# ruiminshen/yolo-tf

Measured on AMD Instinct MI355X. Metric: train_throughput, higher is better.
Workload: dtype bf16; 1 GPU; Darknet-19 YOLOv2 VOC-20 416x416 training step (standardise+fwd+loss+bwd+Adam), batch 16 per GPU (BASELINE configs[1]); global_batch=16, parallelism=dp1, optimizer=adam, weights=random-init (Xavier, seed 0), collective=none (1 rank)

## Files before the change

include/yolo2_hip.h:

```cpp
#ifndef YOLO2_HIP_H
#define YOLO2_HIP_H

#include <stddef.h>
#include <stdint.h>

#ifdef __cplusplus
extern "C" {
#endif

enum { YOLO2_F32 = 0, YOLO2_BF16 = 1 };
enum {
    YOLO2_OK = 0,
    YOLO2_E_ARG = 1,
    YOLO2_E_LAUNCH = 2,
    YOLO2_E_UNSUPPORTED = 3
};

int yolo2_abi_version(void);
const char *yolo2_last_error(void);
uint32_t yolo2_crc32c(const void *data, size_t n, uint32_t crc);
int yolo2_shutdown(void);
int yolo2_check_async_errors(void *stream);
#define YOLO2_ASYNC_ERROR_WORDS 8
int yolo2_async_error_snapshot(unsigned *host_words, void *stream);

size_t yolo2_conv2d_workspace_bytes(int B, int H, int W, int Cp, int Nf, int ksize, int dtype);
size_t yolo2_bn_workspace_bytes(int C);
size_t yolo2_bias_grad_workspace_bytes(int ld);
size_t yolo2_image_prep_workspace_bytes(int B);
size_t yolo2_loss_workspace_bytes(int B, int cells, int A);
size_t yolo2_nms_workspace_bytes(int B, int N, int C);
size_t yolo2_clip_workspace_bytes(int nseg);
size_t yolo2_augment_workspace_bytes(int B);

int yolo2_conv2d(const void *P, const void *F, const float *bias, void *O,
                 int B, int H, int W, int Cp, int ldp, int Nf, int ldo, int ksize,
                 int dtype, void *stream);

int yolo2_conv2d_ws(const void *P, const void *F, const float *bias, void *O, float *ws,
                    size_t ws_bytes, int B, int H, int W, int Cp, int ldp, int Nf, int ldo,
                    int ksize, int dtype, void *stream);

int yolo2_conv2d_wgrad_accumulates(int B, int H, int W, int Cin, int ldx, int Cout, int ldy, int ksize, int dtype);
int yolo2_conv2d_wgrad(const void *X, const void *dY, float *dW,
                       int B, int H, int W, int Cin, int ldx, int Cout, int ldy, int ksize,
                       int dtype, void *stream);

size_t yolo2_conv2d_wgrad_workspace_bytes(int B, int H, int W, int Cin, int ldx, int Cout, int ldy, int ksize, int dtype);
int yolo2_conv2d_wgrad_ws(const void *X, const void *dY, float *dW, float *ws, size_t ws_bytes, int B, int H, int W,
                          int Cin, int ldx, int Cout, int ldy, int ksize, int dtype, void *stream);
int yolo2_set_deterministic(int on);
int yolo2_get_deterministic(void);

int yolo2_filter_prep(const float *W, void *Ffwd, void *Fdgr, int ksize, int Cin, int ldcin,
                      int Cout, int ldcout, int dtype, void *stream);

#define YOLO2_FILTER_PREP_TILE 64
#define YOLO2_FILTER_PREP_TILE_N 128
int yolo2_filter_prep_blocks(int ksize, int ldcin, int ldcout);
typedef struct yolo2_filter_desc {
    const float *W;
    void *Ffwd;
    void *Fdgr;
    int ksize, cin, ldcin, cout, ldcout, first_block;
} yolo2_filter_desc;
int yolo2_filter_prep_batch(const yolo2_filter_desc *descs_device, int n, int total_blocks, int dtype,
                            void *stream);

int yolo2_adam_filter_prep(const yolo2_filter_desc *descs_device, int n, int total_blocks, const long *small_ranges_device, int n_small,
                           float *params, const float *grads, float *m, float *v, float alpha, float beta1, float beta2, float eps,
                           float gscale, int dtype, void *stream);

int yolo2_conv2d_bias_leaky(const void *P, const void *F, const float *bias, void *O, float *ws, size_t ws_bytes, int B,
                            int H, int W, int Cp, int ldp, int Nf, int ldo, int ksize, float alpha, int dtype, void *stream);

int yolo2_conv2d_dgrad_bn(const void *dY, const void *F, void *dX, float *ws, size_t ws_bytes, int B, int H, int W, int Cp, int ldp,
                          int Nf, int ldo, int ksize, const void *Yprev, const float *mean, const float *var, const float *gamma,
                          const float *beta, float *dgamma, float *dbeta, float *bn_part, double *red_ws, float eps, float alpha,
                          int *pending, int dtype, void *stream);
int yolo2_conv2d_dgrad_bn_fuses(int B, int H, int W, int Nf, int ksize, int dtype);
int yolo2_bn_part_to_grads(float *bn_part, int C, float *dgamma, float *dbeta, void *stream);

#define YOLO2_BN_PART_ROWS 256
int yolo2_conv2d_bn(const void *P, const void *F, void *O, float *ws, size_t ws_bytes, int B, int H, int W, int Cp, int ldp,
                    int Nf, int ldo, int ksize, const float *shift, float *bn_part, int dtype, void *stream);
int yolo2_bn_finalize(float *bn_part, const float *shift, long M, int C, float *mean, float *var, float *moving_mean,
                      float *moving_var, double decay, void *stream);

int yolo2_last_bn_part_rows(void);
int yolo2_bn_fin_supported(int rows, int C, int dtype);
int yolo2_bn_leaky_fin(const void *Y, const float *bn_part, int rows, const float *shift, float *mean, float *var, float *moving_mean,
                       float *moving_var, double decay, const float *gamma, const float *beta, void *A, long M, int C, int lda,
                       float eps, float alpha, float *zero, long zero_floats, int dtype, void *stream);
int yolo2_bn_leaky_pool_fin(const void *Y, const float *bn_part, int rows, const float *shift, float *mean, float *var,
                            float *moving_mean, float *moving_var, double decay, const float *gamma, const float *beta, void *P,
                            unsigned char *idx, void *ymax, void *A_full, int B, int H, int W, int C, int ldp, float eps, float alpha,
                            float *zero, long zero_floats, int dtype, void *stream);
int yolo2_bn_leaky_bwd_apply_fin(const void *dA, int ldda, const void *Y, const float *mean, const float *var, const float *gamma,
                                 const float *beta, const float *part, int rows, long plane_stride, float *dgamma, float *dbeta,
                                 void *dY, long M, int C, float eps, float alpha, float *zero, long zero_floats, int dtype, void *stream);
int yolo2_bn_leaky_pool_bwd_apply_fin(const void *dP, int lddp, const unsigned char *idx, const void *Y, const float *mean,
                                      const float *var, const float *gamma, const float *beta, const float *part, int rows,
                                      long plane_stride, float *dgamma, float *dbeta, void *dY, int B, int H, int W, int C, float eps,
                                      float alpha, float *zero, long zero_floats, int dtype, void *stream);
int yolo2_first_layer_wgrad_bn(const void *X, const void *Y, const void *dP, int lddp, const unsigned char *idx, const float *mean, const float *var,
                               const float *gamma, const float *beta, const float *part, int rows, long plane_stride, float *dgamma, float *dbeta,
                               float *dW, int B, int H, int W, int Cin, float eps, float alpha, float *zero, long zero_floats, int dtype, void *stream);
int yolo2_bn_leaky_bwd_reduce_part(const void *dA, int ldda, const void *Y, const float *mean, const float *var, const float *gamma,
                                   const float *beta, double *ws, int *rows, int rows_limit, long M, int C, float eps, float alpha,
                                   int dtype, void *stream);
int yolo2_bn_leaky_pool_bwd_reduce_part(const void *dP, int lddp, const unsigned char *idx, const void *Y, const float *mean,
                                        const float *var, const float *gamma, const float *beta, double *ws, int *rows,
                                        int rows_limit, int B, int H, int W, int C, float eps, float alpha, int dtype, void *stream);

int yolo2_first_layer_stats(const void *P, const void *F, int B, int H, int W, const float *shift, float *bn_part, int dtype, void *stream);
int yolo2_first_layer_bn_leaky_pool(const void *P, const void *F, const float *mean, const float *var, const float *gamma,
                                    const float *beta, void *Pout, unsigned char *idx, int B, int H, int W, int ldp, float eps,
                                    float alpha, int dtype, void *stream);
int yolo2_first_layer_pool_bwd_reduce(const void *P, const void *F, const void *dP, int lddp, const unsigned char *idx,
                                      const float *mean, const float *var, const float *gamma, const float *beta, float *bn_part,
                                      int B, int H, int W, float eps, float alpha, int dtype, void *stream);
int yolo2_first_layer_pool_bwd_apply(const void *P, const void *F, const void *dP, int lddp, const unsigned char *idx,
                                     const float *mean, const float *var, const float *gamma, const float *beta,
                                     const float *dgamma, const float *dbeta, void *dY, int B, int H, int W, float eps, float alpha,
                                     int dtype, void *stream);

int yolo2_bn_stats(const void *Y, float *mean, float *var, double *ws, long M, int C,
                   int dtype, void *stream);
int yolo2_bn_stats_ema(const void *Y, float *mean, float *var, float *moving_mean, float *moving_var,
                       double decay, double *ws, long M, int C, int dtype, void *stream);
int yolo2_bn_ema(float *moving_mean, float *moving_var, const float *mean, const float *var,
                 int C, double decay, void *stream);
int yolo2_bn_leaky(const void *Y, const float *mean, const float *var, const float *gamma,
                   const float *beta, void *A, long M, int C, int lda, float eps, float alpha,
                   int dtype, void *stream);
int yolo2_bn_leaky_bwd_reduce(const void *dA, int ldda, const void *Y, const float *mean,
                              const float *var, const float *gamma, const float *beta,
                              float *dgamma, float *dbeta, double *ws, long M, int C,
                              float eps, float alpha, int dtype, void *stream);
int yolo2_bn_leaky_bwd_apply(const void *dA, int ldda, const void *Y, const float *mean,
                             const float *var, const float *gamma, const float *beta,
                             const float *dgamma, const float *dbeta, void *dY, long M, int C,
                             float eps, float alpha, int dtype, void *stream);

int yolo2_bn_leaky_pool(const void *Y, const float *mean, const float *var, const float *gamma, const float *beta, void *P,
                        unsigned char *idx, int B, int H, int W, int C, int ldp, float eps, float alpha, int dtype, void *stream);
int yolo2_bn_leaky_pool_bwd_reduce(const void *dP, int lddp, const unsigned char *idx, const void *Y, const float *mean,
                                   const float *var, const float *gamma, const float *beta, float *dgamma, float *dbeta,
                                   double *ws, int B, int H, int W, int C, float eps, float alpha, int dtype, void *stream);
int yolo2_bn_leaky_pool_bwd_apply(const void *dP, int lddp, const unsigned char *idx, const void *Y, const float *mean,
                                  const float *var, const float *gamma, const float *beta, const float *dgamma,
                                  const float *dbeta, void *dY, int B, int H, int W, int C, float eps, float alpha,
                                  int dtype, void *stream);

int yolo2_maxpool_fwd(const void *A, void *P, int B, int H, int W, int C, int stride,
                      int dtype, void *stream);
int yolo2_maxpool_bwd(const void *A, const void *dP, void *dA, int B, int H, int W, int C,
                      int stride, int dtype, void *stream);
int yolo2_maxpool_bwd_acc(const void *A, const void *dP, void *dA, int B, int H, int W, int C, int dtype, void *stream);

int yolo2_reorg(const void *in, void *out, int B, int H, int W, int C, int ldo, int dtype,
                void *stream);
int yolo2_reorg_bwd(const void *dout, int ldd, void *din, int B, int H, int W, int C, int dtype,
                    void *stream);
int yolo2_copy_channels(const void *src, int lds, void *dst, int ldd, long M, int C, int dtype,
                        void *stream);
int yolo2_add_inplace(void *dst, const void *src, long n, int dtype, void *stream);
int yolo2_bias_grad(const void *dY, int ld, float *dbias, double *ws, long M, int C, int dtype,
                    void *stream);

int yolo2_image_prep(const float *img, void *out, double *ws, int B, int HW, int mode, int dtype,
                     void *stream);

int yolo2_head_decode(const void *logits, int ld, const float *anchors, float *conf,
                      float *xy_min, float *xy_max, int *nan_flag, int B, int cell_h, int cell_w,
                      int A, int C, int dtype, void *stream);

int yolo2_head_decode_attrs(const void *logits, int ld, const float *anchors, float *iou, float *prob,
                            float *xy, float *wh, int B, int cell_h, int cell_w, int A, int C,
                            int dtype, void *stream);

int yolo2_loss(const void *logits, int ld, const float *anchors, const float *mask,
               const float *prob, const float *coords, const float *off_min, const float *off_max,
               const float *areas, const float *hparam, float *objectives, void *dlogits,
               float *ws, int B, int cell_h, int cell_w, int A, int C, int dtype, void *stream);
int yolo2_loss_partials(const void *logits, int ld, const float *anchors, const float *mask, const float *prob,
                        const float *coords, const float *off_min, const float *off_max, const float *areas,
                        const float *hparam, void *dlogits, float *ws, int B, int cell_h, int cell_w, int A, int C, int dtype,
                        void *stream);
int yolo2_loss_objectives(const float *ws, float *objectives, int B, int cell_h, int cell_w, int A, void *stream);

int yolo1_loss(const void *net, int ld, const float *mask, const float *prob, const float *coords, const float *off_min,
               const float *off_max, const float *areas, const float *hparam, float *objectives, void *dnet, float *ws,
               int B, int cell_h, int cell_w, int boxes_per_cell, int C, int dtype, void *stream);
int yolo1_head_decode(const void *net, int ld, float *conf, float *xy_min, float *xy_max, int *nan_flag, int B, int cell_h,
                      int cell_w, int boxes_per_cell, int C, int dtype, void *stream);
int yolo2_leaky_bwd(const void *A, const void *dA, void *dZ, long n, float alpha, int dtype, void *stream);
int yolo2_dropout(const void *X, void *Y, unsigned char *mask, long n, float keep_prob, unsigned long long seed, int dtype,
                  void *stream);
int yolo2_dropout_bwd(const void *dY, const unsigned char *mask, void *dX, long n, float keep_prob, int dtype, void *stream);
int yolo2_l2_regularizer(const float *w, float *g, long n, float scale, double *loss, void *stream);

int yolo2_nms(float *conf, const float *xy_min, const float *xy_max, int *order_out, int *ws,
              int B, int N, int C, float threshold, float threshold_iou, void *stream);

int yolo2_adam(float *w, const float *g, float *m, float *v, long n, float alpha, float beta1,
               float beta2, float eps, float gscale, void *stream);
int yolo2_momentum(float *w, const float *g, float *acc, long n, float lr, float momentum,
                   float gscale, void *stream);
int yolo2_sgd(float *w, const float *g, long n, float lr, float gscale, void *stream);
int yolo2_rmsprop(float *w, const float *g, float *ms, float *mom, long n, float lr, float decay,
                  float momentum, float eps, float gscale, void *stream);
int yolo2_adagrad(float *w, const float *g, float *acc, long n, float lr, float gscale,
                  void *stream);
int yolo2_adadelta(float *w, const float *g, float *acc, float *acc_update, long n, float lr,
                   float rho, float eps, float gscale, void *stream);
int yolo2_ftrl(float *w, const float *g, float *accum, float *linear, long n, float lr, float lr_power,
               float l1, float l2, float gscale, void *stream);
int yolo2_scale(float *x, long n, float scale, void *stream);
int yolo2_zero_ranges(float *x, const long *ranges_host, int nranges, void *stream);
int yolo2_bn_fold(const float *W, const float *gamma, const float *beta, const float *moving_mean,
                  const float *moving_var, float *Wf, float *bias, long rows, int C, float eps, void *stream);
int yolo2_clip_by_norm(float *g, const long *seg_off, int nseg, float clip, double *ws,
                       void *stream);
size_t yolo2_clip_fixed_workspace_bytes(int nseg);
int yolo2_clip_by_norm_fixed(float *g, const long *seg_off, int nseg, float clip, double *ws, size_t ws_bytes, void *stream);

int yolo2_selftest_tr16(short *out, void *stream);
int yolo2_debug_last_conv_plan(int *out8);
int yolo2_debug_noop(void *stream);
int yolo2_debug_set_igemm_tap(int mode);
int yolo2_debug_set_s4_abl(int abl);
int yolo2_debug_set_pp(int grid, int sched, int min_steps, int min_share);
int yolo2_debug_set_pp_cost(int cv);
int yolo2_debug_set_streamk_wait_us(int us, int unclamped);
int yolo2_debug_last_wgrad_plan(int *out8);
void yolo2_debug_set_wgrad_variant(int variant);
int yolo2_debug_wgrad_row_plan(int B, int H, int W, int Cin, int Cout, int cus, int force_variant, int *out9);
int yolo2_debug_wgrad_ws_plan(int B, int H, int W, int Cin, int ldx, int Cout, int ldy, int ksize, int dtype, int cus, int *out4);
int yolo2_debug_magic_u32(unsigned d, unsigned *m, unsigned *s);

#define YOLO2_AUG_FLIP 1u
#define YOLO2_AUG_BRIGHTNESS 2u
#define YOLO2_AUG_SATURATION 4u
#define YOLO2_AUG_HUE 8u
#define YOLO2_AUG_CONTRAST 16u
#define YOLO2_AUG_NOISE 32u
#define YOLO2_AUG_GRAY 64u
typedef struct yolo2_augment_params {
    long long src_offset;
    int src_w, src_h;
    int crop_x, crop_y, crop_w, crop_h;
    unsigned flags;
    float brightness, saturation, hue, contrast, noise_scale;
    unsigned long long noise_seed;
} yolo2_augment_params;
int yolo2_augment_images(const unsigned char *src, const yolo2_augment_params *params_device, double *ws, float *out,
                         int B, int H, int W, int any_contrast, void *stream);

int yolo2_transform_labels(const int *objects_class, const float *objects_coord, const int *first_object, float *mask,
                           float *prob, float *coords, float *offset_xy_min, float *offset_xy_max, float *areas, int B,
                           int classes, int cell_width, int cell_height, int *error_flag, void *stream);

int yolo2_set_stream_workgroups(int n);
int yolo2_get_stream_workgroups(void);
int yolo2_cast_f32_bf16(const float *src, void *dst, long n, void *stream);
int yolo2_cast_bf16_f32(const void *src, float *dst, long n, void *stream);
int yolo2_debug_occupy(int workgroups, int *stop, int *started, int max_us, void *stream);

enum { YOLO2_EVAL_MODE_DETECT = 0, YOLO2_EVAL_MODE_ALL = 1 };
enum { YOLO2_EVAL_FP = 0, YOLO2_EVAL_TP = 1, YOLO2_EVAL_IGNORED = 2 };
#define YOLO2_EVAL_MAX_GT_PER_IMAGE 512
#define YOLO2_EVAL_MAX_CLASSES (1 << 20)
#define YOLO2_EVAL_STATE_WORDS 2
typedef struct {
    float score;
    int image;
    int box;
    unsigned class_flag;
} yolo2_eval_record;
size_t yolo2_eval_record_bytes(long max_records);
size_t yolo2_eval_collect_workspace_bytes(int B);
size_t yolo2_eval_workspace_bytes(long max_records, int C);
size_t yolo2_eval_result_bytes(int C);
int yolo2_eval_collect(const float *conf, const float *xy_min, const float *xy_max, const int *gt_class, const float *gt_box,
                       const unsigned char *gt_difficult, const int *gt_first, int G, int B, int N, int C, int n_valid, int image_base,
                       int mode, float threshold, float iou_threshold, void *records, long max_records, unsigned long long *state,
                       int *npos, int *ws, void *stream);
int yolo2_eval_finalize(const void *records, long max_records, unsigned long long *state, const int *npos, int C, int n_images, int N,
                        void *ws, size_t ws_bytes, void *results, void *sorted_records, int *cum_tp, int *cum_fp, void *stream);

#define YOLO2_EVAL_COCO_MAX_AREAS 4
#define YOLO2_EVAL_COCO_MAX_IOUS 10
#define YOLO2_EVAL_COCO_MAX_RECALLS 101
#define YOLO2_EVAL_COCO_MAX_SLICES 8
#define YOLO2_EVAL_COCO_MAX_DETS 128
#define YOLO2_EVAL_COCO_MAX_CLASSES 1024
typedef struct {
    float score;
    int image;
    int box;
    int cls;
    int rank;
    unsigned reserved;
    unsigned long long matched;
    unsigned long long ignored;
} yolo2_eval_coco_record;
size_t yolo2_eval_coco_record_bytes(long max_records);
size_t yolo2_eval_coco_collect_workspace_bytes(int B, int N, int C);
size_t yolo2_eval_coco_workspace_bytes(long max_records, int C);
size_t yolo2_eval_coco_result_bytes(int S, int T, int A, int C);
int yolo2_eval_coco_collect(const float *conf, const float *xy_min, const float *xy_max, const int *gt_class, const float *gt_box,
                            const float *gt_area, const unsigned char *gt_flags, const int *gt_first, const float *scale, int G, int B,
                            int N, int C, int n_valid, int image_base, int mode, float threshold, const float *area_ranges, int A,
                            const float *iou_thresholds, int T, int max_dets, void *records, long max_records,
                            unsigned long long *state, int *npig, void *ws, size_t ws_bytes, void *stream);
int yolo2_eval_coco_finalize(const void *records, long max_records, unsigned long long *state, const int *npig, int C, int n_images, int N,
                             int A, int T, int max_dets, const int *slices, int S, const double *recall_thresholds, int R, void *ws,
                             size_t ws_bytes, void *results, void *stream);

#define YOLO2_ANCHOR_MAX_K 32
#define YOLO2_ANCHOR_MAX_JOBS 65535
#define YOLO2_ANCHOR_MAX_BOXES ((1 << 27) - 1)
size_t yolo2_anchor_workspace_bytes(int jobs, int kmax);
int yolo2_anchor_assign(const float *boxes, int n, const float *centroids, const int *job_k, int jobs, int kmax,
                        unsigned long long *ws, size_t ws_bytes, const int *done, unsigned char *assignment, void *stream);
int yolo2_anchor_update(float *centroids, const int *job_k, int jobs, int kmax, unsigned long long *ws, size_t ws_bytes, int n,
                        int *done, int *iterations, long long *counts, double *avg_iou, void *stream);

#define YOLO2_HIST_BUCKETS 1550
#define YOLO2_HIST_WORDS (YOLO2_HIST_BUCKETS + 6)
typedef struct yolo2_hist_job {
    const void *base;
    long long rows;
    int c, ld, dtype;
    int first_item;
} yolo2_hist_job;
size_t yolo2_histogram_workspace_bytes(int njobs);
size_t yolo2_histogram_result_bytes(int njobs);
int yolo2_histogram_items(long long rows, int c, int ld, int dtype);
int yolo2_histogram(const yolo2_hist_job *jobs, int njobs, int items, void *out, size_t out_bytes, void *ws, size_t ws_bytes, void *stream);

#define YOLO2_IMAGE_GROUP 8
#define YOLO2_IMAGE_RECORD_BYTES 16
typedef struct yolo2_image_job {
    const void *base;
    long long rows;
    int c, ld, dtype;
    int first_item;
    long long out_offset;
    long long sum_offset;
} yolo2_image_job;
size_t yolo2_image_summary_workspace_bytes(int njobs, long long sum_pixels);
size_t yolo2_image_summary_result_bytes(int njobs, long long image_bytes);
int yolo2_image_summary_items(long long rows, int c, int ld, int dtype);
int yolo2_image_summary_depth(int c);
int yolo2_image_summary(const yolo2_image_job *jobs, int njobs, int items, void *out, size_t out_bytes, void *ws, size_t ws_bytes, void *stream);

enum { YOLO2_I8_OUT_I8 = 0, YOLO2_I8_OUT_BF16 = 1, YOLO2_I8_OUT_F32 = 2, YOLO2_I8_OUT_ACC = 3 };
int yolo2_conv2d_i8(const void *P, const void *F, const float *mult, const float *bias, void *O, int B, int H, int W, int Cp, int ldp,
                    int Nf, int ldo, int ksize, float alpha, float inv_s_out, int out_kind, void *stream);
typedef struct yolo2_absmax_job {
    const void *base;
    long long rows;
    int c, ld, dtype;
    int slot;
} yolo2_absmax_job;
int yolo2_absmax(const yolo2_absmax_job *jobs, int njobs, unsigned *out, void *stream);
int yolo2_quantize(const void *X, int ldx, void *Q, int ldq, long rows, int c, float inv_s, int dtype, void *stream);
int yolo2_maxpool_i8(const void *A, int lda, void *P, int ldp, int B, int H, int W, int C, int stride, void *stream);
int yolo2_reorg_i8(const void *in, void *out, int B, int H, int W, int C, int ldo, void *stream);

#ifdef __cplusplus
}
#endif
#endif
```

yolo_tf_amd/_lib.py:

```python
import ctypes
import os

_HERE = os.path.dirname(os.path.abspath(__file__))
LIB_PATH = os.environ.get('YOLO2_LIB_PATH') or os.path.join(_HERE, 'csrc', 'libyolo2hip.so')

F32, BF16 = 0, 1
I8_OUT_I8, I8_OUT_BF16, I8_OUT_F32, I8_OUT_ACC = 0, 1, 2, 3


class HipKernelError(RuntimeError):
    pass


_p = ctypes.c_void_p
_i = ctypes.c_int
_l = ctypes.c_long
_f = ctypes.c_float

SIGNATURES = {
    'yolo2_conv2d': [_p, _p, _p, _p, _i, _i, _i, _i, _i, _i, _i, _i, _i, _p],
    'yolo2_conv2d_ws': [_p, _p, _p, _p, _p, ctypes.c_size_t, _i, _i, _i, _i, _i, _i, _i, _i, _i, _p],
    'yolo2_conv2d_bias_leaky': [_p, _p, _p, _p, _p, ctypes.c_size_t, _i, _i, _i, _i, _i, _i, _i, _i, _f, _i, _p],
    'yolo2_conv2d_dgrad_bn': [_p, _p, _p, _p, ctypes.c_size_t, _i, _i, _i, _i, _i, _i, _i, _i, _p, _p, _p, _p, _p, _p, _p, _p, _p, _f, _f, _p, _i, _p],
    'yolo2_bn_part_to_grads': [_p, _i, _p, _p, _p],
    'yolo2_debug_noop': [_p],
    'yolo2_conv2d_wgrad': [_p, _p, _p, _i, _i, _i, _i, _i, _i, _i, _i, _i, _p],
    'yolo2_conv2d_wgrad_ws': [_p, _p, _p, _p, ctypes.c_size_t, _i, _i, _i, _i, _i, _i, _i, _i, _i, _p],
    'yolo2_set_deterministic': [_i],
    'yolo2_filter_prep': [_p, _p, _p, _i, _i, _i, _i, _i, _i, _p],
    'yolo2_filter_prep_batch': [_p, _i, _i, _i, _p],
    'yolo2_adam_filter_prep': [_p, _i, _i, _p, _i, _p, _p, _p, _p, _f, _f, _f, _f, _f, _i, _p],
    'yolo2_first_layer_stats': [_p, _p, _i, _i, _i, _p, _p, _i, _p],
    'yolo2_first_layer_bn_leaky_pool': [_p, _p, _p, _p, _p, _p, _p, _p, _i, _i, _i, _i, _f, _f, _i, _p],
    'yolo2_first_layer_pool_bwd_reduce': [_p, _p, _p, _i, _p, _p, _p, _p, _p, _p, _i, _i, _i, _f, _f, _i, _p],
    'yolo2_first_layer_pool_bwd_apply': [_p, _p, _p, _i, _p, _p, _p, _p, _p, _p, _p, _p, _i, _i, _i, _f, _f, _i, _p],
    'yolo2_conv2d_bn': [_p, _p, _p, _p, ctypes.c_size_t, _i, _i, _i, _i, _i, _i, _i, _i, _p, _p, _i, _p],
    'yolo2_bn_finalize': [_p, _p, _l, _i, _p, _p, _p, _p, ctypes.c_double, _p],
    'yolo2_bn_leaky_fin': [_p, _p, _i, _p, _p, _p, _p, _p, ctypes.c_double, _p, _p, _p, _l, _i, _i, _f, _f, _p, _l, _i, _p],
    'yolo2_bn_leaky_pool_fin': [_p, _p, _i, _p, _p, _p, _p, _p, ctypes.c_double, _p, _p, _p, _p, _p, _p, _i, _i, _i, _i, _i, _f, _f, _p, _l, _i, _p],
    'yolo2_bn_leaky_bwd_apply_fin': [_p, _i, _p, _p, _p, _p, _p, _p, _i, _l, _p, _p, _p, _l, _i, _f, _f, _p, _l, _i, _p],
    'yolo2_first_layer_wgrad_bn': [_p, _p, _p, _i, _p, _p, _p, _p, _p, _p, _i, _l, _p, _p, _p, _i, _i, _i, _i, _f, _f, _p, _l, _i, _p],
    'yolo2_bn_leaky_pool_bwd_apply_fin': [_p, _i, _p, _p, _p, _p, _p, _p, _p, _i, _l, _p, _p, _p, _i, _i, _i, _i, _f, _f, _p, _l, _i, _p],
    'yolo2_bn_leaky_bwd_reduce_part': [_p, _i, _p, _p, _p, _p, _p, _p, _p, _i, _l, _i, _f, _f, _i, _p],
    'yolo2_bn_leaky_pool_bwd_reduce_part': [_p, _i, _p, _p, _p, _p, _p, _p, _p, _p, _i, _i, _i, _i, _i, _f, _f, _i, _p],
    'yolo2_bn_leaky_pool': [_p, _p, _p, _p, _p, _p, _p, _i, _i, _i, _i, _i, _f, _f, _i, _p],
    'yolo2_bn_leaky_pool_bwd_reduce': [_p, _i, _p, _p, _p, _p, _p, _p, _p, _p, _p, _i, _i, _i, _i, _f, _f, _i, _p],
    'yolo2_bn_leaky_pool_bwd_apply': [_p, _i, _p, _p, _p, _p, _p, _p, _p, _p, _p, _i, _i, _i, _i, _f, _f, _i, _p],
    'yolo2_augment_images': [_p, _p, _p, _p, _i, _i, _i, _i, _p],
    'yolo2_transform_labels': [_p, _p, _p, _p, _p, _p, _p, _p, _p, _i, _i, _i, _i, _p, _p],
    'yolo2_bn_stats': [_p, _p, _p, _p, _l, _i, _i, _p],
    'yolo2_bn_stats_ema': [_p, _p, _p, _p, _p, ctypes.c_double, _p, _l, _i, _i, _p],
    'yolo2_bn_ema': [_p, _p, _p, _p, _i, ctypes.c_double, _p],
    'yolo2_bn_leaky': [_p, _p, _p, _p, _p, _p, _l, _i, _i, _f, _f, _i, _p],
    'yolo2_bn_leaky_bwd_reduce': [_p, _i, _p, _p, _p, _p, _p, _p, _p, _p, _l, _i, _f, _f, _i, _p],
    'yolo2_bn_leaky_bwd_apply': [_p, _i, _p, _p, _p, _p, _p, _p, _p, _p, _l, _i, _f, _f, _i, _p],
    'yolo2_maxpool_fwd': [_p, _p, _i, _i, _i, _i, _i, _i, _p],
    'yolo2_maxpool_bwd': [_p, _p, _p, _i, _i, _i, _i, _i, _i, _p],
    'yolo2_maxpool_bwd_acc': [_p, _p, _p, _i, _i, _i, _i, _i, _p],
    'yolo2_reorg': [_p, _p, _i, _i, _i, _i, _i, _i, _p],
    'yolo2_reorg_bwd': [_p, _i, _p, _i, _i, _i, _i, _i, _p],
    'yolo2_copy_channels': [_p, _i, _p, _i, _l, _i, _i, _p],
    'yolo2_add_inplace': [_p, _p, _l, _i, _p],
    'yolo2_bias_grad': [_p, _i, _p, _p, _l, _i, _i, _p],
    'yolo2_image_prep': [_p, _p, _p, _i, _i, _i, _i, _p],
    'yolo2_head_decode': [_p, _i, _p, _p, _p, _p, _p, _i, _i, _i, _i, _i, _i, _p],
    'yolo2_head_decode_attrs': [_p, _i, _p, _p, _p, _p, _p, _i, _i, _i, _i, _i, _i, _p],
    'yolo2_loss': [_p, _i, _p, _p, _p, _p, _p, _p, _p, ctypes.POINTER(_f), _p, _p, _p, _i, _i, _i, _i, _i, _i, _p],
    'yolo2_loss_partials': [_p, _i, _p, _p, _p, _p, _p, _p, _p, ctypes.POINTER(_f), _p, _p, _i, _i, _i, _i, _i, _i, _p],
    'yolo2_loss_objectives': [_p, _p, _i, _i, _i, _i, _p],
    'yolo1_loss': [_p, _i, _p, _p, _p, _p, _p, _p, ctypes.POINTER(_f), _p, _p, _p, _i, _i, _i, _i, _i, _i, _p],
    'yolo1_head_decode': [_p, _i, _p, _p, _p, _p, _i, _i, _i, _i, _i, _i, _p],
    'yolo2_leaky_bwd': [_p, _p, _p, _l, _f, _i, _p],
    'yolo2_dropout': [_p, _p, _p, _l, _f, ctypes.c_ulonglong, _i, _p],
    'yolo2_dropout_bwd': [_p, _p, _p, _l, _f, _i, _p],
    'yolo2_l2_regularizer': [_p, _p, _l, _f, _p, _p],
    'yolo2_nms': [_p, _p, _p, _p, _p, _i, _i, _i, _f, _f, _p],
    'yolo2_adam': [_p, _p, _p, _p, _l, _f, _f, _f, _f, _f, _p],
    'yolo2_momentum': [_p, _p, _p, _l, _f, _f, _f, _p],
    'yolo2_sgd': [_p, _p, _l, _f, _f, _p],
    'yolo2_rmsprop': [_p, _p, _p, _p, _l, _f, _f, _f, _f, _f, _p],
    'yolo2_adagrad': [_p, _p, _p, _l, _f, _f, _p],
    'yolo2_adadelta': [_p, _p, _p, _p, _l, _f, _f, _f, _f, _p],
    'yolo2_clip_by_norm': [_p, _p, _i, _f, _p, _p],
    'yolo2_clip_by_norm_fixed': [_p, _p, _i, _f, _p, ctypes.c_size_t, _p],
    'yolo2_ftrl': [_p, _p, _p, _p, _l, _f, _f, _f, _f, _f, _p],
    'yolo2_scale': [_p, _l, _f, _p],
    'yolo2_zero_ranges': [_p, _p, _i, _p],
    'yolo2_bn_fold': [_p, _p, _p, _p, _p, _p, _p, _l, _i, _f, _p],
    'yolo2_selftest_tr16': [_p, _p],
    'yolo2_set_stream_workgroups': [_i],
    'yolo2_cast_f32_bf16': [_p, _p, _l, _p],
    'yolo2_cast_bf16_f32': [_p, _p, _l, _p],
    'yolo2_debug_occupy': [_i, _p, _p, _i, _p],
    'yolo2_check_async_errors': [_p],
    'yolo2_async_error_snapshot': [_p, _p],
    'yolo2_debug_set_streamk_wait_us': [_i, _i],
    'yolo2_eval_collect': [_p, _p, _p, _p, _p, _p, _p, _i, _i, _i, _i, _i, _i, _i, _f, _f, _p, _l, _p, _p, _p, _p],
    'yolo2_eval_finalize': [_p, _l, _p, _p, _i, _i, _i, _p, ctypes.c_size_t, _p, _p, _p, _p, _p],
    'yolo2_eval_coco_collect': [_p] * 9 + [_i] * 7 + [_f, _p, _i, _p, _i, _i, _p, _l, _p, _p, _p, ctypes.c_size_t, _p],
    'yolo2_eval_coco_finalize': [_p, _l, _p, _p, _i, _i, _i, _i, _i, _i, _p, _i, _p, _i, _p, ctypes.c_size_t, _p, _p],
    'yolo2_anchor_assign': [_p, _i, _p, _p, _i, _i, _p, ctypes.c_size_t, _p, _p, _p],
    'yolo2_anchor_update': [_p, _p, _i, _i, _p, ctypes.c_size_t, _i, _p, _p, _p, _p, _p],
    'yolo2_histogram': [_p, _i, _i, _p, ctypes.c_size_t, _p, ctypes.c_size_t, _p],
    'yolo2_image_summary': [_p, _i, _i, _p, ctypes.c_size_t, _p, ctypes.c_size_t, _p],
    'yolo2_conv2d_i8': [_p, _p, _p, _p, _p, _i, _i, _i, _i, _i, _i, _i, _i, _f, _f, _i, _p],
    'yolo2_absmax': [_p, _i, _p, _p],
    'yolo2_quantize': [_p, _i, _p, _i, _l, _i, _f, _i, _p],
    'yolo2_maxpool_i8': [_p, _i, _p, _i, _i, _i, _i, _i, _i, _p],
    'yolo2_reorg_i8': [_p, _p, _i, _i, _i, _i, _i, _p],
}

QUERIES = {
    'yolo2_abi_version': (_i, []),
    'yolo2_last_error': (ctypes.c_char_p, []),
    'yolo2_shutdown': (_i, []),
    'yolo2_crc32c': (ctypes.c_uint32, [_p, ctypes.c_size_t, ctypes.c_uint32]),
    'yolo2_conv2d_wgrad_accumulates': (_i, [_i] * 9),
    'yolo2_filter_prep_blocks': (_i, [_i, _i, _i]),
    'yolo2_conv2d_dgrad_bn_fuses': (_i, [_i] * 6),
    'yolo2_debug_set_wgrad_variant': (None, [_i]),
    'yolo2_last_bn_part_rows': (_i, []),
    'yolo2_get_stream_workgroups': (_i, []),
    'yolo2_bn_fin_supported': (_i, [_i, _i, _i]),
    'yolo2_debug_last_conv_plan': (_i, [ctypes.POINTER(_i)]),
    'yolo2_debug_set_igemm_tap': (_i, [_i]),
    'yolo2_debug_set_pp': (_i, [_i, _i, _i, _i]),
    'yolo2_debug_set_pp_cost': (_i, [_i]),
    'yolo2_debug_set_s4_abl': (_i, [_i]),
    'yolo2_debug_last_wgrad_plan': (_i, [ctypes.POINTER(_i)]),
    'yolo2_debug_wgrad_row_plan': (_i, [_i, _i, _i, _i, _i, _i, _i, ctypes.POINTER(_i)]),
    'yolo2_debug_wgrad_ws_plan': (_i, [_i] * 10 + [ctypes.POINTER(_i)]),
    'yolo2_conv2d_wgrad_workspace_bytes': (ctypes.c_size_t, [_i] * 9),
    'yolo2_get_deterministic': (_i, []),
    'yolo2_debug_magic_u32': (_i, [ctypes.c_uint, ctypes.POINTER(ctypes.c_uint), ctypes.POINTER(ctypes.c_uint)]),
    'yolo2_conv2d_workspace_bytes': (ctypes.c_size_t, [_i] * 7),
    'yolo2_bn_workspace_bytes': (ctypes.c_size_t, [_i]),
    'yolo2_bias_grad_workspace_bytes': (ctypes.c_size_t, [_i]),
    'yolo2_image_prep_workspace_bytes': (ctypes.c_size_t, [_i]),
    'yolo2_loss_workspace_bytes': (ctypes.c_size_t, [_i, _i, _i]),
    'yolo2_nms_workspace_bytes': (ctypes.c_size_t, [_i, _i, _i]),
    'yolo2_clip_workspace_bytes': (ctypes.c_size_t, [_i]),
    'yolo2_clip_fixed_workspace_bytes': (ctypes.c_size_t, [_i]),
    'yolo2_augment_workspace_bytes': (ctypes.c_size_t, [_i]),
    'yolo2_eval_record_bytes': (ctypes.c_size_t, [_l]),
    'yolo2_eval_collect_workspace_bytes': (ctypes.c_size_t, [_i]),
    'yolo2_eval_workspace_bytes': (ctypes.c_size_t, [_l, _i]),
    'yolo2_eval_result_bytes': (ctypes.c_size_t, [_i]),
    'yolo2_eval_coco_record_bytes': (ctypes.c_size_t, [_l]),
    'yolo2_eval_coco_collect_workspace_bytes': (ctypes.c_size_t, [_i, _i, _i]),
    'yolo2_eval_coco_workspace_bytes': (ctypes.c_size_t, [_l, _i]),
    'yolo2_eval_coco_result_bytes': (ctypes.c_size_t, [_i, _i, _i, _i]),
    'yolo2_anchor_workspace_bytes': (ctypes.c_size_t, [_i, _i]),
    'yolo2_histogram_workspace_bytes': (ctypes.c_size_t, [_i]),
    'yolo2_histogram_result_bytes': (ctypes.c_size_t, [_i]),
    'yolo2_histogram_items': (_i, [ctypes.c_longlong, _i, _i, _i]),
    'yolo2_image_summary_workspace_bytes': (ctypes.c_size_t, [_i, ctypes.c_longlong]),
    'yolo2_image_summary_result_bytes': (ctypes.c_size_t, [_i, ctypes.c_longlong]),
    'yolo2_image_summary_items': (_i, [ctypes.c_longlong, _i, _i, _i]),
    'yolo2_image_summary_depth': (_i, [_i]),
}


class AugmentParams(ctypes.Structure):
    _fields_ = [('src_offset', ctypes.c_longlong), ('src_w', _i), ('src_h', _i), ('crop_x', _i), ('crop_y', _i), ('crop_w', _i), ('crop_h', _i),
                ('flags', ctypes.c_uint), ('brightness', _f), ('saturation', _f), ('hue', _f), ('contrast', _f), ('noise_scale', _f),
                ('noise_seed', ctypes.c_ulonglong)]


class HistJob(ctypes.Structure):
    _fields_ = [('base', ctypes.c_void_p), ('rows', ctypes.c_longlong), ('c', _i), ('ld', _i), ('dtype', _i), ('first_item', _i)]


class ImageJob(ctypes.Structure):
    _fields_ = [('base', ctypes.c_void_p), ('rows', ctypes.c_longlong), ('c', _i), ('ld', _i), ('dtype', _i), ('first_item', _i),
                ('out_offset', ctypes.c_longlong), ('sum_offset', ctypes.c_longlong)]


class AbsmaxJob(ctypes.Structure):
    _fields_ = [('base', ctypes.c_void_p), ('rows', ctypes.c_longlong), ('c', _i), ('ld', _i), ('dtype', _i), ('slot', _i)]


class FilterDesc(ctypes.Structure):
    _fields_ = [('W', ctypes.c_void_p), ('Ffwd', ctypes.c_void_p), ('Fdgr', ctypes.c_void_p), ('ksize', _i), ('cin', _i),
                ('ldcin', _i), ('cout', _i), ('ldcout', _i), ('first_block', _i)]


_lib = None
MISSING = set()


def _mapped_hip_runtimes():
    try:
        with open('/proc/self/maps') as f:
            return sorted({line.split()[-1] for line in f if 'libamdhip64' in line})
    except OSError:
        return []


def load():
    global _lib
    if _lib is not None:
        return _lib
    if not os.path.exists(LIB_PATH):
        raise HipKernelError(
            'HIP extension %s is missing: run `python yolo_tf_amd/csrc/build.py` (or __graft_entry__.build()). '
            'There is no CPU fallback.' % LIB_PATH)
    import torch
    lib = ctypes.CDLL(LIB_PATH)
    runtimes = _mapped_hip_runtimes()
    if len(runtimes) > 1:
        raise HipKernelError('two HIP runtimes are mapped in this process (%s): something loaded %s before torch' % (', '.join(runtimes), LIB_PATH))
    baseline = os.environ.get('YOLO2_LIB_BASELINE') == '1' and bool(os.environ.get('YOLO2_LIB_PATH'))

    def resolve(name):
        try:
            return getattr(lib, name)
        except AttributeError:
            if not baseline:
                raise
            MISSING.add(name)

            def absent(*_args, _name=name):
                raise HipKernelError('%s is not exported by the baseline library %s' % (_name, LIB_PATH))
            setattr(lib, name, absent)
            return None
    for name, (res, args) in QUERIES.items():
        fn = resolve(name)
        if fn is not None:
            fn.restype = res
            fn.argtypes = args
    for name, args in SIGNATURES.items():
        fn = resolve(name)
        if fn is not None:
            fn.restype = _i
            fn.argtypes = args
    _lib = lib
    over = env_overrides()
    if over:
        import warnings
        warnings.warn('YOLO2_* switches set in the environment change kernel selection away from the tested defaults: %s' % ', '.join(over))
    return lib


def env_overrides():
    return sorted('%s=%s' % (k, v) for k, v in os.environ.items() if k.startswith('YOLO2_'))


def query(name, *args):
    return getattr(load(), name)(*args)


def call(name, *args):
    lib = load()
    rc = getattr(lib, name)(*args)
    if rc != 0:
        raise HipKernelError('%s failed (code %d): %s' % (name, rc, lib.yolo2_last_error().decode()))


def ptr(t):
    return None if t is None else t.data_ptr()


def dtype_code(torch_dtype):
    import torch
    if torch_dtype == torch.float32:
        return F32
    if torch_dtype == torch.bfloat16:
        return BF16
    raise ValueError('unsupported dtype %r' % (torch_dtype,))
```

yolo_tf_amd/csrc/conv_c64.hip:

```cpp
#include "common.h"
#include "conv_shared.h"
#include <atomic>

#define C64_TP 256
#define C64_KSTEPS 36
#define C64_STAT_ROWS 32
#define C64_FPITCH 1168

__device__ __forceinline__ int c64_slot_filter(int rho) { return 16 * ((rho >> 2) & 1) + (rho & 3) + 4 * (rho >> 3); }
__device__ __forceinline__ unsigned c64_div(unsigned q, unsigned m, unsigned s) { return __umulhi(q, m) >> s; }

struct C64Geo {
    int H, W, M, Mp;
    int L;
    int RR;
    int HLa;
    int NP0;
    int shl_off;
    unsigned mP, sP, mH, sH;
};

template <int MODE, int NFG>
__global__ __launch_bounds__(512) void conv_c64_fwd_kernel(
    const bf16 *__restrict__ X, unsigned x_bytes, const bf16 *__restrict__ F, bf16 *__restrict__ O, C64Geo g,
    const float *__restrict__ vec, float *__restrict__ bn_part, float alpha) {
    extern __shared__ __attribute__((aligned(1024))) unsigned char smem[];
    constexpr int NB = NFG == 4 ? 2 : 1;
    constexpr int NPASS = NFG == 4 ? 2 : 1;
    constexpr int ROWB = NFG * 64;
    const int H = g.H, W = g.W, Mp = g.Mp;
    const int tid = threadIdx.x, lane = tid & 63;
    const int wave = __builtin_amdgcn_readfirstlane(tid >> 6);
    const int fg = NFG == 4 ? (wave & 3) : 0;
    const int pg = NFG == 4 ? (wave >> 2) : wave;
    const int half = lane >> 5, l31 = lane & 31;
    const unsigned P1 = (unsigned)(W + 1), H1 = (unsigned)(H + 1);
    const int s0 = (int)blockIdx.x * g.L;
    const int e0 = min(s0 + g.L, Mp);
    if (s0 >= Mp) return;
    const int RRB = g.RR * 128, NPR = g.RR >> 3;
    const int pbase = s0 - g.HLa;

    const __amdgpu_buffer_rsrc_t rsrcX = __builtin_amdgcn_make_buffer_rsrc(const_cast<bf16 *>(X), 0, x_bytes, 0x00020000);
    typedef __attribute__((address_space(3))) void *lds_void_ptr;
    typedef const __attribute__((address_space(3))) bf16x8 *lds_frag_ptr;

    bf16x8 filt[C64_KSTEPS];
    auto load_filter = [&]() {
        constexpr int RPR = NFG == 4 ? 64 : 32, FROUND = RPR * C64_FPITCH;
        const __amdgpu_buffer_rsrc_t rsrcF = __builtin_amdgcn_make_buffer_rsrc(const_cast<bf16 *>(F), 0, (unsigned)(NFG * 32) * 1152u, 0x00020000);
        unsigned char *const fst = smem + g.NP0 * 1024;
#pragma unroll 1
        for (int rd = 0; rd < (NFG == 4 ? 2 : 1); ++rd) {
            for (int p = wave; p * 1024 < FROUND; p += 8) {
                const int pos = p * 1024 + lane * 16;
                const int n = pos / C64_FPITCH, off = pos - n * C64_FPITCH;
                const unsigned voff = (off < 1152 && n < RPR) ? (unsigned)((RPR * rd + n) * 1152 + off) : Y2_OOB;
                __builtin_amdgcn_raw_ptr_buffer_load_lds(rsrcF, (lds_void_ptr)(fst + p * 1024), 16, voff, 0, 0, 0);
            }
            asm volatile("s_waitcnt vmcnt(0)" ::: "memory");
            __syncthreads();
            if (NFG == 1 || (fg >> 1) == rd) {
                const unsigned a0 = y2_lds_addr(fst) + (unsigned)((32 * (fg & 1) + c64_slot_filter(l31)) * C64_FPITCH + 16 * half);
#pragma unroll
                for (int st = 0; st < C64_KSTEPS; ++st) filt[st] = *(lds_frag_ptr)(uintptr_t)(a0 + (unsigned)(st * 32));
            }
            __syncthreads();
        }
    };

    const int prow = lane >> 3;
    auto stage_piece = [&](int j, int slot) {
        const int row = j * 8 + prow;
        const unsigned q = (unsigned)(pbase + row);
        const unsigned R = c64_div(q, g.mP, g.sP);
        const unsigned img = c64_div(R, g.mH, g.sH);
        const unsigned c = q - __umul24(R, P1), r = R - __umul24(img, H1);
        const bool ok = (q < (unsigned)Mp) & (c < (unsigned)W) & (r < (unsigned)H);
        const unsigned m = q - R - __umul24(img, (unsigned)W);
        const unsigned voff = ok ? m * 128u + (unsigned)((((lane & 7) ^ ((row >> 1) & 7))) << 4) : Y2_OOB;
        __builtin_amdgcn_raw_ptr_buffer_load_lds(rsrcX, (lds_void_ptr)(smem + slot * 1024), 16, voff, 0, 0, 0);
    };
    for (int j = wave; j < g.NP0; j += 8) stage_piece(j, j);
    load_filter();

    const unsigned lds0 = y2_lds_addr(smem);
    unsigned abase[9];
#pragma unroll
    for (int tp = 0; tp < 9; ++tp) {
        const int shift = (tp / 3 - 1) * (W + 1) + (tp % 3 - 1);
        const int row = pg * (NFG == 4 ? 64 : 32) + l31 + g.HLa + shift;
        abase[tp] = (unsigned)(row * 128 + ((half ^ ((row >> 1) & 7)) << 4));
    }

    typedef __attribute__((ext_vector_type(2))) float f32x2;
    f32x2 cst[8];
    float *const shl = reinterpret_cast<float *>(smem + g.shl_off);
    float tq[8];
#pragma unroll
    for (int qd = 0; qd < 8; ++qd) tq[qd] = 0.f;
    if (MODE == 1) {
        if (tid < 128) shl[tid] = vec ? vec[tid] : 0.f;
        asm volatile("s_waitcnt lgkmcnt(0)" ::: "memory");
    }
#pragma unroll
    for (int r2 = 0; r2 < 8; ++r2) {
        const int f = 32 * fg + 16 * half + 2 * r2;
        cst[r2] = (MODE == 2 && vec) ? f32x2{vec[f], vec[f + 1]} : f32x2{0.f, 0.f};
    }

    const int T = (e0 - s0 + C64_TP - 1) / C64_TP;
    int pslot = g.NP0;
    if (pslot >= NPR) pslot -= NPR;
    unsigned tro = 0;
    for (int t = 0; t < T; ++t) {
        __builtin_amdgcn_s_barrier();
        const int tb = s0 + t * C64_TP;
        if (t + 1 < T) {
#pragma unroll
            for (int u = 0; u < 4; ++u) {
                const int k = wave + 8 * u;
                int sl = pslot + k;
                if (sl >= NPR) sl -= NPR;
                stage_piece(g.NP0 + t * 32 + k, sl);
            }
        }
        pslot += 32;
        if (pslot >= NPR) pslot -= NPR;
#pragma unroll 1
        for (int pa = 0; pa < NPASS; ++pa) {
            if (tb + pa * 128 >= e0) break;
            f32x16 acc[2];
#pragma unroll
            for (int i = 0; i < 2; ++i)
#pragma unroll
                for (int r = 0; r < 16; ++r) acc[i][r] = 0.f;
            unsigned poff = tro + (unsigned)(pa * 16384);
            if (poff >= (unsigned)RRB) poff -= (unsigned)RRB;
            bf16x8 fb[2][NB];
            unsigned ad[NB];
            auto load = [&](int st, int set) {
                const int tp = st >> 2, kk = st & 3;
                if (kk == 0) {
                    unsigned x = abase[tp] + poff;
#pragma unroll
                    for (int i = 0; i < NB; ++i) {
                        x = min(x, x - (unsigned)RRB);
                        ad[i] = x + lds0;
                        x += 4096u;
                    }
                }
#pragma unroll
                for (int i = 0; i < NB; ++i) fb[set][i] = *(lds_frag_ptr)(uintptr_t)(ad[i] ^ (unsigned)(kk * 32));
            };
            load(0, 0);
#pragma unroll
            for (int st = 0; st < C64_KSTEPS; ++st) {
                if (st + 1 < C64_KSTEPS) load(st + 1, (st + 1) & 1);
                __builtin_amdgcn_sched_barrier(0);
                if (NFG == 4) {
#pragma unroll
                    for (int i = 0; i < NB; ++i) acc[i] = __builtin_amdgcn_mfma_f32_32x32x16_bf16(filt[st], fb[st & 1][i], acc[i], 0, 0, 0);
                } else {
                    acc[st & 1] = __builtin_amdgcn_mfma_f32_32x32x16_bf16(filt[st], fb[st & 1][0], acc[st & 1], 0, 0, 0);
                }
                __builtin_amdgcn_sched_barrier(0);
            }
            if (NFG == 1) {
#pragma unroll
                for (int r = 0; r < 16; ++r) acc[0][r] += acc[1][r];
            }
#if defined(__HIP_DEVICE_COMPILE__)
            if (pa == NPASS - 1 || tb + (pa + 1) * 128 >= e0)
                asm volatile("s_waitcnt vmcnt(0)" ::: "memory");
            const bool odd = (lane & 1) != 0;
            typedef __attribute__((ext_vector_type(2))) __bf16 bf16x2;
            unsigned pk[NB][8];
            float lfi[NB];
            unsigned moffi[NB];
#pragma unroll
            for (int i = 0; i < NB; ++i) {
                const unsigned q = (unsigned)(tb + (NFG == 4 ? pa * 128 + pg * 64 + i * 32 : pg * 32) + l31);
                const unsigned R = c64_div(q, g.mP, g.sP);
                const unsigned c = q - __umul24(R, P1);
                const unsigned img = c64_div(R, g.mH, g.sH);
                const unsigned r_ = R - __umul24(img, H1);
                const bool live = (q < (unsigned)e0) & (c < (unsigned)W) & (r_ < (unsigned)H);
                const unsigned m = __umul24(__umul24(img, (unsigned)H) + r_, (unsigned)W) + c;
                moffi[i] = live ? m * (unsigned)ROWB + (unsigned)(fg * 64 + half * 32) : 0xffffffffu;
                lfi[i] = live ? 1.0f : 0.0f;
#pragma unroll
                for (int qd = 0; qd < 8; ++qd) {
                    float v0 = acc[i][2 * qd], v1 = acc[i][2 * qd + 1];
                    if (MODE == 2) {
                        v0 += cst[qd][0]; v1 += cst[qd][1];
                        v0 = fmaxf(v0, alpha * v0); v1 = fmaxf(v1, alpha * v1);
                    }
                    const bf16x2 o2 = {(bf16)v0, (bf16)v1};
                    pk[i][qd] = __builtin_bit_cast(unsigned, o2);
                }
            }
            __builtin_amdgcn_sched_barrier(0);
#pragma unroll
            for (int i = 0; i < NB; ++i) {
                unsigned s0_[4], s1_[4];
#pragma unroll
                for (int d = 0; d < 4; ++d) {
                    const unsigned x = pk[i][d], y = pk[i][4 + d];
                    const unsigned xs = (unsigned)__builtin_amdgcn_mov_dpp((int)x, 0xB1, 0xF, 0xF, true), ys = (unsigned)__builtin_amdgcn_mov_dpp((int)y, 0xB1, 0xF, 0xF, true);
                    s0_[d] = odd ? ys : x;
                    s1_[d] = odd ? y : xs;
                }
                const unsigned mo_even = (unsigned)__builtin_amdgcn_mov_dpp((int)moffi[i], 0xA0, 0xF, 0xF, true);
                const unsigned mo_odd = (unsigned)__builtin_amdgcn_mov_dpp((int)moffi[i], 0xF5, 0xF, 0xF, true);
                const unsigned lo16 = odd ? 16u : 0u;
                if (mo_even != 0xffffffffu)
                    *reinterpret_cast<u32x4 *>(reinterpret_cast<unsigned char *>(O) + mo_even + lo16) = u32x4{s0_[0], s0_[1], s0_[2], s0_[3]};
                if (mo_odd != 0xffffffffu)
                    *reinterpret_cast<u32x4 *>(reinterpret_cast<unsigned char *>(O) + mo_odd + lo16) = u32x4{s1_[0], s1_[1], s1_[2], s1_[3]};
            }
            __builtin_amdgcn_sched_barrier(0);
            if (MODE == 1 && bn_part) {
                const bool odd2 = (lane & 2) != 0;
#pragma unroll
                for (int qd = 0; qd < 8; ++qd) {
                    const f32x2 svq = *reinterpret_cast<const f32x2 *>(shl + 32 * fg + 16 * half + 2 * qd);
                    f32x2 a1 = {0.f, 0.f}, a2 = {0.f, 0.f};
#pragma unroll
                    for (int i = 0; i < NB; ++i) {
                        const f32x2 lf2 = {lfi[i], lfi[i]};
                        const f32x2 y2 = {__builtin_bit_cast(float, pk[i][qd] << 16), __builtin_bit_cast(float, pk[i][qd] & 0xffff0000u)};
                        const f32x2 d2 = (y2 - svq) * lf2;
                        a1 += d2;
                        a2 = __builtin_elementwise_fma(d2, d2, a2);
                    }
                    float k0, k1;
                    {
                        const float t0_ = odd ? a1[0] : a2[0], t1_ = odd ? a1[1] : a2[1];
                        const float r0 = __builtin_bit_cast(float, __builtin_amdgcn_mov_dpp(__builtin_bit_cast(int, t0_), 0xB1, 0xF, 0xF, true));
                        const float r1 = __builtin_bit_cast(float, __builtin_amdgcn_mov_dpp(__builtin_bit_cast(int, t1_), 0xB1, 0xF, 0xF, true));
                        k0 = (odd ? a2[0] : a1[0]) + r0;
                        k1 = (odd ? a2[1] : a1[1]) + r1;
                    }
                    {
                        const float s_ = odd2 ? k0 : k1;
                        const float r_ = __builtin_bit_cast(float, __builtin_amdgcn_mov_dpp(__builtin_bit_cast(int, s_), 0x4E, 0xF, 0xF, true));
                        tq[qd] += (odd2 ? k1 : k0) + r_;
                    }
                }
            }
#endif
        }
        tro += (unsigned)(C64_TP * 128);
        if (tro >= (unsigned)RRB) tro -= (unsigned)RRB;
    }
    if (MODE == 1 && bn_part) {
#pragma unroll
        for (int o = 4; o <= 16; o <<= 1) {
            float x[8];
#pragma unroll
            for (int qd = 0; qd < 8; ++qd) x[qd] = __shfl_xor(tq[qd], o, 64);
#pragma unroll
            for (int qd = 0; qd < 8; ++qd) tq[qd] += x[qd];
        }
        if (l31 < 4) {
            const int slot = (int)(blockIdx.x & (C64_STAT_ROWS - 1));
            const int plane = lane & 1, par = (lane >> 1) & 1;
#pragma unroll
            for (int qd = 0; qd < 8; ++qd)
                unsafeAtomicAdd(bn_part + (plane * Y2_BN_PART_ROWS + slot) * 128 + 32 * fg + 16 * half + 2 * qd + par, tq[qd]);
        }
    }
}

#define C64W_TP 128
__global__ __launch_bounds__(512) void conv_c64_wide_kernel(const bf16 *__restrict__ X, unsigned x_bytes, const bf16 *__restrict__ F, bf16 *__restrict__ O, C64Geo g) {
    extern __shared__ __attribute__((aligned(1024))) unsigned char smem[];
    constexpr int TP = C64W_TP;
    const int H = g.H, W = g.W, Mp = g.Mp;
    const int tid = threadIdx.x, lane = tid & 63;
    const int wave = __builtin_amdgcn_readfirstlane(tid >> 6);
    const int fg = wave & 1, kh = (wave >> 1) & 1, pg = wave >> 2;
    const int half = lane >> 5, l31 = lane & 31;
    const unsigned P1 = (unsigned)(W + 1), H1 = (unsigned)(H + 1);
    const int s0 = (int)blockIdx.x * g.L;
    const int e0 = min(s0 + g.L, Mp);
    if (s0 >= Mp) return;
    const int RRB = g.RR * 128, NPR = g.RR >> 3;
    const int pbase = s0 - g.HLa;
    unsigned char *const xchg = smem + 2 * RRB;

    const __amdgpu_buffer_rsrc_t rsrcX = __builtin_amdgcn_make_buffer_rsrc(const_cast<bf16 *>(X), 0, x_bytes, 0x00020000);
    typedef __attribute__((address_space(3))) void *lds_void_ptr;
    typedef const __attribute__((address_space(3))) bf16x8 *lds_frag_ptr;

    const int prow = lane >> 3;
    auto stage_piece = [&](int j, int slot) {
        const int row = j * 8 + prow;
        const unsigned q = (unsigned)(pbase + row);
        const unsigned R = c64_div(q, g.mP, g.sP);
        const unsigned img = c64_div(R, g.mH, g.sH);
        const unsigned c = q - __umul24(R, P1), r = R - __umul24(img, H1);
        const bool ok = (q < (unsigned)Mp) & (c < (unsigned)W) & (r < (unsigned)H);
        const unsigned m = q - R - __umul24(img, (unsigned)W);
        const unsigned voff = ok ? m * 256u + (unsigned)((((lane & 7) ^ ((row >> 1) & 7))) << 4) : Y2_OOB;
        __builtin_amdgcn_raw_ptr_buffer_load_lds(rsrcX, (lds_void_ptr)(smem + slot * 1024), 16, voff, 0, 0, 0);
        __builtin_amdgcn_raw_ptr_buffer_load_lds(rsrcX, (lds_void_ptr)(smem + RRB + slot * 1024), 16, ok ? voff + 128u : Y2_OOB, 0, 0, 0);
    };
    for (int j = wave; j < g.NP0; j += 8) stage_piece(j, j);

    bf16x8 filt[C64_KSTEPS];
    {
        constexpr int FROUND = 32 * C64_FPITCH;
        const __amdgpu_buffer_rsrc_t rsrcF = __builtin_amdgcn_make_buffer_rsrc(const_cast<bf16 *>(F), 0, 64u * 2304u, 0x00020000);
        unsigned char *const fst = smem + RRB + g.NP0 * 1024;
#pragma unroll 1
        for (int rd = 0; rd < 4; ++rd) {
            const int fgr = rd & 1, khr = rd >> 1;
            for (int p = wave; p * 1024 < FROUND; p += 8) {
                const int pos = p * 1024 + lane * 16;
                const int n = pos / C64_FPITCH, off = pos - n * C64_FPITCH;
                const unsigned voff = (off < 1152 && n < 32) ? (unsigned)((32 * fgr + n) * 2304 + khr * 1152 + off) : Y2_OOB;
                __builtin_amdgcn_raw_ptr_buffer_load_lds(rsrcF, (lds_void_ptr)(fst + p * 1024), 16, voff, 0, 0, 0);
            }
            asm volatile("s_waitcnt vmcnt(0)" ::: "memory");
            __syncthreads();
            if (fg == fgr && kh == khr) {
                const unsigned a0 = y2_lds_addr(fst) + (unsigned)(c64_slot_filter(l31) * C64_FPITCH + 16 * half);
#pragma unroll
                for (int st = 0; st < C64_KSTEPS; ++st) filt[st] = *(lds_frag_ptr)(uintptr_t)(a0 + (unsigned)(st * 32));
            }
            __syncthreads();
        }
    }

    const unsigned lds0 = y2_lds_addr(smem) + (unsigned)(kh * RRB);
    unsigned abase[9];
#pragma unroll
    for (int tp = 0; tp < 9; ++tp) {
        const int shift = (tp / 3 - 1) * (W + 1) + (tp % 3 - 1);
        const int row = pg * 64 + l31 + g.HLa + shift;
        abase[tp] = (unsigned)(row * 128 + ((half ^ ((row >> 1) & 7)) << 4));
    }

    const int T = (e0 - s0 + TP - 1) / TP;
    int pslot = g.NP0;
    if (pslot >= NPR) pslot -= NPR;
    unsigned tro = 0;
    for (int t = 0; t < T; ++t) {
        __builtin_amdgcn_s_barrier();
        const int tb = s0 + t * TP;
        if (t + 1 < T) {
#pragma unroll
            for (int u = 0; u < 2; ++u) {
                const int k = wave + 8 * u;
                int sl = pslot + k;
                if (sl >= NPR) sl -= NPR;
                stage_piece(g.NP0 + t * (TP / 8) + k, sl);
            }
        }
        pslot += TP / 8;
        if (pslot >= NPR) pslot -= NPR;
        f32x16 acc[2];
#pragma unroll
        for (int i = 0; i < 2; ++i)
#pragma unroll
            for (int r = 0; r < 16; ++r) acc[i][r] = 0.f;
        bf16x8 fb[2][2];
        unsigned ad[2];
        auto load = [&](int st, int set) {
            const int tp = st >> 2, kk = st & 3;
            if (kk == 0) {
                unsigned x = abase[tp] + tro;
#pragma unroll
                for (int i = 0; i < 2; ++i) {
                    x = min(x, x - (unsigned)RRB);
                    ad[i] = x + lds0;
                    x += 4096u;
                }
            }
#pragma unroll
            for (int i = 0; i < 2; ++i) fb[set][i] = *(lds_frag_ptr)(uintptr_t)(ad[i] ^ (unsigned)(kk * 32));
        };
        load(0, 0);
#pragma unroll
        for (int st = 0; st < C64_KSTEPS; ++st) {
            if (st + 1 < C64_KSTEPS) load(st + 1, (st + 1) & 1);
            __builtin_amdgcn_sched_barrier(0);
#pragma unroll
            for (int i = 0; i < 2; ++i) acc[i] = __builtin_amdgcn_mfma_f32_32x32x16_bf16(filt[st], fb[st & 1][i], acc[i], 0, 0, 0);
            __builtin_amdgcn_sched_barrier(0);
        }
#if defined(__HIP_DEVICE_COMPILE__)
        f32x16 keep, give;
#pragma unroll
        for (int r = 0; r < 16; ++r) { keep[r] = kh ? acc[1][r] : acc[0][r]; give[r] = kh ? acc[0][r] : acc[1][r]; }
        {
            f32x4 *const xw = reinterpret_cast<f32x4 *>(xchg + wave * 4096);
#pragma unroll
            for (int q4 = 0; q4 < 4; ++q4) xw[q4 * 64 + lane] = f32x4{give[4 * q4], give[4 * q4 + 1], give[4 * q4 + 2], give[4 * q4 + 3]};
            asm volatile("s_waitcnt lgkmcnt(0)" ::: "memory");
            __builtin_amdgcn_s_barrier();
            const f32x4 *const xr = reinterpret_cast<const f32x4 *>(xchg + (wave ^ 2) * 4096);
#pragma unroll
            for (int q4 = 0; q4 < 4; ++q4) {
                const f32x4 v = xr[q4 * 64 + lane];
                keep[4 * q4] += v[0]; keep[4 * q4 + 1] += v[1]; keep[4 * q4 + 2] += v[2]; keep[4 * q4 + 3] += v[3];
            }
        }
        asm volatile("s_waitcnt vmcnt(0)" ::: "memory");
        {
            const bool odd = (lane & 1) != 0;
            typedef __attribute__((ext_vector_type(2))) __bf16 bf16x2;
            const unsigned q = (unsigned)(tb + pg * 64 + kh * 32 + l31);
            const unsigned R = c64_div(q, g.mP, g.sP);
            const unsigned c = q - __umul24(R, P1);
            const unsigned img = c64_div(R, g.mH, g.sH);
            const unsigned r_ = R - __umul24(img, H1);
            const bool live = (q < (unsigned)e0) & (c < (unsigned)W) & (r_ < (unsigned)H);
            const unsigned m = __umul24(__umul24(img, (unsigned)H) + r_, (unsigned)W) + c;
            const unsigned moff = live ? m * 128u + (unsigned)(fg * 64 + half * 32) : 0xffffffffu;
            unsigned pk[8];
#pragma unroll
            for (int qd = 0; qd < 8; ++qd) {
                const bf16x2 o2 = {(bf16)keep[2 * qd], (bf16)keep[2 * qd + 1]};
                pk[qd] = __builtin_bit_cast(unsigned, o2);
            }
            unsigned s0_[4], s1_[4];
#pragma unroll
            for (int d = 0; d < 4; ++d) {
                const unsigned x = pk[d], y = pk[4 + d];
                const unsigned xs = (unsigned)__builtin_amdgcn_mov_dpp((int)x, 0xB1, 0xF, 0xF, true), ys = (unsigned)__builtin_amdgcn_mov_dpp((int)y, 0xB1, 0xF, 0xF, true);
                s0_[d] = odd ? ys : x;
                s1_[d] = odd ? y : xs;
            }
            const unsigned mo_even = (unsigned)__builtin_amdgcn_mov_dpp((int)moff, 0xA0, 0xF, 0xF, true);
            const unsigned mo_odd = (unsigned)__builtin_amdgcn_mov_dpp((int)moff, 0xF5, 0xF, 0xF, true);
            const unsigned lo16 = odd ? 16u : 0u;
            if (mo_even != 0xffffffffu)
                *reinterpret_cast<u32x4 *>(reinterpret_cast<unsigned char *>(O) + mo_even + lo16) = u32x4{s0_[0], s0_[1], s0_[2], s0_[3]};
            if (mo_odd != 0xffffffffu)
                *reinterpret_cast<u32x4 *>(reinterpret_cast<unsigned char *>(O) + mo_odd + lo16) = u32x4{s1_[0], s1_[1], s1_[2], s1_[3]};
        }
#endif
        tro += (unsigned)(TP * 128);
        if (tro >= (unsigned)RRB) tro -= (unsigned)RRB;
    }
}

static int y2_c64_wide(const void *P, const void *F, void *O, int B, int H, int W, int cus, hipStream_t st) {
    const long Mp = (long)B * (H + 1) * (W + 1);
    if (Mp + 2 * C64W_TP >= (1L << 23) || H < 1 || W < 1 || cus < 1) return 1;
    C64Geo g;
    g.H = H; g.W = W; g.M = B * H * W; g.Mp = (int)Mp;
    g.L = (int)(((Mp + cus - 1) / cus + C64W_TP - 1) / C64W_TP) * C64W_TP;
    const int grid = (int)((Mp + g.L - 1) / g.L);
    g.HLa = (W + 2 + 7) & ~7;
    g.NP0 = (g.HLa + C64W_TP + W + 2 + 7) / 8;
    g.RR = (8 * g.NP0 + C64W_TP + 63) & ~63;
    g.shl_off = 0;
    const size_t plane = (size_t)g.RR * 128, lds = 2 * plane + 8 * 4096;
    if (lds > 160 * 1024 || (plane - (size_t)g.NP0 * 1024) + 8 * 4096 < 37 * 1024) return 1;
    y2_magic_u32((unsigned)(W + 1), &g.mP, &g.sP);
    y2_magic_u32((unsigned)(H + 1), &g.mH, &g.sH);
    static std::atomic<size_t> lds_set[64];
    int dev = 0;
    if (hipGetDevice(&dev) != hipSuccess || dev < 0 || dev >= 64) dev = 0;
    if (lds > lds_set[dev].load(std::memory_order_relaxed)) {
        if (hipFuncSetAttribute((const void *)conv_c64_wide_kernel, hipFuncAttributeMaxDynamicSharedMemorySize, (int)lds) != hipSuccess) return 1;
        lds_set[dev].store(lds, std::memory_order_relaxed);
    }
    conv_c64_wide_kernel<<<grid, 512, lds, st>>>((const bf16 *)P, (unsigned)((size_t)g.M * 128 * 2), (const bf16 *)F, (bf16 *)O, g);
    return 0;
}

bool y2_c64_shape(int Cp, int ldp, int Nf, int ldo, int ksize, int dtype) {
    if (dtype != YOLO2_BF16 || ksize != 3) return false;
    if (Cp == 128 && ldp == 128) return Nf == 64 && ldo == 64;
    return Cp == 64 && ldp == 64 && ((Nf == 128 && ldo == 128) || (Nf == 32 && ldo == 32));
}

int y2_c64_fwd(const void *P, const void *F, void *O, int B, int H, int W, int Nf, const float *bias, float alpha, const float *bn_shift, float *bn_part,
               int cus, int *rows, hipStream_t st) {
    if (Nf == 64) {
        if (bn_part || bias || alpha != 1.0f) return 1;
        if (rows) *rows = 0;
        return y2_c64_wide(P, F, O, B, H, W, cus, st);
    }
    const long Mp = (long)B * (H + 1) * (W + 1);
    if (Mp + 2 * C64_TP >= (1L << 23) || H < 1 || W < 1 || cus < 1) return 1;
    const bool narrow = Nf == 32;
    if (narrow && (bn_part || bias || alpha != 1.0f)) return 1;
    C64Geo g;
    g.H = H; g.W = W; g.M = B * H * W; g.Mp = (int)Mp;
    const int gran = narrow ? 256 : 128;
    g.L = (int)(((Mp + cus - 1) / cus + gran - 1) / gran) * gran;
    const int grid = (int)((Mp + g.L - 1) / g.L);
    g.HLa = (W + 2 + 7) & ~7;
    g.NP0 = (g.HLa + C64_TP + W + 2 + 7) / 8;
    g.RR = (8 * g.NP0 + C64_TP + 63) & ~63;
    const size_t fround = (size_t)(narrow ? 32 : 64) * C64_FPITCH;
    size_t lds = (size_t)g.RR * 128;
    if (lds < (size_t)g.NP0 * 1024 + (fround + 1023) / 1024 * 1024) lds = (size_t)g.NP0 * 1024 + (fround + 1023) / 1024 * 1024;
    g.shl_off = (int)lds;
    lds += 512;
    if (lds > 160 * 1024) return 1;
    y2_magic_u32((unsigned)(W + 1), &g.mP, &g.sP);
    y2_magic_u32((unsigned)(H + 1), &g.mH, &g.sH);
    const unsigned x_bytes = (unsigned)((size_t)g.M * 64 * 2);
    static std::atomic<size_t> lds_set[4][64];
    int dev = 0;
    if (hipGetDevice(&dev) != hipSuccess || dev < 0 || dev >= 64) dev = 0;
#define C64_LAUNCH(SLOT, MODEv, NFGv, vecp)                                                                                                  \
    do {                                                                                                                                     \
        if (lds > lds_set[SLOT][dev].load(std::memory_order_relaxed)) {                                                                      \
            if (hipFuncSetAttribute((const void *)conv_c64_fwd_kernel<MODEv, NFGv>, hipFuncAttributeMaxDynamicSharedMemorySize, (int)lds) != hipSuccess) return 1; \
            lds_set[SLOT][dev].store(lds, std::memory_order_relaxed);                                                                        \
        }                                                                                                                                    \
        conv_c64_fwd_kernel<MODEv, NFGv><<<grid, 512, lds, st>>>((const bf16 *)P, x_bytes, (const bf16 *)F, (bf16 *)O, g, vecp, bn_part, alpha); \
    } while (0)
    if (narrow) C64_LAUNCH(3, 0, 1, (const float *)nullptr);
    else if (bn_part) C64_LAUNCH(1, 1, 4, bn_shift);
    else if (bias || alpha != 1.0f) C64_LAUNCH(2, 2, 4, bias);
    else C64_LAUNCH(0, 0, 4, (const float *)nullptr);
#undef C64_LAUNCH
    if (rows) *rows = grid < C64_STAT_ROWS ? grid : C64_STAT_ROWS;
    return 0;
}
```

yolo_tf_amd/csrc/conv_igemm.hip:

```cpp
#include "common.h"
#include "conv_shared.h"
#include "conv_epilogue.h"
#include <stdlib.h>
#include <atomic>
#include <mutex>
#include <type_traits>

template <typename T> struct Mma;
template <> struct Mma<bf16> {
    static constexpr int KSTEP = 16;
    typedef bf16x8 Frag;
    static __device__ __forceinline__ f32x16 mma(Frag a, Frag b, f32x16 c) {
        return __builtin_amdgcn_mfma_f32_32x32x16_bf16(a, b, c, 0, 0, 0);
    }
};
template <> struct Mma<float> {
    static constexpr int KSTEP = 2;
    typedef float Frag;
    static __device__ __forceinline__ f32x16 mma(Frag a, Frag b, f32x16 c) {
        return __builtin_amdgcn_mfma_f32_32x32x2f32(a, b, c, 0, 0, 0);
    }
};

template <typename T, int BN, int WGN, int NSTAGE, int KS, int SPLITK, bool CTAIL, int CH = 4, int NW = 4, int BMv = 128, bool BNBWD = false>
// ... 443 lines not shown
extern "C" int yolo2_async_error_snapshot(unsigned *host_words, void *stream) {
    if (!host_words) { yolo2_set_error("yolo2_async_error_snapshot: host_words is NULL"); return YOLO2_E_ARG; }
    int dev = 0;
    if (hipGetDevice(&dev) != hipSuccess || dev < 0 || dev >= 64) { yolo2_set_error("yolo2_async_error_snapshot: no current device"); return YOLO2_E_LAUNCH; }
    unsigned *pool;
    {
        std::lock_guard<std::mutex> lock(g_flag_mutex);
        pool = g_flag_pool[dev];
    }
    if (!pool) {
        for (int i = 0; i < YOLO2_ASYNC_ERROR_WORDS; ++i) host_words[i] = 0u;
        return YOLO2_OK;
    }
    static_assert(YOLO2_ASYNC_ERROR_WORDS == Y2_STREAM_FLAG_SETS, "one status word per flag set");
    async_error_gather_kernel<<<1, 64, 0, (hipStream_t)stream>>>(pool, host_words);
    Y2_CHECK_LAUNCH();
    return YOLO2_OK;
}
extern "C" int yolo2_check_async_errors(void *stream) {
    int dev = 0;
    if (hipStreamSynchronize((hipStream_t)stream) != hipSuccess || hipGetDevice(&dev) != hipSuccess || dev < 0 || dev >= 64) {
        yolo2_set_error("yolo2_check_async_errors: HIP error: %s", hipGetErrorString(hipGetLastError()));
        return YOLO2_E_LAUNCH;
    }
    std::lock_guard<std::mutex> lock(g_flag_mutex);
    if (!g_flag_pool[dev]) return YOLO2_OK;
    unsigned status[Y2_STREAM_FLAG_SETS] = {0};
    if (hipMemcpy2D(status, sizeof(unsigned), g_flag_pool[dev] + Y2_STREAM_FLAG_WORDS, Y2_STREAM_FLAG_STRIDE * sizeof(unsigned), sizeof(unsigned),
                    Y2_STREAM_FLAG_SETS, hipMemcpyDeviceToHost) != hipSuccess) {
        yolo2_set_error("yolo2_check_async_errors: reading the stream-K status words failed");
        return YOLO2_E_LAUNCH;
    }
    unsigned gave_up = 0;
    for (int i = 0; i < Y2_STREAM_FLAG_SETS; ++i) gave_up += status[i];
    if (!gave_up) return YOLO2_OK;
    (void)hipDeviceSynchronize();
    (void)hipMemset(g_flag_pool[dev], 0, (size_t)Y2_STREAM_FLAG_SETS * Y2_STREAM_FLAG_STRIDE * sizeof(unsigned));
    const unsigned ticks = g_sk_wait_ticks.load(std::memory_order_relaxed);
    for (int i = 0; ticks && i < Y2_STREAM_FLAG_SETS; ++i)
        (void)hipMemcpy(g_flag_pool[dev] + (size_t)i * Y2_STREAM_FLAG_STRIDE + Y2_STREAM_FLAG_WORDS + 1, &ticks, sizeof(ticks), hipMemcpyHostToDevice);
    yolo2_set_error("stream-K hand-off: %u wait(s) for a partner workgroup's partial tile gave up; convolution outputs since the last check are invalid", gave_up);
    return YOLO2_E_LAUNCH;
}
extern "C" int yolo2_debug_set_streamk_wait_us(int us, int unclamped) {
    if (us < 0 || (unsigned)us > 0xffffffffu / 100u) { yolo2_set_error("yolo2_debug_set_streamk_wait_us: us outside 0 .. %u (100 MHz ticks in 32 bits)", 0xffffffffu / 100u); return YOLO2_E_ARG; }
    const unsigned ticks = (unsigned)us * 100u;
    g_sk_wait_ticks.store(ticks, std::memory_order_relaxed);
    g_sk_unclamped.store(unclamped, std::memory_order_relaxed);
    int dev = 0;
    if (hipGetDevice(&dev) != hipSuccess || dev < 0 || dev >= 64) { yolo2_set_error("yolo2_debug_set_streamk_wait_us: no current device"); return YOLO2_E_LAUNCH; }
    std::lock_guard<std::mutex> lock(g_flag_mutex);
    if (!ensure_pool_locked(dev)) { yolo2_set_error("yolo2_debug_set_streamk_wait_us: no flag pool"); return YOLO2_E_LAUNCH; }
    (void)hipDeviceSynchronize();
    for (int i = 0; i < Y2_STREAM_FLAG_SETS; ++i)
        if (hipMemcpy(g_flag_pool[dev] + (size_t)i * Y2_STREAM_FLAG_STRIDE + Y2_STREAM_FLAG_WORDS + 1, &ticks, sizeof(ticks), hipMemcpyHostToDevice) != hipSuccess)
            return YOLO2_E_LAUNCH;
    return YOLO2_OK;
}
extern "C" int yolo2_shutdown(void) {
    std::lock_guard<std::mutex> lock(g_flag_mutex);
    int cur = 0;
    (void)hipGetDevice(&cur);
    for (int d = 0; d < 64; ++d)
        if (g_flag_pool[d]) {
            if (hipSetDevice(d) == hipSuccess) { (void)hipDeviceSynchronize(); (void)hipFree(g_flag_pool[d]); }
            g_flag_pool[d] = nullptr;
            g_flag_counter[d] = 0;
        }
    (void)hipSetDevice(cur);
    return YOLO2_OK;
}

static int choose_ksplit(int tiles, int nk, int target) {
    if (target <= 0 || nk < 128 || tiles > 128) return 1;
    int ks = (target + tiles - 1) / tiles;
    int max_ks = nk / 8;
    if (ks > max_ks) ks = max_ks;
    return ks < 1 ? 1 : ks;
}

static thread_local int g_last_plan[8] = {0, 0, 0, 0, 0, 0, 0, 0};
static thread_local int g_last_stat_rows = Y2_BN_PART_ROWS;
static int y2_stat_rows_limit(int Nf, int vec) {
    int lpr = Nf / vec;
    if (lpr > 16) lpr = 16;
    if (lpr < 1) lpr = 1;
    const long lim = (128L << 10) / ((long)lpr * vec * 8);
    return lim > Y2_BN_PART_ROWS ? Y2_BN_PART_ROWS : (int)lim;
}
static int y2_stat_rows(long wave_rows, int limit) {
    if (wave_rows <= limit) return (int)wave_rows;
    int r = 16;
    while (r < 128 && (long)r * 16 < wave_rows) r <<= 1;
    while (r > limit) r >>= 1;
    return r;
}
static Y2BnBwd y2_with_stat_rows(Y2BnBwd bz, long wave_rows, int Nf, int vec) {
    const int limit = y2_stat_rows_limit(Nf, vec);
    const int r = y2_stat_rows(wave_rows, limit);
    g_last_stat_rows = r;
    bz.stat_mask_inv = wave_rows <= limit ? 0 : (Y2_BN_PART_ROWS - 1) ^ (r - 1);
    return bz;
}
extern "C" int yolo2_last_bn_part_rows(void) { return g_last_stat_rows; }
#define Y2_IGEMM_ARGS (const T *)P, p_bytes, (const T *)F, f_bytes, bias, (T *)O, ws, H, W, Cp, ldp, Nf, ldo, M, NT, remap, bn_shift
#define Y2_IGEMM_BM(BMv, BNv, WGNv, NSv, KSv, SPLITv, CTv, CHv, NWv, gridv)                                        \
    do {                                                                                                           \
        const dim3 g_ = (gridv);                                                                                   \
        const int plan_[8] = {BMv, BNv, NWv, CHv, NSv, SPLITv, (int)g_.x, (int)g_.y};                              \
        for (int i_ = 0; i_ < 8; ++i_) g_last_plan[i_] = plan_[i_];                                                \
        typedef Y2IgemmPlan<T, BMv, BNv, WGNv, NSv, CHv, NWv> Plan_;       \
                                                 \
        const bool fusedbw_ = bz.Y && SPLITv != 1 && !CTv && wide_store && Plan_::WIDE_FITS;                       \
        const Y2BnBwd bz_ = y2_with_stat_rows(bz, (long)cdiv(M, BMv) * (fusedbw_ ? Plan_::STAT_ROWS_BNBWD : Plan_::STAT_ROWS_FWD), Nf, VEC); \
        if (!bz.Y)                                                                                                 \
            conv_igemm_kernel<T, BNv, WGNv, NSv, KSv, SPLITv, CTv, CHv, NWv, BMv, false><<<g_, NWv * 64, 0, st>>>(  \
                Y2_IGEMM_ARGS, bn_part, sk_flags, act_alpha, wide_store, bz_);                                     \
        else if (fusedbw_)                                                                                         \
            conv_igemm_kernel<T, BNv, WGNv, NSv, KSv, (SPLITv == 1 ? 0 : SPLITv), false, CHv, NWv, BMv, true><<<g_, NWv * 64, 0, st>>>( \
                Y2_IGEMM_ARGS, bn_part, sk_flags, act_alpha, wide_store, bz_);                                     \
        else {       \
            *stats_done = false;                                                                                   \
            conv_igemm_kernel<T, BNv, WGNv, NSv, KSv, SPLITv, CTv, CHv, NWv, BMv, false><<<g_, NWv * 64, 0, st>>>(  \
                Y2_IGEMM_ARGS, nullptr, sk_flags, act_alpha, wide_store, Y2BnBwd{nullptr, nullptr, nullptr, nullptr, nullptr, 0.f, 0.f, 0}); \
        }                                                                                                          \
    } while (0)
#define Y2_IGEMM(BNv, WGNv, NSv, KSv, SPLITv, CTv, CHv, NWv, gridv) Y2_IGEMM_BM(128, BNv, WGNv, NSv, KSv, SPLITv, CTv, CHv, NWv, gridv)
#define Y2_IGEMM_KS_CT(BNv, WGNv, NSv, SPLITv, NWv, gridv)                              \
    do {                                                                               \
        if (ksize == 3) {                                                              \
            if (ctail) Y2_IGEMM(BNv, WGNv, NSv, 3, SPLITv, true, 4, NWv, gridv);       \
            else Y2_IGEMM(BNv, WGNv, NSv, 3, SPLITv, false, 4, NWv, gridv);            \
        } else {                                                                       \
            if (ctail) Y2_IGEMM(BNv, WGNv, NSv, 1, SPLITv, true, 4, NWv, gridv);       \
            else Y2_IGEMM(BNv, WGNv, NSv, 1, SPLITv, false, 4, NWv, gridv);            \
        }                                                                              \
    } while (0)
#define Y2_IGEMM_KS_WIDE(SPLITv, gridv)                                                 \
    do {                                                                               \
        if (ksize == 3) Y2_IGEMM(128, 2, 3, 3, SPLITv, false, 8, 8, gridv);            \
        else Y2_IGEMM(128, 2, 3, 1, SPLITv, false, 8, 8, gridv);                       \
    } while (0)

static std::atomic<int> g_igemm_tap{y2_env_int("YOLO2_IGEMM_TAP", 2)};
extern "C" int yolo2_debug_set_igemm_tap(int mode) {
    g_igemm_tap.store(mode == 3 ? 3 : (mode != 0 ? 2 : 0), std::memory_order_relaxed);
    return YOLO2_OK;
}
static std::atomic<int> g_s4_abl{0};
extern "C" int yolo2_debug_set_s4_abl(int abl) {
    g_s4_abl.store(abl, std::memory_order_relaxed);
    return YOLO2_OK;
}
static std::atomic<int> g_pp_grid{0};
static std::atomic<int> g_pp_dmapos{y2_env_int("YOLO2_PP_SCHED", 2)};
static std::atomic<long> g_pp_min_steps{18};
static std::atomic<long> g_pp_min_share{24};
static const int g_pp_long_share = y2_env_int("YOLO2_PP_LONG_SHARE", 26);
static std::atomic<int> g_pp_cv{y2_env_int("YOLO2_PP_CV", 6)};
extern "C" int yolo2_debug_set_pp_cost(int cv) {
    if (cv < 0 || cv > 4096) { yolo2_set_error("yolo2_debug_set_pp_cost: 0 .. 4096 K steps"); return YOLO2_E_ARG; }
    g_pp_cv.store(cv, std::memory_order_relaxed);
    return YOLO2_OK;
}
extern "C" int yolo2_debug_set_pp(int grid, int dmapos, int min_steps, int min_share) {
    if (grid != -1) g_pp_grid.store(grid, std::memory_order_relaxed);
    if (dmapos >= 0) g_pp_dmapos.store(dmapos, std::memory_order_relaxed);
    if (min_steps >= 0) g_pp_min_steps.store(min_steps, std::memory_order_relaxed);
    if (min_share >= 0) g_pp_min_share.store(min_share, std::memory_order_relaxed);
    return YOLO2_OK;
}

static std::atomic<int> g_stream_wgs{0};
extern "C" int yolo2_set_stream_workgroups(int n) {
    if (n < 0 || n > Y2_STREAM_FLAG_WORDS) { yolo2_set_error("yolo2_set_stream_workgroups: 0 (default) .. %d", Y2_STREAM_FLAG_WORDS); return YOLO2_E_ARG; }
    g_stream_wgs.store(n, std::memory_order_relaxed);
    return YOLO2_OK;
}
extern "C" int yolo2_get_stream_workgroups(void) {
    const int n = g_stream_wgs.load(std::memory_order_relaxed);
    return n > 0 ? n : tune().cus;
}
static Tune tune_now() {
    Tune t = tune();
    const int n = g_stream_wgs.load(std::memory_order_relaxed);
    if (n > 0) { t.cus = n; t.stream_max_tiles = 3 * n; }
    return t;
}

template <typename T>
static int launch_conv(const void *P, const void *F, const float *bias, void *O, float *ws, size_t ws_bytes, int B, int H, int W,
                       int Cp, int ldp, int Nf, int ldo, int ksize, hipStream_t st, const float *bn_shift, float *bn_part, bool *stats_done, float act_alpha,
                       const Y2BnBwd bz = Y2BnBwd{nullptr, nullptr, nullptr, nullptr, nullptr, 0.f, 0.f, 0}) {
    const int M = B * H * W;
    const int MT = cdiv(M, 128);
    constexpr int VEC = 16 / sizeof(T);
    constexpr int BK = 4 * VEC;
    const Tune tu = tune_now();
    const unsigned p_bytes = (unsigned)((size_t)M * ldp * sizeof(T));
    const unsigned f_bytes = (unsigned)((size_t)Nf * ksize * ksize * Cp * sizeof(T));
    const bool ctail = (Cp % BK) != 0;
    unsigned *sk_flags = nullptr;
    const int wide_store = ((uintptr_t)O & 15) == 0 && ldo % VEC == 0 && (Nf % VEC == 0 || ldo < Nf + VEC);
    const int remap = tu.remap >= 0 ? tu.remap : (f_bytes <= (3u << 19) ? 1 : 0);
    const int MT2 = cdiv(M, 256), NT2 = cdiv(Nf, 128);
    const long nk_wide = (Cp % (8 * VEC) == 0) ? (long)ksize * ksize * (Cp / (8 * VEC)) : 0;
    if constexpr (std::is_same<T, bf16>::value) {
        const int tap_mode = g_igemm_tap.load(std::memory_order_relaxed);
        if (tap_mode != 0 && ksize == 3 && Cp % 64 == 0 && W <= 55 && Nf > 64 && wide_store && ws && tu.stream &&
            (long)9 * (Cp / 64) >= g_pp_min_steps.load(std::memory_order_relaxed) && tu.cus <= Y2_STREAM_FLAG_WORDS) {
            const long tiles_t = (long)MT2 * NT2, units_p = tiles_t * 9 * (Cp / 64);
            const int gm = g_pp_grid.load(std::memory_order_relaxed);
            const bool can_stream = (size_t)tu.cus * 256 * 128 * sizeof(float) <= ws_bytes;
            int grid = 0;
            if (gm == 1) grid = can_stream ? tu.cus : 0;
            else if (gm == 2) grid = tiles_t <= Y2_STREAM_FLAG_WORDS ? (int)tiles_t : 0;
            else if (gm >= 8) grid = (can_stream && gm <= tu.cus) ? gm : 0;
            else if (gm <= -2) grid = (can_stream && tiles_t * -gm <= tu.cus) ? (int)(tiles_t * -gm) : 0;
            else if (tiles_t * 10 >= (long)tu.cus * 6 && tiles_t <= tu.cus) grid = (int)tiles_t;
            else if (can_stream && ((units_p >= g_pp_min_share.load(std::memory_order_relaxed) * tu.cus && tiles_t * 4 >= tu.cus) ||
                                    (bz.Y && M >= 8192 && units_p >= 10L * tu.cus) ||
                                    (g_pp_long_share > 0 && units_p >= (long)g_pp_long_share * tu.cus && tiles_t * 8 >= tu.cus))) grid = tu.cus;
            if (grid > units_p && !g_sk_unclamped.load(std::memory_order_relaxed)) grid = (int)units_p;
            if (grid > 0 && (sk_flags = stream_flags()) != nullptr) {
                const int plan_[8] = {256, 128, 8, 8, 18, 2, grid, 1};
                for (int i_ = 0; i_ < 8; ++i_) g_last_plan[i_] = plan_[i_];
                const int tile_rows = tap_mode == 3 ? (bz.Y ? Y2S_STAT_ROWS_BNBWD : Y2S_STAT_ROWS_FWD) : (bz.Y ? Y2P_STAT_ROWS_BNBWD : Y2P_STAT_ROWS_FWD);
                const Y2BnBwd bz_ = y2_with_stat_rows(bz, (long)MT2 * tile_rows, Nf, VEC);
                int cv = grid == tiles_t ? 0 : g_pp_cv.load(std::memory_order_relaxed);
                if (cv > units_p / grid / 2) cv = (int)(units_p / grid / 2);
                g_last_plan[7] = 1 + (cv << 8);
                if (tap_mode == 3) {
                    g_last_plan[2] = 4;
                    if (y2_conv3x3_s4_launch(P, p_bytes, F, f_bytes, bias, O, ws, H, W, Cp, ldp, Nf, ldo, M, NT2, bn_shift, bn_part, sk_flags, act_alpha, bz_, 1, grid,
                                             g_s4_abl.load(std::memory_order_relaxed), st) == 0)
                        return 0;
                    g_last_plan[2] = 8;
                }
                if (y2_conv3x3_pp_launch(P, p_bytes, F, f_bytes, bias, O, ws, H, W, Cp, ldp, Nf, ldo, M, NT2, bn_shift, bn_part, sk_flags, act_alpha, bz_,
                                          1, grid, g_pp_dmapos.load(std::memory_order_relaxed), cv, st) == 0)
                    return 0;
            }
        }
    }
    if (Nf > 64 && tu.bm256 && ws && tu.stream && nk_wide >= 128 && MT2 * NT2 >= 64 && MT2 * NT2 <= 3 * tu.cus && tu.cus <= Y2_STREAM_FLAG_WORDS &&
        (size_t)tu.cus * 256 * 128 * sizeof(float) <= ws_bytes && (sk_flags = stream_flags()) != nullptr) {
        const int NT = NT2;
        dim3 grid(tu.cus);
        if (ksize == 3) Y2_IGEMM_BM(256, 128, 2, 3, 3, 2, false, 8, 8, grid);
        else Y2_IGEMM_BM(256, 128, 2, 3, 1, 2, false, 8, 8, grid);
    } else if (Nf > 64) {
        const int NT = cdiv(Nf, 128);
        int ks = (ws && !y2_deterministic()) ? choose_ksplit(MT * NT, ksize * ksize * cdiv(Cp, 4 * VEC), tu.target_blocks) : 1;
        if (ks > 1 && (size_t)M * Nf * sizeof(float) > ws_bytes) ks = 1;
        const bool wide = tu.wide && ks == 1 && MT * NT <= 256 && Cp % (8 * VEC) == 0;
        const long units = (long)MT * NT * ksize * ksize * (Cp / (8 * VEC));
        const bool stream = tu.stream && ws && tu.wide && Cp % (8 * VEC) == 0 && units >= 24L * tu.cus &&
                            (MT * NT < tu.cus || (MT * NT <= tu.stream_max_tiles && units / (MT * NT) >= 96)) &&
                            tu.cus <= Y2_STREAM_FLAG_WORDS && (size_t)tu.cus * 128 * 128 * sizeof(float) <= ws_bytes &&
                            (sk_flags = stream_flags()) != nullptr;
        if (stream) {
            dim3 grid(tu.cus);
            if (ksize == 3) Y2_IGEMM(128, 2, 3, 3, 2, false, 8, 8, grid);
            else Y2_IGEMM(128, 2, 3, 1, 2, false, 8, 8, grid);
        } else if (ks > 1) {
            *stats_done = false;
            if (hipMemsetAsync(ws, 0, (size_t)M * Nf * sizeof(float), st) != hipSuccess) return 1;
            dim3 grid(MT * NT, ks);
            Y2_IGEMM_KS_CT(128, 2, 3, 1, 4, grid);
            long total = (long)M * Nf;
            int g = (int)((total + 255) / 256 < 2048 ? (total + 255) / 256 : 2048);
            splitk_finish_kernel<T><<<g, 256, 0, st>>>(ws, bias, (T *)O, M, Nf, ldo, act_alpha);
        } else {
            ws = nullptr;
            dim3 grid(MT * NT);
            if (wide) Y2_IGEMM_KS_WIDE(0, grid);
            else if (Cp % (8 * VEC) == 0) {
                if (ksize == 3) Y2_IGEMM(128, 2, 2, 3, 0, false, 8, 8, grid);
                else Y2_IGEMM(128, 2, 2, 1, 0, false, 8, 8, grid);
            } else Y2_IGEMM_KS_CT(128, 2, 3, 0, 8, grid);
        }
    } else {
        const int NT = 1;
        ws = nullptr;
        dim3 grid(MT);
        if (ksize == 3 && Cp % (8 * VEC) == 0) {
            if (Nf > 32) Y2_IGEMM(64, 1, 2, 3, 0, false, 8, 4, grid);
            else Y2_IGEMM(32, 1, 2, 3, 0, false, 8, 4, grid);
        } else if (Nf > 32) Y2_IGEMM_KS_CT(64, 1, 3, 0, 4, grid);
        else Y2_IGEMM_KS_CT(32, 1, 3, 0, 4, grid);
    }
    return 0;
}

static bool y2_dgrad_bn_fuses(int B, int H, int W, int Nf, int ksize, int dtype) {
    static const bool fuse = y2_env_int("YOLO2_FUSE_BN_BWD", 1) != 0;
    static const bool fuse_narrow = y2_env_int("YOLO2_FUSE_BN_BWD_NARROW", 0) != 0;
    const int vec = dtype == YOLO2_BF16 ? 8 : 4;
    return fuse && Nf % vec == 0 && (fuse_narrow || !(ksize == 3 && Nf <= 64 && (long)B * H * W >= 100000));
}
extern "C" int yolo2_conv2d_dgrad_bn_fuses(int B, int H, int W, int Nf, int ksize, int dtype) {
    return (B > 0 && H > 0 && W > 0 && Nf > 0 && (dtype == YOLO2_F32 || dtype == YOLO2_BF16) && y2_dgrad_bn_fuses(B, H, W, Nf, ksize, dtype)) ? 1 : 0;
}

static int conv2d_impl(const void *P, const void *F, const float *bias, void *O, float *ws, size_t ws_bytes, int B, int H,
                       int W, int Cp, int ldp, int Nf, int ldo, int ksize, int dtype, void *stream, const char *fn,
                       const float *bn_shift = nullptr, float *bn_part = nullptr, float act_alpha = 1.0f, const Y2BnBwd *bwd = nullptr,
                       float *dgamma = nullptr, float *dbeta = nullptr, double *red_ws = nullptr, int *pending = nullptr) {
    if (!(P && F && O) || !(B > 0 && H > 0 && W > 0 && Cp > 0 && Nf > 0) || !(ksize == 1 || ksize == 3) || !(ldp >= Cp && ldo >= Nf)) {
        yolo2_set_error("%s: argument check failed: pointers / extents / ksize / strides", fn);
        return YOLO2_E_ARG;
    }
    const int vec = dtype == YOLO2_BF16 ? 8 : 4;
    const size_t esz = dtype == YOLO2_BF16 ? 2 : 4;
    if ((size_t)B * H * W * (size_t)ldp * esz >= (1ull << 31) || (size_t)Nf * ksize * ksize * Cp * esz >= (1ull << 31) || (size_t)B * H * W >= (1ull << 31) ||
        Cp % vec || ldp % vec || ((uintptr_t)P & 15) || ((uintptr_t)F & 15)) {
        yolo2_set_error("%s: argument check failed: operand >= 2 GiB or misaligned (channels must be a multiple of %d)", fn, vec);
        return YOLO2_E_ARG;
    }
    int rc = 0;
    static const bool first_direct = y2_env_int("YOLO2_FIRST_DIRECT", 1) != 0;
    if (first_direct && !bias && !bwd && act_alpha == 1.0f && y2_first_layer_shape(Cp, ldp, Nf, ldo, ksize)) {
        if (dtype != YOLO2_F32 && dtype != YOLO2_BF16) { yolo2_set_error("%s: bad dtype %d", fn, dtype); return YOLO2_E_ARG; }
        y2_first_layer_fwd(P, F, O, B, H, W, dtype, (hipStream_t)stream, bn_shift, bn_part);
        for (int i = 0; i < 8; ++i) g_last_plan[i] = -1;
        g_last_stat_rows = Y2_BN_PART_ROWS;
        Y2_CHECK_LAUNCH();
        return YOLO2_OK;
    }
    static const bool c32_direct = y2_env_int("YOLO2_C32", 1) != 0;
    if (c32_direct && !bwd && y2_c32_shape(Cp, ldp, Nf, ldo, ksize, dtype) && ((uintptr_t)O & 15) == 0) {
        const Tune tu = tune_now();
        int rows = 0;
        if (y2_c32_fwd(P, F, O, B, H, W, bias, act_alpha, bn_shift, bn_part, tu.cus, &rows, (hipStream_t)stream) == 0) {
            const int plan_[8] = {512, 64, 8, 8, 9, 0, rows, 1};
            for (int i = 0; i < 8; ++i) g_last_plan[i] = plan_[i];
            if (bn_part) g_last_stat_rows = rows;
            Y2_CHECK_LAUNCH();
            return YOLO2_OK;
        }
    }
    static const bool c64_direct = y2_env_int("YOLO2_C64", 1) != 0;
    if (c64_direct && !bwd && y2_c64_shape(Cp, ldp, Nf, ldo, ksize, dtype) && ((uintptr_t)O & 15) == 0 && ((uintptr_t)F & 15) == 0) {
        const Tune tu = tune_now();
        int rows = 0;
        if (y2_c64_fwd(P, F, O, B, H, W, Nf, bias, act_alpha, bn_shift, bn_part, tu.cus, &rows, (hipStream_t)stream) == 0) {
            const int plan_[8] = {Nf == 64 ? 128 : 256, Nf, 8, 8, 9, 0, rows, 1};
            for (int i = 0; i < 8; ++i) g_last_plan[i] = plan_[i];
            if (bn_part) g_last_stat_rows = rows;
            Y2_CHECK_LAUNCH();
            return YOLO2_OK;
        }
    }
    bool stats_done = true;
    if (bwd) {
        static const bool d1_direct = y2_env_int("YOLO2_D1", 1) != 0;
        const bool can = y2_dgrad_bn_fuses(B, H, W, Nf, ksize, dtype);
        if (can && d1_direct && bn_part && y2_d1_shape(Cp, ldp, Nf, ldo, ksize, dtype, (long)B * H * W) && ((uintptr_t)O & 15) == 0 && ((uintptr_t)bwd->Y & 15) == 0) {
            const Tune tu = tune_now();
            int rows = 0;
            if (y2_d1_dgrad_bn(P, F, O, (long)B * H * W, Cp, Nf, bn_part, *bwd, tu.cus, &rows, (hipStream_t)stream) == 0) {
                const int plan_[8] = {128, 128, 8, Cp / 8, 1, 0x100, rows, Nf / 128};
                for (int i = 0; i < 8; ++i) g_last_plan[i] = plan_[i];
                g_last_stat_rows = rows;
                Y2_CHECK_LAUNCH();
                if (pending) *pending = 1;
                return pending ? YOLO2_OK : y2_bn_part_to_grads(bn_part, Nf, dgamma, dbeta, (hipStream_t)stream);
            }
        }
        if (can) {
            Y2_DISPATCH_DTYPE(dtype, rc = launch_conv<T>(P, F, bias, O, ws, ws_bytes, B, H, W, Cp, ldp, Nf, ldo, ksize, (hipStream_t)stream,
                                                         nullptr, bn_part, &stats_done, act_alpha, *bwd));
        } else {
            stats_done = false;
            Y2_DISPATCH_DTYPE(dtype, rc = launch_conv<T>(P, F, bias, O, ws, ws_bytes, B, H, W, Cp, ldp, Nf, ldo, ksize, (hipStream_t)stream,
                                                         nullptr, nullptr, &stats_done, act_alpha));
            stats_done = false;
        }
        if (rc) { yolo2_set_error("%s: workspace memset failed", fn); return YOLO2_E_LAUNCH; }
        Y2_CHECK_LAUNCH();
        g_last_plan[5] |= stats_done ? 0x100 : 0;
        if (pending) *pending = stats_done ? 1 : 0;
        if (stats_done) return pending ? YOLO2_OK : y2_bn_part_to_grads(bn_part, Nf, dgamma, dbeta, (hipStream_t)stream);
        return yolo2_bn_leaky_bwd_reduce(O, ldo, bwd->Y, bwd->mean, bwd->var, bwd->gamma, bwd->beta, dgamma, dbeta, red_ws, (long)B * H * W, Nf,
                                         bwd->eps, bwd->alpha, dtype, stream);
    }
    Y2_DISPATCH_DTYPE(dtype, rc = launch_conv<T>(P, F, bias, O, ws, ws_bytes, B, H, W, Cp, ldp, Nf, ldo, ksize, (hipStream_t)stream,
                                                 bn_shift, bn_part, &stats_done, act_alpha));
    if (rc) { yolo2_set_error("%s: workspace memset failed", fn); return YOLO2_E_LAUNCH; }
    Y2_CHECK_LAUNCH();
    if (bn_part && !stats_done)
        return y2_colsum_into(O, ldo, (long)B * H * W, Nf, bn_shift, bn_part, dtype, (hipStream_t)stream, &g_last_stat_rows);
    return YOLO2_OK;
}

extern "C" size_t yolo2_conv2d_workspace_bytes(int B, int H, int W, int Cp, int Nf, int ksize, int dtype) {
    if (!(B > 0 && H > 0 && W > 0 && Cp > 0 && Nf > 0) || !(dtype == YOLO2_F32 || dtype == YOLO2_BF16)) return 0;
    const Tune &tu = tune();
    const size_t M = (size_t)B * H * W;
    const int vec = dtype == YOLO2_BF16 ? 8 : 4;
    size_t need = (size_t)tu.cus * 256 * 128 * sizeof(float);
    const long tiles = (long)cdiv((long)M, 128) * cdiv(Nf, 128);
    if (choose_ksplit((int)(tiles > (1 << 30) ? (1 << 30) : tiles), ksize * ksize * cdiv(Cp, 4 * vec), tu.target_blocks) > 1 && M * Nf * sizeof(float) > need)
        need = M * Nf * sizeof(float);
    return need;
}

extern "C" int yolo2_debug_last_conv_plan(int *out8) {
    if (!out8) return YOLO2_E_ARG;
    for (int i = 0; i < 8; ++i) out8[i] = g_last_plan[i];
    return YOLO2_OK;
}

extern "C" int yolo2_conv2d(const void *P, const void *F, const float *bias, void *O, int B, int H,
                            int W, int Cp, int ldp, int Nf, int ldo, int ksize, int dtype, void *stream) {
    return conv2d_impl(P, F, bias, O, nullptr, 0, B, H, W, Cp, ldp, Nf, ldo, ksize, dtype, stream, "yolo2_conv2d");
}

extern "C" int yolo2_conv2d_bn(const void *P, const void *F, void *O, float *ws, size_t ws_bytes, int B, int H, int W, int Cp, int ldp,
                               int Nf, int ldo, int ksize, const float *shift, float *bn_part, int dtype, void *stream) {
    if (!shift || !bn_part || ldo != Nf) {
        yolo2_set_error("yolo2_conv2d_bn: argument check failed: shift / bn_part NULL or ldo != Nf");
        return YOLO2_E_ARG;
    }
    return conv2d_impl(P, F, nullptr, O, ws, ws_bytes, B, H, W, Cp, ldp, Nf, ldo, ksize, dtype, stream, "yolo2_conv2d_bn", shift, bn_part);
}

extern "C" int yolo2_conv2d_dgrad_bn(const void *dY, const void *F, void *dX, float *ws, size_t ws_bytes, int B, int H, int W, int Cp, int ldp,
                                     int Nf, int ldo, int ksize, const void *Yprev, const float *mean, const float *var, const float *gamma,
                                     const float *beta, float *dgamma, float *dbeta, float *bn_part, double *red_ws, float eps, float alpha,
                                     int *pending, int dtype, void *stream) {
    if (!Yprev || !mean || !var || !gamma || !beta || !dgamma || !dbeta || !bn_part || !red_ws) {
        yolo2_set_error("yolo2_conv2d_dgrad_bn: argument check failed: a producer-layer pointer is NULL");
        return YOLO2_E_ARG;
    }
    const Y2BnBwd bz{Yprev, mean, var, gamma, beta, eps, alpha, 0};
    return conv2d_impl(dY, F, nullptr, dX, ws, ws_bytes, B, H, W, Cp, ldp, Nf, ldo, ksize, dtype, stream, "yolo2_conv2d_dgrad_bn", nullptr, bn_part, 1.0f,
                       &bz, dgamma, dbeta, red_ws, pending);
}
extern "C" int yolo2_bn_part_to_grads(float *bn_part, int C, float *dgamma, float *dbeta, void *stream) {
    if (!bn_part || !dgamma || !dbeta || C <= 0) { yolo2_set_error("yolo2_bn_part_to_grads: argument check failed"); return YOLO2_E_ARG; }
    return y2_bn_part_to_grads(bn_part, C, dgamma, dbeta, (hipStream_t)stream);
}

extern "C" int yolo2_conv2d_bias_leaky(const void *P, const void *F, const float *bias, void *O, float *ws, size_t ws_bytes, int B, int H, int W,
                                       int Cp, int ldp, int Nf, int ldo, int ksize, float alpha, int dtype, void *stream) {
    if (!bias) { yolo2_set_error("yolo2_conv2d_bias_leaky: bias is NULL"); return YOLO2_E_ARG; }
    return conv2d_impl(P, F, bias, O, ws, ws_bytes, B, H, W, Cp, ldp, Nf, ldo, ksize, dtype, stream, "yolo2_conv2d_bias_leaky", nullptr, nullptr, alpha);
}

extern "C" int yolo2_conv2d_ws(const void *P, const void *F, const float *bias, void *O, float *ws, size_t ws_bytes, int B,
                               int H, int W, int Cp, int ldp, int Nf, int ldo, int ksize, int dtype, void *stream) {
    return conv2d_impl(P, F, bias, O, ws, ws_bytes, B, H, W, Cp, ldp, Nf, ldo, ksize, dtype, stream, "yolo2_conv2d_ws");
}
```

yolo_tf_amd/csrc/conv_shared.h:

```cpp
#pragma once
#include "common.h"

#define Y2_OOB 0x80000000u

#define Y2_STREAM_FLAG_WORDS 1024
#define Y2_STREAM_FLAG_STRIDE (Y2_STREAM_FLAG_WORDS + 64)
#define Y2_SK_DEFAULT_WAIT_TICKS 200000000u
#if defined(__HIP_DEVICE_COMPILE__)
__device__ __forceinline__ void y2_sk_wait_and_clear(unsigned *flags, int p) {
    if (__hip_atomic_load(flags + p, __ATOMIC_RELAXED, __HIP_MEMORY_SCOPE_AGENT) == 0u) {
        const unsigned cfg = __hip_atomic_load(flags + Y2_STREAM_FLAG_WORDS + 1, __ATOMIC_RELAXED, __HIP_MEMORY_SCOPE_AGENT);
        const unsigned long long limit = cfg ? cfg : Y2_SK_DEFAULT_WAIT_TICKS, t0 = wall_clock64();
        while (__hip_atomic_load(flags + p, __ATOMIC_RELAXED, __HIP_MEMORY_SCOPE_AGENT) == 0u) {
            __builtin_amdgcn_s_sleep(8);
            if (wall_clock64() - t0 > limit) {
                __hip_atomic_fetch_add(flags + Y2_STREAM_FLAG_WORDS, 1u, __ATOMIC_RELAXED, __HIP_MEMORY_SCOPE_AGENT);
                break;
            }
        }
    }
    __hip_atomic_store(flags + p, 0u, __ATOMIC_RELAXED, __HIP_MEMORY_SCOPE_AGENT);
}
#else
__device__ inline void y2_sk_wait_and_clear(unsigned *, int) {}
#endif

struct Y2BnBwd {
    const void *Y;
    const float *mean, *var, *gamma, *beta;
    float eps, alpha;
    int stat_mask_inv;
};

template <typename T, int BM, int BN, int WGN, int NSTAGE, int CH, int NW> struct Y2IgemmPlan {
    static constexpr int VEC = 16 / (int)sizeof(T);
    static constexpr int ROWB = CH * 16;
    static constexpr int RPI = 64 / CH;
    static constexpr int WGM = NW / WGN;
    static constexpr int TM = BM / WGM / 32, TN = BN / WGN / 32;
    static constexpr int B_IT = (BN / RPI + NW - 1) / NW;
    static constexpr int STAGE = (BM + B_IT * NW * RPI) * ROWB, RING = NSTAGE * STAGE;
    static constexpr int WROWS = TM * 32, WROWB = TN * 32 * (int)sizeof(T), WSTRIDE = WROWB + 16, WCPR = WROWB / 16;
    static constexpr int IMAGES = NW * WROWS * WSTRIDE;
    static constexpr bool WIDE_FITS = IMAGES <= RING;
    static constexpr bool RED = WGM > 1 && IMAGES + NW * WCPR * 2 * VEC * 4 <= RING;
    static constexpr int STAT_ROWS_FWD = WGM, STAT_ROWS_BNBWD = RED ? 1 : WGM;
};
constexpr int Y2P_STAT_ROWS_FWD = 4, Y2P_STAT_ROWS_BNBWD = 1;
constexpr int Y2S_STAT_ROWS_FWD = 4, Y2S_STAT_ROWS_BNBWD = 4;
constexpr int D1_STAT_ROWS = 32;

int y2_conv3x3_pp_launch(const void *P, unsigned p_bytes, const void *F, unsigned f_bytes, const float *bias, void *O, float *ws, int H, int W, int Cp,
                         int ldp, int Nf, int ldo, int M, int NT, const float *bn_shift, float *bn_part, unsigned *sk_flags, float act_alpha,
                         const Y2BnBwd &bz, int k_rotate, int grid, int sched, int cv, hipStream_t st);

int y2_conv3x3_s4_launch(const void *P, unsigned p_bytes, const void *F, unsigned f_bytes, const float *bias, void *O, float *ws, int H, int W, int Cp,
                         int ldp, int Nf, int ldo, int M, int NT, const float *bn_shift, float *bn_part, unsigned *sk_flags, float act_alpha,
                         const Y2BnBwd &bz, int k_rotate, int grid, int abl, hipStream_t st);

struct Y2W3Plan { int variant, ks, qchunk, blocks, remap, direct, BC, BN, waves; };
Y2W3Plan y2_wgrad3_plan(int B, int H, int W, int Cin, int Cout, int cus, int force_variant);
int y2_wgrad3_launch(const Y2W3Plan &p, const void *X, const void *dY, float *dW, int B, int H, int W, int Cin, int ldx, int Cout, int ldy, hipStream_t st,
                     float *ws = nullptr);
__host__ __device__ inline long y2_wgrad_slot_stride(int taps, int Cin, int Cout) { return ((long)taps * Cin * Cout + 3) & ~3L; }
void y2_magic_u32(unsigned d, unsigned *m, unsigned *s);

bool y2_w32_shape(int Cin, int ldx, int Cout, int ldy, int ksize, int dtype);
int y2_w32_blocks(int B, int H, int W, int cus);
int y2_w32_wgrad(const void *X, const void *dY, float *dW, int B, int H, int W, int cus, int *blocks, hipStream_t st, float *ws = nullptr);

bool y2_c32_shape(int Cp, int ldp, int Nf, int ldo, int ksize, int dtype);
int y2_c32_fwd(const void *P, const void *F, void *O, int B, int H, int W, const float *bias, float alpha, const float *bn_shift, float *bn_part,
               int cus, int *rows, hipStream_t st);

bool y2_c64_shape(int Cp, int ldp, int Nf, int ldo, int ksize, int dtype);
int y2_c64_fwd(const void *P, const void *F, void *O, int B, int H, int W, int Nf, const float *bias, float alpha, const float *bn_shift, float *bn_part,
               int cus, int *rows, hipStream_t st);

bool y2_d1_shape(int Cp, int ldp, int Nf, int ldo, int ksize, int dtype, long M);
int y2_d1_dgrad_bn(const void *P, const void *F, void *O, long M, int Cp, int Nf, float *bn_part, const Y2BnBwd &bz, int cus, int *rows, hipStream_t st);
```

yolo_tf_amd/engine.py:

```python
import numpy as np
import os

import torch

from . import ops, _lib
from .graph import pad8

BN_EPS = 1e-5
BN_DECAY = 0.999
LEAKY_ALPHA = 0.1

_DTYPES = {'bf16': torch.bfloat16, 'bfloat16': torch.bfloat16, 'f32': torch.float32, 'float32': torch.float32}


BN_PART_ROWS = 256
ARENA_ALIGN = 64


def layout_params(graph):
    offsets, off = {}, 0
    for v in reversed(graph.trainable()):
        offsets[v.name] = (off, v.size)
        off += (v.size + ARENA_ALIGN - 1) // ARENA_ALIGN * ARENA_ALIGN
    return offsets, off


def layer_end_offsets(graph, offsets):
    ends = {}
    for op in graph.ops:
        if op['kind'] == 'conv':
            names = [op['weights'].name] + [op[k].name for k in ('gamma', 'beta', 'biases') if k in op]
            ends[op['name']] = max(offsets[n][0] + (offsets[n][1] + ARENA_ALIGN - 1) // ARENA_ALIGN * ARENA_ALIGN for n in names)
    return ends


_SKEW_KB = 20
_skew_counter = [0]


def staggered(n, dtype, device, fill=0.0):
    esz = torch.empty(0, dtype=dtype).element_size()
    if _SKEW_KB <= 0 or n * esz < (1 << 20):
        return torch.full((n,), fill, dtype=dtype, device=device) if fill else torch.zeros(n, dtype=dtype, device=device)
    k = _skew_counter[0] = _skew_counter[0] + 1
    skew = (k % 16) * _SKEW_KB * 1024 // esz
    base = torch.full((n + 16 * _SKEW_KB * 1024 // esz,), fill, dtype=dtype, device=device) if fill else torch.zeros(n + 16 * _SKEW_KB * 1024 // esz, dtype=dtype, device=device)
    return base[skew:skew + n]


class _PartPool(object):

    def __init__(self, n, floats, device):
        self.bufs = [torch.zeros(floats, dtype=torch.float32, device=device) for _ in range(n)]
        self.dirty = [0] * n
        self.busy = [False] * n

    def acquire(self, floats):
        for i, (d, b) in enumerate(zip(self.dirty, self.busy)):
            if d == 0 and not b:
                break
        else:
            i = next(j for j, b in enumerate(self.busy) if not b)
            self.bufs[i][:self.dirty[i]].zero_()
        self.dirty[i] = int(floats)
        self.busy[i] = True
        return i

    def consumed(self, i, cleared=False):
        self.busy[i] = False
        if cleared:
            self.dirty[i] = 0

    def take_to_zero(self, exclude):
        for i, (d, b) in enumerate(zip(self.dirty, self.busy)):
            if i != exclude and d and not b:
                self.dirty[i] = 0
                return self.bufs[i], d
        return None, 0


class Engine(object):
    def __init__(self, graph, batch_size, dtype='bf16', training=True, seed=0, device=None, sync_bn=False, side_priority=-1, deterministic=False):
        self.deterministic = bool(deterministic) and training
        if self.deterministic and any(op.get('l2') or (op['kind'] == 'conv' and not op['bn'] and op['act']) for op in graph.ops):
            raise NotImplementedError('deterministic=True covers the YOLOv2 family: the YOLO (v1) fully connected head is not audited')
        if not torch.cuda.is_available():
            raise RuntimeError('yolo_tf_amd.Engine needs an MI355X (no CPU path exists)')
        ops._lib.load()
        self.side_priority = side_priority
        self.sync_bn = bool(sync_bn) and training
        self.bn_group, self.bn_world = None, 1
        self.graph = graph
        self.B = int(batch_size)
        self.dtype = _DTYPES[dtype] if isinstance(dtype, str) else dtype
        self.training = training
        self.device = torch.device(device if device is not None else 'cuda:%d' % torch.cuda.current_device())
        self._alloc_variables()
        self._alloc_activations()
        self.init_variables(seed)
        self._filters_dirty = True
        self._zero_ranges = None
        self.reg_loss = torch.zeros(1, dtype=torch.float64, device=self.device)
        self._has_l2 = any(op.get('l2') for op in graph.ops)
        self.dropout_masks = None
        self.dropout_seed = int(seed) + 1
        self.dropout_rank = 0
        self.dropout_step = 0
        self._dropout_calls = 0
        self._masks = {}
        self._phase = 'fwd'
        self.kernel_timer = None

    def _alloc_variables(self):
        g = self.graph
        other = [v for v in g.variables.values() if not v.trainable]
        self.param_offsets, off = layout_params(g)
        self.n_params = off
        self.params = staggered(off, torch.float32, self.device)
        self.grads = staggered(off, torch.float32, self.device) if self.training else None
        self.state_offsets = {}
        off = 0
        for v in other:
            self.state_offsets[v.name] = (off, v.size)
            off += (v.size + 3) // 4 * 4
        self.state = torch.zeros(max(off, 4), dtype=torch.float32, device=self.device)
        self.state_snap = torch.zeros_like(self.state)
        self.svar = {}
        self.var = {}
        self.gvar = {}
        for name, (o, n) in self.param_offsets.items():
            self.var[name] = self.params[o:o + n]
            if self.training:
                self.gvar[name] = self.grads[o:o + n]
        for name, (o, n) in self.state_offsets.items():
            self.var[name] = self.state[o:o + n]
            self.svar[name] = self.state_snap[o:o + n]
        segs = sorted(self.param_offsets.values())
        self.seg_off = torch.tensor([s[0] for s in segs] + [self.n_params], dtype=torch.int64, device=self.device)
        self.n_seg = len(segs)

    def init_variables(self, seed=0):
        rng = np.random.RandomState(seed)
        for v in self.graph.variables.values():
            self.var[v.name].copy_(torch.from_numpy(v.init(rng, v.shape).reshape(-1)))
        self._filters_dirty = True

    def get_variables(self):
        torch.cuda.synchronize()
        return {v.name: self.var[v.name].cpu().numpy().reshape(v.shape) for v in self.graph.variables.values()}

    def set_variables(self, values, strict=True):
        for v in self.graph.variables.values():
            if v.name in values:
                a = np.asarray(values[v.name], np.float32)
                assert a.shape == v.shape, (v.name, a.shape, v.shape)
                self.var[v.name].copy_(torch.from_numpy(np.ascontiguousarray(a).reshape(-1)))
            elif strict:
                raise KeyError(v.name)
        self._filters_dirty = True

    def get_gradients(self):
        torch.cuda.synchronize()
        return {v.name: self.gvar[v.name].cpu().numpy().reshape(v.shape) for v in self.graph.trainable()}

    def _alloc_activations(self):
        B, T, dev = self.B, self.dtype, self.device
        self._roots, self._groots = {}, {}
        for t in self.graph.tensors:
            if t.base is None:
                self._roots[t.name] = staggered(B * t.h * t.w * t.ld, T, dev)
                if self.training and t not in self.graph.inputs.values():
                    self._groots[t.name] = staggered(B * t.h * t.w * t.ld, T, dev)
        self.conv = {}
        max_y = 0
        max_c = 8
        for op in self.graph.ops:
            if op['kind'] != 'conv':
                continue
            k, cin, cout = op['ksize'], op['cin'], op['cout']
            cp, ldy = pad8(cin), pad8(cout)
            st = {'Ffwd': staggered(cout * k * k * cp, T, dev)}
            if self.training and op['x'] not in self.graph.inputs.values():
                st['Fdgr'] = staggered(cin * k * k * ldy, T, dev)
            if op['bn']:
                st['mean'] = torch.zeros(cout, dtype=torch.float32, device=dev)
                st['var'] = torch.ones(cout, dtype=torch.float32, device=dev)
            self.conv[op['name']] = st
            max_y = max(max_y, B * op['out'].h * op['out'].w * ldy)
            max_c = max(max_c, ldy)
        self._bindings = {}
        self._tmp_roots = {}
        self.fold_finalize = os.environ.get('YOLO2_FOLD_FINALIZE', '1') != '0' and not self.sync_bn
        self.pool_ymax = self.fold_finalize
        self._bind(self.graph)
        self.fold_bn = os.environ.get('YOLO2_FOLD_BN', '1') != '0'
        self.fuse_bn_stats = os.environ.get('YOLO2_FUSE_BN_STATS', '1') != '0' and not self.deterministic
        self.parts = _PartPool(3, 2 * 256 * max(max_c, 8), dev)
        self.bn_part = self.parts.bufs[0]
        self.fuse_first = os.environ.get('YOLO2_FUSE_FIRST', 'infer')
        self.fuse_first_wgrad = os.environ.get('YOLO2_FUSE_FIRST_WGRAD', '1') != '0' and not self.deterministic
        if self.deterministic and self.training:
            self.fuse_first = 'infer'
        self._bz_pending = {}
        self._fin_rows_limit = {}
        conv_bytes = 0
        for op in self.graph.ops:
            if op['kind'] == 'conv':
                x = op['x']
                for cp, nf in ((pad8(op['cin']), op['cout']), (pad8(op['cout']), op['cin'])):
                    conv_bytes = max(conv_bytes, ops.workspace_bytes('conv2d', B, x.h, x.w, cp, nf, op['ksize'], ops.dtype_code(T)))
        self.conv_ws = torch.zeros(conv_bytes // 4 + 1024, dtype=torch.float32, device=dev)
        ws_bytes = max(ops.workspace_bytes('bn', max_c), ops.workspace_bytes('bias_grad', max_c)) + ops.workspace_bytes('image_prep', B)
        self.ws = torch.zeros(ws_bytes // 8 + 64, dtype=torch.float64, device=dev)
        if self.training:
            self.dy_ring = [staggered(max_y, T, dev) for _ in range(3)]
            self.dy_free = [None, None, None]
            prio = int(os.environ.get('YOLO2_SIDE_PRIORITY', str(self.side_priority)))
            lo, hi = torch.cuda.Stream.priority_range()
            self.side_stream = torch.cuda.Stream(device=dev, priority=max(min(prio, max(lo, hi)), min(lo, hi)))
            self.overlap_wgrad = os.environ.get('YOLO2_OVERLAP_WGRAD', '1') != '0'
            self.overlap_max_m = 1 << 40
            self.wgrad_ws = None
            if self.deterministic:
                self._alloc_wgrad_ws(self.graph)
        self.img = None

    def _bind(self, graph):
        B, T, dev = self.B, self.dtype, self.device
        act, gact = {}, {}
        for t in graph.tensors:
            r, off, ld = t.storage()
            root = self._roots[r.name]
            assert B * r.h * r.w * r.ld <= root.numel(), 'input size exceeds the one the engine was allocated for (%s)' % r.name
            act[t] = (root[off:], ld)
            if r.name in self._groots:
                gact[t] = (self._groots[r.name][off:], ld)
        fused_pool, fwd_pool = {}, {}
        if os.environ.get('YOLO2_FUSE_POOL', '1') != '0':
            uses = {}
            for op in graph.ops:
                for t in (op.get('inputs') or [op['x']]):
                    uses[t] = uses.get(t, 0) + 1
            producers = {op['out']: op for op in graph.ops if op['kind'] == 'conv'}
            for op in graph.ops:
                x = op.get('x')
                if (op['kind'] == 'pool' and op['stride'] == 2 and x in producers and producers[x]['bn'] and uses.get(x, 0) == 1
                        and x.h % 2 == 0 and x.w % 2 == 0 and act[x][1] == x.c and act[op['out']][1] == op['out'].c
                        and act[producers[x]['y']][1] == x.c and x.c // (8 if T == torch.bfloat16 else 4) <= 256):
                    fused_pool[x] = op
                    st = self.conv[producers[x]['name']]
                    need = B * (x.h // 2) * (x.w // 2) * x.c
                    if self.training and ('pool_idx' not in st or st['pool_idx'].numel() < need):
                        st['pool_idx'] = torch.zeros(need, dtype=torch.uint8, device=dev)
                    if self.training and self.pool_ymax and ('pool_ymax' not in st or st['pool_ymax'].numel() < need):
                        st['pool_ymax'] = staggered(need, T, dev)
            for op in graph.ops:
                x = op.get('x')
                if (self.training and op['kind'] == 'pool' and op['stride'] == 2 and x in producers and producers[x]['bn'] and x not in fused_pool
                        and uses.get(x, 0) > 1 and x.h % 2 == 0 and x.w % 2 == 0 and act[x][1] == x.c and act[op['out']][1] == op['out'].c
                        and act[producers[x]['y']][1] == x.c and x.c // (8 if T == torch.bfloat16 else 4) <= 256
                        ):
                    fwd_pool[x] = op
        bn_bwd_fused = {}
        if self.training and os.environ.get('YOLO2_FUSE_BN_BWD', '1') != '0' and not self.deterministic:
            uses = {}
            for op in graph.ops:
                for t in (op.get('inputs') or [op['x']]):
                    uses[t] = uses.get(t, 0) + 1
            producers = {op['out']: op for op in graph.ops if op['kind'] == 'conv'}
            for op in graph.ops:
                x = op.get('x')
                if (op['kind'] == 'conv' and x in producers and producers[x]['bn'] and 'fold_bias' not in self.conv[producers[x]['name']]
                        and uses.get(x, 0) == 1 and x not in fused_pool and x in gact and gact[x][1] == x.c and act[producers[x]['y']][1] == x.c
                        and ops.conv2d_dgrad_bn_fuses(self.B, x.h, x.w, op['cin'], op['ksize'], self.dtype)):
                    bn_bwd_fused[op['name']] = producers[x]
        inp = next(iter(graph.inputs.values()))
        self._bindings[(inp.h, inp.w)] = {'graph': graph, 'act': act, 'gact': gact, 'fused_pool': fused_pool, 'zero_ranges': None, 'tmp_grad': {},
                                          'bn_bwd_fused': bn_bwd_fused, 'fwd_pool': fwd_pool}
        self._use(inp.h, inp.w)

    def _use(self, h, w):
        bnd = self._bindings[(h, w)]
        self._cur = bnd
        self.graph, self.act, self.gact, self.fused_pool = bnd['graph'], bnd['act'], bnd['gact'], bnd['fused_pool']
        self._zero_ranges, self.tmp_grad = bnd['zero_ranges'], bnd['tmp_grad']
        self.bn_bwd_fused, self.fwd_pool = bnd['bn_bwd_fused'], bnd['fwd_pool']

    def add_size(self, graph):
        names = [v.name for v in graph.variables.values()]
        assert names == [v.name for v in self._bindings[next(iter(self._bindings))]['graph'].variables.values()], 'different network'
        cur = self._cur
        self._bind(graph)
        if self.deterministic:
            self._alloc_wgrad_ws(graph)
        self._cur = cur
        self._use(*[k for k, v in self._bindings.items() if v is cur][0])

    def _alloc_wgrad_ws(self, graph):
        need = 0
        for op in graph.ops:
            if op['kind'] == 'conv':
                x = op['x']
                r, off, ldx = x.storage()
                need = max(need, ops.conv2d_wgrad_workspace_bytes(self.B, x.h, x.w, op['cin'], ldx, op['cout'], pad8(op['cout']), op['ksize'], self.dtype))
        if self.wgrad_ws is None or self.wgrad_ws.numel() * 4 < need:
            self.wgrad_ws = torch.empty(need // 4 + 4, dtype=torch.float32, device=self.device)

    def _wgrad(self, xb, dy, dW, B, h, w, cin, ldx, cout, ldy, k):
        if self.deterministic:
            stream = torch.cuda.current_stream().cuda_stream
            if self._wgrad_stream is None:
                self._wgrad_stream = stream
            assert stream == self._wgrad_stream, 'deterministic mode: filter gradients of one backward sweep on two streams share one workspace'
            ops.conv2d_wgrad_ws(xb, dy, dW, self.wgrad_ws, B, h, w, cin, ldx, cout, ldy, k)
        else:
            ops.conv2d_wgrad(xb, dy, dW, B, h, w, cin, ldx, cout, ldy, k)

    def set_size(self, height, width):
        if (height, width) not in self._bindings:
            raise KeyError('input size %dx%d was not bound (Engine.add_size)' % (height, width))
        self._use(height, width)

    def _conv(self, P, F, bias, O, H, W, Cp, ldp, Nf, ldo, k, real_k, bn_shift=None, bn_bwd=None):
        t = self.kernel_timer if Nf > 64 else None
        if t is not None:
            t.start(2.0 * self.B * H * W * Nf * real_k, self._phase if k == 3 else '1x1')
        pending = False
        part = None
        if bn_shift is not None:
            part = self.parts.acquire(2 * 256 * Nf)
            ops.conv2d_bn(P, F, O, self.conv_ws, self.B, H, W, Cp, ldp, Nf, ldo, k, bn_shift, self.parts.bufs[part])
        elif bn_bwd is not None:
            y, mean, var, gamma, beta, dgam, dbet = bn_bwd
            part = self.parts.acquire(2 * 256 * Nf)
            pending = ops.conv2d_dgrad_bn(P, F, O, self.conv_ws, self.B, H, W, Cp, ldp, Nf, ldo, k, y, mean, var, gamma, beta, dgam, dbet,
                                          self.parts.bufs[part], self.ws, BN_EPS, LEAKY_ALPHA)
        else:
            ops.conv2d_ws(P, F, bias, O, self.conv_ws, self.B, H, W, Cp, ldp, Nf, ldo, k)
        if t is not None:
            t.stop()
        if bn_bwd is not None:
            if not pending:
                self.parts.dirty[part] = 0
                self.parts.consumed(part)
                return None
            rows = ops.last_bn_part_rows()
            if self.fold_finalize and ops.bn_fin_supported(rows, Nf, self.dtype):
                return part, rows
            ops.bn_part_to_grads(self.parts.bufs[part], Nf, bn_bwd[5], bn_bwd[6])
            self.parts.consumed(part, cleared=True)
            return None
        if bn_shift is not None:
            return part, ops.last_bn_part_rows()
        return None

    def _prepare_filters(self):
        if not self._filters_dirty:
            return
        self._filter_descs()
        for op in self.graph.ops:
            if op['kind'] == 'conv' and 'fold_w' in self.conv[op['name']]:
                st = self.conv[op['name']]
                ops.bn_fold(self.var[op['weights'].name], self.var[op['gamma'].name], self.var[op['beta'].name], self.var[op['moving_mean'].name],
                            self.var[op['moving_variance'].name], st['fold_w'], st['fold_bias'], op['ksize'] ** 2 * op['cin'], op['cout'], BN_EPS)
        ops.filter_prep_batch(self._fdesc, self._fdesc_n, self._fdesc_blocks, self.dtype)
        self._filters_dirty = False

    def _filter_descs(self):
        if getattr(self, '_fdesc', None) is not None:
            return
        from ._lib import FilterDesc
        convs = [op for op in self.graph.ops if op['kind'] == 'conv']
        arr = (FilterDesc * len(convs))()
        first = 0
        for d, op in zip(arr, convs):
            st = self.conv[op['name']]
            k, ldcin, ldcout = op['ksize'], pad8(op['cin']), pad8(op['cout'])
            if self._folds(op):
                st['fold_w'] = torch.empty_like(self.var[op['weights'].name])
                st['fold_bias'] = torch.empty(op['cout'], dtype=torch.float32, device=self.device)
            d.W = (st['fold_w'] if 'fold_w' in st else self.var[op['weights'].name]).data_ptr()
            d.Ffwd = st['Ffwd'].data_ptr()
            d.Fdgr = st['Fdgr'].data_ptr() if 'Fdgr' in st else None
            d.ksize, d.cin, d.ldcin, d.cout, d.ldcout, d.first_block = k, op['cin'], ldcin, op['cout'], ldcout, first
            first += ops.filter_prep_blocks(k, ldcin, ldcout)
        raw = bytes(arr)
        self._fdesc = torch.frombuffer(bytearray(raw), dtype=torch.uint8).to(self.device)
        self._fdesc_n, self._fdesc_blocks = len(convs), first
        import ctypes
        self._fdesc1_info = {}
        size = ctypes.sizeof(FilterDesc)
        bounds = [d.first_block for d in arr] + [first]
        for i, (d, op) in enumerate(zip(arr, convs)):
            self._fdesc1_info[op['name']] = (i * size, bounds[i + 1] - bounds[i])
            d.first_block = 0
        self._fdesc1 = torch.frombuffer(bytearray(bytes(arr)), dtype=torch.uint8).to(self.device)
        covered = sorted(self.param_offsets[op['weights'].name] for op in self.graph.ops if op['kind'] == 'conv')
        small = sorted(v for k, v in self.param_offsets.items() if v not in covered)
        flat = [x for o, n in small for x in (o, n)]
        self._small = torch.tensor(flat if flat else [0, 0], dtype=torch.int64, device=self.device)
        self._n_small = len(small)

    def adam_update_and_prepare(self, m, v, alpha, beta1, beta2, eps, gscale):
        self._filter_descs()
        ops.adam_filter_prep(self._fdesc, self._fdesc_n, self._fdesc_blocks, self._small, self._n_small, self.params, self.grads, m, v,
                             alpha, beta1, beta2, eps, gscale, self.dtype)
        self._filters_dirty = False

    def adam_update_layer(self, op, m, v, alpha, beta1, beta2, eps, gscale):
        self._filter_descs()
        off, blocks = self._fdesc1_info[op['name']]
        ops.adam_filter_prep(self._fdesc1[off:], 1, blocks, self._small, 0, self.params, self.grads, m, v, alpha, beta1, beta2, eps, gscale, self.dtype)

    def adam_update_small(self, m, v, alpha, beta1, beta2, eps, gscale):
        self._filter_descs()
        ops.adam_filter_prep(self._fdesc, 0, 0, self._small, self._n_small, self.params, self.grads, m, v, alpha, beta1, beta2, eps, gscale, self.dtype)
        self._filters_dirty = False

    def _folds(self, op):
        return (not self.training and self.fold_bn and op['bn'] and op['out'] not in self.fused_pool
                and op['x'] not in self.graph.inputs.values())

    def set_images(self, images, mode=0):
        (inp,) = self.graph.inputs.values()
        assert images.dtype == torch.float32 and images.is_cuda and images.numel() == self.B * inp.h * inp.w * 3
        self.img = images.contiguous()
        ops.image_prep(self.img, self.act[inp][0], self.ws, self.B, inp.h * inp.w, mode)

    def _plan_grad_zeroing(self):
        if False:
            return [(0, self.n_params)]
        if self.deterministic:
            return []
        ranges = []
        for op in self.graph.ops:
            if op['kind'] != 'conv':
                continue
            x, out = op['x'], op['out']
            ldx, ldy = self.act[x][1], pad8(op['cout'])
            if ops.conv2d_wgrad_accumulates(self.B, x.h, x.w, op['cin'], ldx, op['cout'], ldy, op['ksize'], self.dtype):
                off, size = self.param_offsets[op['weights'].name]
                ranges.append((off, off + (size + 3) // 4 * 4))
        ranges.sort()
        merged = []
        for a, b in ranges:
            if merged and a <= merged[-1][1]:
                merged[-1] = (merged[-1][0], max(merged[-1][1], b))
            else:
                merged.append((a, b))
        out = []
        for a, b in merged:
            if out and a - out[-1][1] <= (1 << 20):
                out[-1] = (out[-1][0], b)
            else:
                out.append((a, b))
        return out

    def zero_grads(self):
        if self._zero_ranges is None:
            self._zero_ranges = self._cur['zero_ranges'] = self._plan_grad_zeroing()
        if self._zero_ranges:
            ops.zero_ranges(self.grads, self._zero_ranges)

    def forward(self):
        with ops.deterministic_launches(self.deterministic):
            self._forward()

    def _forward(self):
        self._prepare_filters()
        B = self.B
        if self.training:
            self.state_snap.copy_(self.state)
        pooled = set()
        for op in self.graph.ops:
            kind = op['kind']
            if kind == 'conv':
                x, out = op['x'], op['out']
                xb, ldx = self.act[x]
                st = self.conv[op['name']]
                M = B * out.h * out.w
                if op['bn'] and 'fold_bias' in st:
                    ob, ldo = self.act[out]
                    ops.conv2d_bias_leaky(xb, st['Ffwd'], st['fold_bias'], ob, self.conv_ws, B, x.h, x.w, pad8(x.c), ldx, op['cout'], ldo, op['ksize'], LEAKY_ALPHA)
                elif op['bn'] and self._first_fused(op):
                    gamma, beta = self.var[op['gamma'].name], self.var[op['beta'].name]
                    mmean, mvar = self.var[op['moving_mean'].name], self.var[op['moving_variance'].name]
                    pool = self.fused_pool[out]
                    pb, ldp = self.act[pool['out']]
                    if self.training:
                        part = self.parts.acquire(2 * 256 * 32)
                        shift = self.svar[op['moving_mean'].name]
                        ops.first_layer_stats(xb, st['Ffwd'], B, x.h, x.w, shift, self.parts.bufs[part])
                        ops.bn_finalize(self.parts.bufs[part], shift, M, 32, st['mean'], st['var'], mmean, mvar, BN_DECAY)
                        self.parts.consumed(part, cleared=True)
                        mean, var = st['mean'], st['var']
                    else:
                        mean, var = mmean, mvar
                    ops.first_layer_bn_leaky_pool(xb, st['Ffwd'], mean, var, gamma, beta, pb, st.get('pool_idx') if self.training else None,
                                                  B, x.h, x.w, ldp, BN_EPS, LEAKY_ALPHA)
                elif op['bn']:
                    yb, ldy = self.act[op['y']]
                    gamma, beta = self.var[op['gamma'].name], self.var[op['beta'].name]
                    mmean, mvar = self.var[op['moving_mean'].name], self.var[op['moving_variance'].name]
                    fused = self.training and self.fuse_bn_stats and ldy == op['cout']
                    shift = self.svar[op['moving_mean'].name]
                    produced = self._conv(xb, st['Ffwd'], None, yb, x.h, x.w, pad8(x.c), ldx, op['cout'], ldy, op['ksize'], op['ksize'] ** 2 * op['cin'],
                                          bn_shift=shift if fused else None)
                    fin = None
                    if fused:
                        part, rows = produced
                        if self.fold_finalize and ops.bn_fin_supported(rows, op['cout'], self.dtype):
                            fin = (part, rows)
                        else:
                            if self.sync_bn and self.bn_world > 1:
                                self._sync_bn_sums(self.parts.bufs[part], op['cout'])
                            ops.bn_finalize(self.parts.bufs[part], shift, M * (self.bn_world if self.sync_bn else 1), op['cout'], st['mean'], st['var'],
                                            mmean, mvar, BN_DECAY)
                            self.parts.consumed(part, cleared=True)
                        mean, var = st['mean'], st['var']
                    elif self.training:
                        assert not (self.sync_bn and self.bn_world > 1), 'sync_bn needs the statistics from the convolution epilogue (YOLO2_FUSE_BN_STATS=1, dense output)'
                        ops.bn_stats_ema(yb, st['mean'], st['var'], mmean, mvar, BN_DECAY, self.ws, M, op['cout'])
                        mean, var = st['mean'], st['var']
                    else:
                        mean, var = mmean, mvar
                    pool = self.fused_pool.get(out)
                    if fin is not None:
                        part, rows = fin
                        zbuf, zn = self.parts.take_to_zero(part)
                        if pool is not None:
                            pb, ldp = self.act[pool['out']]
                            ops.bn_leaky_pool_fin(yb, self.parts.bufs[part], rows, shift, mean, var, mmean, mvar, BN_DECAY, gamma, beta, pb, st.get('pool_idx'),
                                                  B, out.h, out.w, op['cout'], ldp, BN_EPS, LEAKY_ALPHA, zbuf, zn, ymax=st.get('pool_ymax'))
                            st['ymax_valid'] = 'pool_ymax' in st
                        elif out in self.fwd_pool:
                            pb, ldp = self.act[self.fwd_pool[out]['out']]
                            ops.bn_leaky_pool_fin(yb, self.parts.bufs[part], rows, shift, mean, var, mmean, mvar, BN_DECAY, gamma, beta, pb, None,
                                                  B, out.h, out.w, op['cout'], ldp, BN_EPS, LEAKY_ALPHA, zbuf, zn, a_full=self.act[out][0])
                            pooled.add(self.fwd_pool[out]['name'])
                        else:
                            ob, ldo = self.act[out]
                            ops.bn_leaky_fin(yb, self.parts.bufs[part], rows, shift, mean, var, mmean, mvar, BN_DECAY, gamma, beta, ob, M, op['cout'], ldo,
                                             BN_EPS, LEAKY_ALPHA, zbuf, zn)
                        self.parts.consumed(part)
                    elif pool is not None:
                        pb, ldp = self.act[pool['out']]
                        ops.bn_leaky_pool(yb, mean, var, gamma, beta, pb, st.get('pool_idx'), B, out.h, out.w, op['cout'], ldp, BN_EPS, LEAKY_ALPHA)
                        st['ymax_valid'] = False
                    else:
                        ob, ldo = self.act[out]
                        ops.bn_leaky(yb, mean, var, gamma, beta, ob, M, op['cout'], ldo, BN_EPS, LEAKY_ALPHA)
                elif op['act']:
                    ob, ldo = self.act[out]
                    ops.conv2d_bias_leaky(xb, st['Ffwd'], self.var[op['biases'].name], ob, self.conv_ws, B, x.h, x.w, pad8(x.c), ldx, op['cout'], ldo, op['ksize'], LEAKY_ALPHA)
                else:
                    ob, ldo = self.act[out]
                    self._conv(xb, st['Ffwd'], self.var[op['biases'].name], ob, x.h, x.w, pad8(x.c), ldx, op['cout'], ldo, op['ksize'], op['ksize'] ** 2 * op['cin'])
            elif kind == 'flatten':
                pass
            elif kind == 'dropout':
                x, out = op['x'], op['out']
                n = B * x.h * x.w * self.act[x][1]
                mask = self._dropout_mask(op, n)
                fixed = self.dropout_masks is not None
                self._dropout_calls += 1
                ops.dropout(self.act[x][0], self.act[out][0], mask, n, op['keep_prob'], 0 if fixed else self._dropout_seed_for(op))
            elif kind == 'pool':
                x, out = op['x'], op['out']
                if x in self.fused_pool or op['name'] in pooled:
                    continue
                assert self.act[x][1] == x.c and self.act[out][1] == out.c
                ops.maxpool_fwd(self.act[x][0], self.act[out][0], B, x.h, x.w, x.c, op['stride'])
            elif kind == 'reorg':
                x, out = op['x'], op['out']
                assert self.act[x][1] == x.c
                ops.reorg(self.act[x][0], self.act[out][0], B, x.h, x.w, x.c, self.act[out][1])
            elif kind == 'concat':
                pass
            else:
                raise ValueError(kind)

    def _grad_sink(self, t, written):
        gb, ld = self.gact[t]
        if t not in written:
            written.add(t)
            return gb, ld, None
        tmp = self.tmp_grad.get(t)
        if tmp is None:
            n = self.B * t.h * t.w * ld
            root = self._tmp_roots.get(t.name)
            if root is None or root.numel() < n:
                root = self._tmp_roots[t.name] = torch.zeros(n, dtype=self.dtype, device=self.device)
            tmp = self.tmp_grad[t] = root
        n = self.B * t.h * t.w * ld
        return tmp, ld, (lambda: ops.add_inplace(gb, tmp, n))

    def backward(self, on_layer_done=None):
        with ops.deterministic_launches(self.deterministic):
            self._backward(on_layer_done)

    def _backward(self, on_layer_done=None):
        B = self.B
        self._wgrad_stream = None
        written = set()
        reduced = set()
        inputs = set(self.graph.inputs.values())
        self._phase = 'dgrad'
        if self._has_l2:
            self.reg_loss.zero_()
        main = torch.cuda.current_stream()
        side = self.side_stream if self.overlap_wgrad else None
        slot = 0
        for op in reversed(self.graph.ops):
            kind = op['kind']
            if kind == 'conv':
                x, out = op['x'], op['out']
                st = self.conv[op['name']]
                M = B * out.h * out.w
                cout, k = op['cout'], op['ksize']
                ldy = pad8(cout)
                wgrad_done = False
                gob, ldgo = self.gact[out]
                xb, ldx = self.act[x]
                if op['bn']:
                    yb, _ = self.act[op['y']]
                    gamma, beta = self.var[op['gamma'].name], self.var[op['beta'].name]
                    dgam, dbet = self.gvar[op['gamma'].name], self.gvar[op['beta'].name]
                    pool = self.fused_pool.get(out)
                    pfin = None
                    limit = self._fin_limit(cout) if self.fold_finalize else 0
                    first = self._first_fused(op)
                    if first:
                        dpb, lddp = self.gact[pool['out']]
                        part = self.parts.acquire(2 * 256 * 32)
                        ops.first_layer_pool_bwd_reduce(xb, st['Ffwd'], dpb, lddp, st['pool_idx'], st['mean'], st['var'], gamma, beta, self.parts.bufs[part],
                                                        B, x.h, x.w, BN_EPS, LEAKY_ALPHA)
                        ops.bn_part_to_grads(self.parts.bufs[part], 32, dgam, dbet)
                        self.parts.consumed(part, cleared=True)
                    elif pool is not None:
                        dpb, lddp = self.gact[pool['out']]
                        if limit >= 64 and st.get('ymax_valid'):
                            rows = ops.bn_leaky_bwd_reduce_part(dpb, lddp, st['pool_ymax'], st['mean'], st['var'], gamma, beta, self.ws, limit,
                                                                M // 4, cout, BN_EPS, LEAKY_ALPHA)
                            pfin = (self.ws, rows, rows * cout)
                        elif limit >= 128:
                            rows = ops.bn_leaky_pool_bwd_reduce_part(dpb, lddp, st['pool_idx'], yb, st['mean'], st['var'], gamma, beta, self.ws, limit,
                                                                     B, out.h, out.w, cout, BN_EPS, LEAKY_ALPHA)
                            pfin = (self.ws, rows, rows * cout)
                        else:
                            ops.bn_leaky_pool_bwd_reduce(dpb, lddp, st['pool_idx'], yb, st['mean'], st['var'], gamma, beta, dgam, dbet, self.ws,
                                                         B, out.h, out.w, cout, BN_EPS, LEAKY_ALPHA)
                    elif op['name'] in reduced:
                        pend = self._bz_pending.pop(op['name'], None)
                        if pend is not None:
                            pfin = (self.parts.bufs[pend[0]], pend[1], 256 * cout, pend[0])
                    elif limit >= 64:
                        rows = ops.bn_leaky_bwd_reduce_part(gob, ldgo, yb, st['mean'], st['var'], gamma, beta, self.ws, limit, M, cout, BN_EPS, LEAKY_ALPHA)
                        pfin = (self.ws, rows, rows * cout)
                    else:
                        ops.bn_leaky_bwd_reduce(gob, ldgo, yb, st['mean'], st['var'], gamma, beta, dgam, dbet, self.ws, M, cout, BN_EPS, LEAKY_ALPHA)
                    slot = (slot + 1) % 3
                    dy = self.dy_ring[slot]
                    if self.dy_free[slot] is not None:
                        main.wait_event(self.dy_free[slot])
                    if first:
                        ops.first_layer_pool_bwd_apply(xb, st['Ffwd'], dpb, lddp, st['pool_idx'], st['mean'], st['var'], gamma, beta, dgam, dbet, dy,
                                                       B, x.h, x.w, BN_EPS, LEAKY_ALPHA)
                    elif pfin is not None:
                        own = pfin[3] if len(pfin) > 3 else -1
                        zbuf, zn = self.parts.take_to_zero(own)
                        if pool is not None and self._first_wgrad_fused(op, lddp):
                            ops.first_layer_wgrad_bn(xb, yb, dpb, lddp, st['pool_idx'], st['mean'], st['var'], gamma, beta, pfin[0], pfin[1], pfin[2],
                                                     dgam, dbet, self.gvar[op['weights'].name], B, x.h, x.w, op['cin'], BN_EPS, LEAKY_ALPHA, zbuf, zn)
                            self._l2(op)
                            wgrad_done = True
                        elif pool is not None:
                            ops.bn_leaky_pool_bwd_apply_fin(dpb, lddp, st['pool_idx'], yb, st['mean'], st['var'], gamma, beta, pfin[0], pfin[1], pfin[2],
                                                            dgam, dbet, dy, B, out.h, out.w, cout, BN_EPS, LEAKY_ALPHA, zbuf, zn)
                        else:
                            ops.bn_leaky_bwd_apply_fin(gob, ldgo, yb, st['mean'], st['var'], gamma, beta, pfin[0], pfin[1], pfin[2], dgam, dbet, dy,
                                                       M, cout, BN_EPS, LEAKY_ALPHA, zbuf, zn)
                        if own >= 0:
                            self.parts.consumed(own)
                    elif pool is not None:
                        ag, ab = self._sync_bn_grads(dgam, dbet, cout)
                        ops.bn_leaky_pool_bwd_apply(dpb, lddp, st['pool_idx'], yb, st['mean'], st['var'], gamma, beta, ag, ab, dy,
                                                    B, out.h, out.w, cout, BN_EPS, LEAKY_ALPHA)
                    else:
                        ag, ab = self._sync_bn_grads(dgam, dbet, cout)
                        ops.bn_leaky_bwd_apply(gob, ldgo, yb, st['mean'], st['var'], gamma, beta, ag, ab, dy, M, cout, BN_EPS, LEAKY_ALPHA)
                    ring = True
                elif op['act']:
                    assert ldgo == ldy and self.act[out][1] == ldy
                    slot = (slot + 1) % 3
                    dy = self.dy_ring[slot]
                    if self.dy_free[slot] is not None:
                        main.wait_event(self.dy_free[slot])
                    ops.leaky_bwd(self.act[out][0], gob, dy, M * ldy, LEAKY_ALPHA)
                    ops.bias_grad(dy, ldy, self.gvar[op['biases'].name], self.ws, M, cout)
                    ring = True
                else:
                    dy = gob
                    assert ldgo == ldy
                    ops.bias_grad(dy, ldy, self.gvar[op['biases'].name], self.ws, M, cout)
                    ring = False
                done = None
                if wgrad_done:
                    pass
                elif side is not None and M <= self.overlap_max_m:
                    ready = torch.cuda.Event()
                    ready.record(main)
                    side.wait_event(ready)
                    with torch.cuda.stream(side):
                        self._wgrad(xb, dy, self.gvar[op['weights'].name], B, x.h, x.w, op['cin'], ldx, cout, ldy, k)
                        self._l2(op)
                        done = torch.cuda.Event()
                        done.record(side)
                    if ring:
                        self.dy_free[slot] = done
                else:
                    self._wgrad(xb, dy, self.gvar[op['weights'].name], B, x.h, x.w, op['cin'], ldx, cout, ldy, k)
                    self._l2(op)
                if x not in inputs:
                    prod = self.bn_bwd_fused.get(op['name'])
                    dst, ldd, fin = self._grad_sink(x, written)
                    if prod is not None and fin is None:
                        pst = self.conv[prod['name']]
                        pend = self._conv(dy, st['Fdgr'], None, dst, x.h, x.w, ldy, ldy, op['cin'], ldd, k, k * k * cout,
                                          bn_bwd=(self.act[prod['y']][0], pst['mean'], pst['var'], self.var[prod['gamma'].name], self.var[prod['beta'].name],
                                                  self.gvar[prod['gamma'].name], self.gvar[prod['beta'].name]))
                        reduced.add(prod['name'])
                        if pend is not None:
                            self._bz_pending[prod['name']] = pend
                    else:
                        self._conv(dy, st['Fdgr'], None, dst, x.h, x.w, ldy, ldy, op['cin'], ldd, k, k * k * cout)
                    if fin:
                        fin()
                if on_layer_done is not None:
                    on_layer_done(op, done)
            elif kind == 'pool':
                x, out = op['x'], op['out']
                if x in self.fused_pool:
                    continue
                if x in written and op['stride'] == 2 and self.gact[x][1] == x.c:
                    ops.maxpool_bwd_acc(self.act[x][0], self.gact[out][0], self.gact[x][0], B, x.h, x.w, x.c)
                    continue
                dst, ldd, fin = self._grad_sink(x, written)
                assert ldd == x.c
                ops.maxpool_bwd(self.act[x][0], self.gact[out][0], dst, B, x.h, x.w, x.c, op['stride'])
                if fin:
                    fin()
            elif kind == 'reorg':
                x, out = op['x'], op['out']
                dst, ldd, fin = self._grad_sink(x, written)
                assert ldd == x.c
                ops.reorg_bwd(self.gact[out][0], self.gact[out][1], dst, B, x.h, x.w, x.c)
                if fin:
                    fin()
            elif kind == 'concat':
                for v in op['inputs']:
                    written.add(v)
            elif kind == 'flatten':
                written.add(op['x'])
            elif kind == 'dropout':
                x, out = op['x'], op['out']
                dst, ldd, fin = self._grad_sink(x, written)
                n = B * x.h * x.w * ldd
                ops.dropout_bwd(self.gact[out][0], self._dropout_mask(op, n), dst, n, op['keep_prob'])
                if fin:
                    fin()
        self._phase = 'fwd'
        if side is not None:
            main.wait_stream(side)

    def _sync_bn_sums(self, part, C):
        import torch.distributed as dist
        sums = self._bn_sync_buf(2 * C)
        ops.bn_part_to_grads(part, C, sums[:C], sums[C:])
        dist.all_reduce(sums, group=self.bn_group)
        part[:C].copy_(sums[:C])
        part[BN_PART_ROWS * C:BN_PART_ROWS * C + C].copy_(sums[C:])

    def _sync_bn_grads(self, dgam, dbet, C):
        if not (self.sync_bn and self.bn_world > 1):
            return dgam, dbet
        import torch.distributed as dist
        sums = self._bn_sync_buf(2 * C)
        sums[:C].copy_(dgam)
        sums[C:].copy_(dbet)
        dist.all_reduce(sums, group=self.bn_group)
        sums.mul_(1.0 / self.bn_world)
        return sums[:C], sums[C:]

    def _bn_sync_buf(self, n):
        buf = getattr(self, '_bn_sync', None)
        if buf is None or buf.numel() < n:
            buf = self._bn_sync = torch.zeros(max(n, 4096), dtype=torch.float32, device=self.device)
        return buf[:n]

    def _first_fused(self, op):
        if self.fuse_first == '0' or (self.training and self.fuse_first != '1'):
            return False
        x, out = op['x'], op['out']
        return (op['bn'] and x in self.graph.inputs.values() and op['ksize'] == 3 and op['cin'] == 3 and self.act[x][1] == 8 and op['cout'] == 32
                and out in self.fused_pool and self.act[self.fused_pool[out]['out']][1] >= 32 and x.h % 2 == 0 and x.w % 2 == 0
                and (not self.training or self.fuse_bn_stats))

    def _first_wgrad_fused(self, op, lddp):
        x, out = op['x'], op['out']
        return (self.fuse_first_wgrad and op['bn'] and x in self.graph.inputs.values() and op['ksize'] == 3 and op['cin'] <= 8 and self.act[x][1] == 8
                and op['cout'] == 32 and out in self.fused_pool and lddp >= 32 and lddp % 8 == 0 and x.h % 2 == 0 and x.w % 2 == 0
                and 'yolo2_first_layer_wgrad_bn' not in _lib.MISSING)

    def _fin_limit(self, C):
        v = self._fin_rows_limit.get(C)
        if v is None:
            v = self._fin_rows_limit[C] = ops.bn_fin_rows_limit(C, self.dtype)
        return v

    def _l2(self, op):
        if op.get('l2', 0.0) > 0.0:
            w = self.var[op['weights'].name]
            ops.l2_regularizer(w, self.gvar[op['weights'].name], w.numel(), op['l2'], self.reg_loss)

    def _dropout_seed_for(self, op):
        idx = [o['name'] for o in self.graph.ops if o['kind'] == 'dropout'].index(op['name'])
        h = (self.dropout_seed * 0x9E3779B97F4A7C15 + self.dropout_rank * 0xC2B2AE3D27D4EB4F + self.dropout_step * 0x165667B19E3779F9 + idx * 0xD6E8FEB86659FD93)
        h &= (1 << 64) - 1
        h ^= h >> 31
        return (h % ((1 << 62) - 1)) + 1

    def _dropout_mask(self, op, n):
        if self.dropout_masks is not None:
            return self.dropout_masks[op['name']]
        m = self._masks.get(op['name'])
        if m is None or m.numel() < n:
            m = self._masks[op['name']] = torch.zeros(n, dtype=torch.uint8, device=self.device)
        return m

    def output(self):
        return self.graph.ops[-1]['out']

    def summarizable_tensors(self):
        assert self.training, 'the summaries describe a training step'
        skipped = set()
        for op in self.graph.ops:
            if op['kind'] == 'conv' and op['bn']:
                if op['out'] in self.fused_pool:
                    skipped.add(op['out'])
                if self._first_fused(op):
                    skipped.add(op['y'])
        out = []
        for t in self.graph.tensors:
            if t.flat_of is not None:
                continue
            if t in skipped:
                out.append((t, None))
            else:
                buf, ld = self.act[t]
                out.append((t, (buf, self.B * t.h * t.w, t.c, ld)))
        return out
```

yolo_tf_amd/ops.py:

```python
import ctypes

import numpy as np
import torch

from . import _lib
from ._lib import call, ptr, dtype_code


_raw_stream = getattr(torch._C, '_cuda_getCurrentRawStream', None)
_raw_device = getattr(torch._C, '_cuda_getDevice', None)


def _stream():
    if _raw_stream is None or _raw_device is None:
        return ctypes.c_void_p(torch.cuda.current_stream().cuda_stream)
    return ctypes.c_void_p(_raw_stream(_raw_device()))


def pad8(c):
    return (c + 7) // 8 * 8


def conv2d(P, F, bias, O, B, H, W, Cp, ldp, Nf, ldo, ksize):
    call('yolo2_conv2d', ptr(P), ptr(F), ptr(bias), ptr(O), B, H, W, Cp, ldp, Nf, ldo, ksize, dtype_code(P.dtype), _stream())


def conv2d_ws(P, F, bias, O, ws, B, H, W, Cp, ldp, Nf, ldo, ksize):
    call('yolo2_conv2d_ws', ptr(P), ptr(F), ptr(bias), ptr(O), ptr(ws), ws.numel() * ws.element_size(), B, H, W, Cp, ldp, Nf, ldo, ksize,
         dtype_code(P.dtype), _stream())


def conv2d_bias_leaky(P, F, bias, O, ws, B, H, W, Cp, ldp, Nf, ldo, ksize, alpha):
    call('yolo2_conv2d_bias_leaky', ptr(P), ptr(F), ptr(bias), ptr(O), ptr(ws), ws.numel() * ws.element_size(), B, H, W, Cp, ldp, Nf, ldo, ksize,
         alpha, dtype_code(P.dtype), _stream())


def conv2d_bn(P, F, O, ws, B, H, W, Cp, ldp, Nf, ldo, ksize, shift, bn_part):
    call('yolo2_conv2d_bn', ptr(P), ptr(F), ptr(O), ptr(ws), ws.numel() * ws.element_size(), B, H, W, Cp, ldp, Nf, ldo, ksize,
         ptr(shift), ptr(bn_part), dtype_code(P.dtype), _stream())


def conv2d_dgrad_bn(dY, F, dX, ws, B, H, W, Cp, ldp, Nf, ldo, ksize, Yprev, mean, var, gamma, beta, dgamma, dbeta, bn_part, red_ws, eps, alpha):
    pending = ctypes.c_int(0)
    call('yolo2_conv2d_dgrad_bn', ptr(dY), ptr(F), ptr(dX), ptr(ws), ws.numel() * ws.element_size(), B, H, W, Cp, ldp, Nf, ldo, ksize,
         ptr(Yprev), ptr(mean), ptr(var), ptr(gamma), ptr(beta), ptr(dgamma), ptr(dbeta), ptr(bn_part), ptr(red_ws), eps, alpha,
         ctypes.byref(pending), dtype_code(dY.dtype), _stream())
    return bool(pending.value)


def conv2d_dgrad_bn_fuses(B, H, W, Nf, ksize, dtype):
    lib = _lib.load()
    if 'yolo2_conv2d_dgrad_bn_fuses' in _lib.MISSING:
        return True
    return bool(lib.yolo2_conv2d_dgrad_bn_fuses(B, H, W, Nf, ksize, dtype_code(dtype)))


def filter_prep_blocks(ksize, ldcin, ldcout):
    lib = _lib.load()
    if 'yolo2_filter_prep_blocks' in _lib.MISSING:
        return ksize * ksize * ((ldcin + 63) // 64) * ((ldcout + 63) // 64)
    return int(lib.yolo2_filter_prep_blocks(ksize, ldcin, ldcout))


def bn_part_to_grads(bn_part, C, dgamma, dbeta):
    call('yolo2_bn_part_to_grads', ptr(bn_part), C, ptr(dgamma), ptr(dbeta), _stream())


def bn_finalize(bn_part, shift, M, C, mean, var, mm, mv, decay):
    call('yolo2_bn_finalize', ptr(bn_part), ptr(shift), M, C, ptr(mean), ptr(var), ptr(mm), ptr(mv), decay, _stream())


def conv2d_wgrad_accumulates(B, H, W, Cin, ldx, Cout, ldy, ksize, dtype):
    return bool(_lib.load().yolo2_conv2d_wgrad_accumulates(B, H, W, Cin, ldx, Cout, ldy, ksize, dtype_code(dtype)))


def conv2d_wgrad(X, dY, dW, B, H, W, Cin, ldx, Cout, ldy, ksize):
    call('yolo2_conv2d_wgrad', ptr(X), ptr(dY), ptr(dW), B, H, W, Cin, ldx, Cout, ldy, ksize, dtype_code(X.dtype), _stream())


def conv2d_wgrad_workspace_bytes(B, H, W, Cin, ldx, Cout, ldy, ksize, dtype):
    return int(_lib.query('yolo2_conv2d_wgrad_workspace_bytes', B, H, W, Cin, ldx, Cout, ldy, ksize, dtype_code(dtype)))


def conv2d_wgrad_ws(X, dY, dW, ws, B, H, W, Cin, ldx, Cout, ldy, ksize):
    call('yolo2_conv2d_wgrad_ws', ptr(X), ptr(dY), ptr(dW), ptr(ws), 0 if ws is None else ws.numel() * ws.element_size(), B, H, W, Cin, ldx, Cout, ldy,
         ksize, dtype_code(X.dtype), _stream())


def wgrad_ws_plan(B, H, W, Cin, ldx, Cout, ldy, ksize, dtype, cus):
    out = (ctypes.c_int * 4)()
    rc = _lib.load().yolo2_debug_wgrad_ws_plan(B, H, W, Cin, ldx, Cout, ldy, ksize, dtype_code(dtype), cus, out)
    if rc != 0:
        raise _lib.HipKernelError('yolo2_debug_wgrad_ws_plan failed (code %d)' % rc)
    return dict(zip(('family', 'slots', 'slot_floats', 'blocks'), list(out)))


def set_deterministic(on):
    call('yolo2_set_deterministic', 1 if on else 0)


class deterministic_launches(object):

    def __init__(self, on):
        self.on = bool(on)
        self.prev = 0

    def __enter__(self):
        if self.on:
            self.prev = int(_lib.query('yolo2_get_deterministic'))
            if not self.prev:
                set_deterministic(True)

    def __exit__(self, *exc):
        if self.on and not self.prev:
            set_deterministic(False)
        return False


def filter_prep(Wt, Ffwd, Fdgr, ksize, Cin, ldcin, Cout, ldcout, dtype):
    call('yolo2_filter_prep', ptr(Wt), ptr(Ffwd), ptr(Fdgr), ksize, Cin, ldcin, Cout, ldcout, dtype_code(dtype), _stream())


def filter_prep_batch(descs_dev, n, total_blocks, dtype):
    call('yolo2_filter_prep_batch', ptr(descs_dev), n, total_blocks, dtype_code(dtype), _stream())


def adam_filter_prep(descs_dev, n, total_blocks, small_dev, n_small, params, grads, m, v, alpha, b1, b2, eps, gscale, dtype):
    call('yolo2_adam_filter_prep', ptr(descs_dev), n, total_blocks, ptr(small_dev), n_small, ptr(params), ptr(grads), ptr(m), ptr(v), alpha, b1, b2, eps, gscale,
         dtype_code(dtype), _stream())


def bn_stats(Y, mean, var, ws, M, C):
    call('yolo2_bn_stats', ptr(Y), ptr(mean), ptr(var), ptr(ws), M, C, dtype_code(Y.dtype), _stream())


def bn_stats_ema(Y, mean, var, mm, mv, decay, ws, M, C):
    call('yolo2_bn_stats_ema', ptr(Y), ptr(mean), ptr(var), ptr(mm), ptr(mv), decay, ptr(ws), M, C, dtype_code(Y.dtype), _stream())


def bn_ema(mm, mv, mean, var, C, decay):
    call('yolo2_bn_ema', ptr(mm), ptr(mv), ptr(mean), ptr(var), C, decay, _stream())


def bn_leaky(Y, mean, var, gamma, beta, A, M, C, lda, eps, alpha):
    call('yolo2_bn_leaky', ptr(Y), ptr(mean), ptr(var), ptr(gamma), ptr(beta), ptr(A), M, C, lda, eps, alpha, dtype_code(Y.dtype), _stream())


def bn_leaky_bwd_reduce(dA, ldda, Y, mean, var, gamma, beta, dgamma, dbeta, ws, M, C, eps, alpha):
    call('yolo2_bn_leaky_bwd_reduce', ptr(dA), ldda, ptr(Y), ptr(mean), ptr(var), ptr(gamma), ptr(beta), ptr(dgamma), ptr(dbeta), ptr(ws),
         M, C, eps, alpha, dtype_code(Y.dtype), _stream())


def bn_leaky_bwd_apply(dA, ldda, Y, mean, var, gamma, beta, dgamma, dbeta, dY, M, C, eps, alpha):
    call('yolo2_bn_leaky_bwd_apply', ptr(dA), ldda, ptr(Y), ptr(mean), ptr(var), ptr(gamma), ptr(beta), ptr(dgamma), ptr(dbeta), ptr(dY),
         M, C, eps, alpha, dtype_code(Y.dtype), _stream())


def last_bn_part_rows():
    return int(_lib.load().yolo2_last_bn_part_rows())


def bn_fin_supported(rows, C, dtype):
    return bool(_lib.load().yolo2_bn_fin_supported(int(rows), int(C), dtype_code(dtype)))


def bn_fin_rows_limit(C, dtype, cap=1024):
    r = cap
    while r >= 1 and not bn_fin_supported(r, C, dtype):
        r //= 2
    return r


def _zero_args(zero, zero_floats):
    return (ptr(zero) if zero_floats else None), int(zero_floats)


def bn_leaky_fin(Y, bn_part, rows, shift, mean, var, mm, mv, decay, gamma, beta, A, M, C, lda, eps, alpha, zero=None, zero_floats=0):
    z, zn = _zero_args(zero, zero_floats)
    call('yolo2_bn_leaky_fin', ptr(Y), ptr(bn_part), rows, ptr(shift), ptr(mean), ptr(var), ptr(mm), ptr(mv), decay, ptr(gamma), ptr(beta), ptr(A),
         M, C, lda, eps, alpha, z, zn, dtype_code(Y.dtype), _stream())


def bn_leaky_pool_fin(Y, bn_part, rows, shift, mean, var, mm, mv, decay, gamma, beta, P, idx, B, H, W, C, ldp, eps, alpha, zero=None, zero_floats=0, ymax=None, a_full=None):
    z, zn = _zero_args(zero, zero_floats)
    call('yolo2_bn_leaky_pool_fin', ptr(Y), ptr(bn_part), rows, ptr(shift), ptr(mean), ptr(var), ptr(mm), ptr(mv), decay, ptr(gamma), ptr(beta),
         ptr(P), ptr(idx), ptr(ymax), ptr(a_full), B, H, W, C, ldp, eps, alpha, z, zn, dtype_code(Y.dtype), _stream())


def bn_leaky_bwd_apply_fin(dA, ldda, Y, mean, var, gamma, beta, part, rows, plane_stride, dgamma, dbeta, dY, M, C, eps, alpha, zero=None, zero_floats=0):
    z, zn = _zero_args(zero, zero_floats)
    call('yolo2_bn_leaky_bwd_apply_fin', ptr(dA), ldda, ptr(Y), ptr(mean), ptr(var), ptr(gamma), ptr(beta), ptr(part), rows, plane_stride,
         ptr(dgamma), ptr(dbeta), ptr(dY), M, C, eps, alpha, z, zn, dtype_code(Y.dtype), _stream())


def bn_leaky_pool_bwd_apply_fin(dP, lddp, idx, Y, mean, var, gamma, beta, part, rows, plane_stride, dgamma, dbeta, dY, B, H, W, C, eps, alpha,
                                zero=None, zero_floats=0):
    z, zn = _zero_args(zero, zero_floats)
    call('yolo2_bn_leaky_pool_bwd_apply_fin', ptr(dP), lddp, ptr(idx), ptr(Y), ptr(mean), ptr(var), ptr(gamma), ptr(beta), ptr(part), rows, plane_stride,
         ptr(dgamma), ptr(dbeta), ptr(dY), B, H, W, C, eps, alpha, z, zn, dtype_code(Y.dtype), _stream())


def first_layer_wgrad_bn(X, Y, dP, lddp, idx, mean, var, gamma, beta, part, rows, plane_stride, dgamma, dbeta, dW, B, H, W, Cin, eps, alpha,
                         zero=None, zero_floats=0):
    z, zn = _zero_args(zero, zero_floats)
    call('yolo2_first_layer_wgrad_bn', ptr(X), ptr(Y), ptr(dP), lddp, ptr(idx), ptr(mean), ptr(var), ptr(gamma), ptr(beta), ptr(part), rows, plane_stride,
         ptr(dgamma), ptr(dbeta), ptr(dW), B, H, W, Cin, eps, alpha, z, zn, dtype_code(Y.dtype), _stream())


def bn_leaky_bwd_reduce_part(dA, ldda, Y, mean, var, gamma, beta, ws, rows_limit, M, C, eps, alpha):
    rows = ctypes.c_int(0)
    call('yolo2_bn_leaky_bwd_reduce_part', ptr(dA), ldda, ptr(Y), ptr(mean), ptr(var), ptr(gamma), ptr(beta), ptr(ws), ctypes.byref(rows), rows_limit, M, C,
         eps, alpha, dtype_code(Y.dtype), _stream())
    return rows.value


def bn_leaky_pool_bwd_reduce_part(dP, lddp, idx, Y, mean, var, gamma, beta, ws, rows_limit, B, H, W, C, eps, alpha):
    rows = ctypes.c_int(0)
    call('yolo2_bn_leaky_pool_bwd_reduce_part', ptr(dP), lddp, ptr(idx), ptr(Y), ptr(mean), ptr(var), ptr(gamma), ptr(beta), ptr(ws), ctypes.byref(rows),
         rows_limit, B, H, W, C, eps, alpha, dtype_code(Y.dtype), _stream())
    return rows.value


def bn_leaky_pool(Y, mean, var, gamma, beta, P, idx, B, H, W, C, ldp, eps, alpha):
    call('yolo2_bn_leaky_pool', ptr(Y), ptr(mean), ptr(var), ptr(gamma), ptr(beta), ptr(P), ptr(idx), B, H, W, C, ldp, eps, alpha,
         dtype_code(Y.dtype), _stream())


def bn_leaky_pool_bwd_reduce(dP, lddp, idx, Y, mean, var, gamma, beta, dgamma, dbeta, ws, B, H, W, C, eps, alpha):
    call('yolo2_bn_leaky_pool_bwd_reduce', ptr(dP), lddp, ptr(idx), ptr(Y), ptr(mean), ptr(var), ptr(gamma), ptr(beta), ptr(dgamma), ptr(dbeta),
         ptr(ws), B, H, W, C, eps, alpha, dtype_code(Y.dtype), _stream())


def bn_leaky_pool_bwd_apply(dP, lddp, idx, Y, mean, var, gamma, beta, dgamma, dbeta, dY, B, H, W, C, eps, alpha):
    call('yolo2_bn_leaky_pool_bwd_apply', ptr(dP), lddp, ptr(idx), ptr(Y), ptr(mean), ptr(var), ptr(gamma), ptr(beta), ptr(dgamma), ptr(dbeta),
         ptr(dY), B, H, W, C, eps, alpha, dtype_code(Y.dtype), _stream())


def maxpool_fwd(A, P, B, H, W, C, stride):
    call('yolo2_maxpool_fwd', ptr(A), ptr(P), B, H, W, C, stride, dtype_code(A.dtype), _stream())


def maxpool_bwd(A, dP, dA, B, H, W, C, stride):
    call('yolo2_maxpool_bwd', ptr(A), ptr(dP), ptr(dA), B, H, W, C, stride, dtype_code(A.dtype), _stream())


def maxpool_bwd_acc(A, dP, dA, B, H, W, C):
    call('yolo2_maxpool_bwd_acc', ptr(A), ptr(dP), ptr(dA), B, H, W, C, dtype_code(A.dtype), _stream())


def reorg(x, out, B, H, W, C, ldo):
    call('yolo2_reorg', ptr(x), ptr(out), B, H, W, C, ldo, dtype_code(x.dtype), _stream())


def reorg_bwd(dout, ldd, din, B, H, W, C):
    call('yolo2_reorg_bwd', ptr(dout), ldd, ptr(din), B, H, W, C, dtype_code(din.dtype), _stream())


def copy_channels(src, lds, dst, ldd, M, C):
    call('yolo2_copy_channels', ptr(src), lds, ptr(dst), ldd, M, C, dtype_code(src.dtype), _stream())


def add_inplace(dst, src, n):
    call('yolo2_add_inplace', ptr(dst), ptr(src), n, dtype_code(dst.dtype), _stream())


def bias_grad(dY, ld, dbias, ws, M, C):
    call('yolo2_bias_grad', ptr(dY), ld, ptr(dbias), ptr(ws), M, C, dtype_code(dY.dtype), _stream())


def image_prep(img, out, ws, B, HW, mode):
    call('yolo2_image_prep', ptr(img), ptr(out), ptr(ws), B, HW, mode, dtype_code(out.dtype), _stream())


def head_decode(logits, ld, anchors, conf, xy_min, xy_max, nan_flag, B, ch, cw, A, C):
    call('yolo2_head_decode', ptr(logits), ld, ptr(anchors), ptr(conf), ptr(xy_min), ptr(xy_max), ptr(nan_flag), B, ch, cw, A, C,
         dtype_code(logits.dtype), _stream())


def head_decode_attrs(logits, ld, anchors, iou, prob, xy, wh, B, ch, cw, A, C):
    call('yolo2_head_decode_attrs', ptr(logits), ld, ptr(anchors), ptr(iou), ptr(prob), ptr(xy), ptr(wh), B, ch, cw, A, C,
         dtype_code(logits.dtype), _stream())


def loss(logits, ld, anchors, labels, hparam, objectives, dlogits, ws, B, ch, cw, A, C):
    hp = (ctypes.c_float * 4)(*[float(v) for v in hparam])
    mask, prob, coords, omin, omax, areas = labels
    call('yolo2_loss', ptr(logits), ld, ptr(anchors), ptr(mask), ptr(prob), ptr(coords), ptr(omin), ptr(omax), ptr(areas), hp,
         ptr(objectives), ptr(dlogits), ptr(ws), B, ch, cw, A, C, dtype_code(logits.dtype), _stream())


def loss_partials(logits, ld, anchors, labels, hparam, dlogits, ws, B, ch, cw, A, C):
    hp = (ctypes.c_float * 4)(*[float(v) for v in hparam])
    mask, prob, coords, omin, omax, areas = labels
    call('yolo2_loss_partials', ptr(logits), ld, ptr(anchors), ptr(mask), ptr(prob), ptr(coords), ptr(omin), ptr(omax), ptr(areas), hp,
         ptr(dlogits), ptr(ws), B, ch, cw, A, C, dtype_code(logits.dtype), _stream())


def loss_objectives(ws, objectives, B, ch, cw, A):
    call('yolo2_loss_objectives', ptr(ws), ptr(objectives), B, ch, cw, A, _stream())


def loss_ws_floats(B, cells, A):
    return workspace_bytes('loss', B, cells, A) // 4


def nms(conf, xy_min, xy_max, order, ws, B, N, C, thr, thr_iou):
    call('yolo2_nms', ptr(conf), ptr(xy_min), ptr(xy_max), ptr(order), ptr(ws), B, N, C, thr, thr_iou, _stream())


def adam(w, g, m, v, n, alpha, b1, b2, eps, gscale=1.0):
    call('yolo2_adam', ptr(w), ptr(g), ptr(m), ptr(v), n, alpha, b1, b2, eps, gscale, _stream())


def momentum(w, g, acc, n, lr, mom, gscale=1.0):
    call('yolo2_momentum', ptr(w), ptr(g), ptr(acc), n, lr, mom, gscale, _stream())


def sgd(w, g, n, lr, gscale=1.0):
    call('yolo2_sgd', ptr(w), ptr(g), n, lr, gscale, _stream())


def rmsprop(w, g, ms, mom, n, lr, decay, momentum_, eps, gscale=1.0):
    call('yolo2_rmsprop', ptr(w), ptr(g), ptr(ms), ptr(mom), n, lr, decay, momentum_, eps, gscale, _stream())


def adagrad(w, g, acc, n, lr, gscale=1.0):
    call('yolo2_adagrad', ptr(w), ptr(g), ptr(acc), n, lr, gscale, _stream())


def adadelta(w, g, acc, accu, n, lr, rho, eps, gscale=1.0):
    call('yolo2_adadelta', ptr(w), ptr(g), ptr(acc), ptr(accu), n, lr, rho, eps, gscale, _stream())


def ftrl(w, g, accum, linear, n, lr, lr_power, l1, l2, gscale=1.0):
    call('yolo2_ftrl', ptr(w), ptr(g), ptr(accum), ptr(linear), n, lr, lr_power, l1, l2, gscale, _stream())


def scale(x, n, s):
    call('yolo2_scale', ptr(x), n, s, _stream())


def zero_ranges(x, ranges):
    flat = (ctypes.c_long * (2 * len(ranges)))(*[int(v) for ab in ranges for v in ab])
    call('yolo2_zero_ranges', ptr(x), flat, len(ranges), _stream())


def bn_fold(W, gamma, beta, mean, var, Wf, bias, rows, C, eps):
    call('yolo2_bn_fold', ptr(W), ptr(gamma), ptr(beta), ptr(mean), ptr(var), ptr(Wf), ptr(bias), rows, C, eps, _stream())


def workspace_bytes(kind, *args):
    return int(_lib.query('yolo2_%s_workspace_bytes' % kind, *args))


def clip_by_norm(g, seg_off, nseg, clip, ws):
    call('yolo2_clip_by_norm', ptr(g), ptr(seg_off), nseg, clip, ptr(ws), _stream())

# ... 358 lines not shown
```

Baseline: 4697 img/s.

## Fuse BN-leaky backward reduction into c64 data-gradient conv epilogue

Adds a BN-backward epilogue to the 64-channel conv kernels (narrow and wide) so the data-gradient conv also computes dgamma/dbeta partials from the previous layer's activations, including pooled producers that use pool_ymax. This removes a separate reduction pass that re-reads the gradient and activation tensors. The engine now routes more layers, including pool-fused ones, through the fused path. In exchange the epilogue adds extra loads, cross-lane shuffles and LDS reduction work, plus a new template variant and atomics.

```diff
diff --git a/include/yolo2_hip.h b/include/yolo2_hip.h
--- a/include/yolo2_hip.h
+++ b/include/yolo2_hip.h
@@ -79,6 +79,7 @@
                           const float *beta, float *dgamma, float *dbeta, float *bn_part, double *red_ws, float eps, float alpha,
                           int *pending, int dtype, void *stream);
 int yolo2_conv2d_dgrad_bn_fuses(int B, int H, int W, int Nf, int ksize, int dtype);
+int yolo2_conv2d_dgrad_bn_fuses_at(int B, int H, int W, int Cp, int ldp, int Nf, int ldo, int ksize, int dtype);
 int yolo2_bn_part_to_grads(float *bn_part, int C, float *dgamma, float *dbeta, void *stream);
 
 #define YOLO2_BN_PART_ROWS 256
diff --git a/yolo_tf_amd/_lib.py b/yolo_tf_amd/_lib.py
--- a/yolo_tf_amd/_lib.py
+++ b/yolo_tf_amd/_lib.py
@@ -118,6 +118,7 @@
     'yolo2_conv2d_wgrad_accumulates': (_i, [_i] * 9),
     'yolo2_filter_prep_blocks': (_i, [_i, _i, _i]),
     'yolo2_conv2d_dgrad_bn_fuses': (_i, [_i] * 6),
+    'yolo2_conv2d_dgrad_bn_fuses_at': (_i, [_i] * 9),
     'yolo2_debug_set_wgrad_variant': (None, [_i]),
     'yolo2_last_bn_part_rows': (_i, []),
     'yolo2_get_stream_workgroups': (_i, []),
diff --git a/yolo_tf_amd/csrc/conv_c64.hip b/yolo_tf_amd/csrc/conv_c64.hip
--- a/yolo_tf_amd/csrc/conv_c64.hip
+++ b/yolo_tf_amd/csrc/conv_c64.hip
@@ -1,5 +1,6 @@
 #include "common.h"
 #include "conv_shared.h"
+#include "bn_leaky.h"
 #include <atomic>
 
 #define C64_TP 256
@@ -20,10 +21,91 @@
     unsigned mP, sP, mH, sH;
 };
 
-template <int MODE, int NFG>
+#if defined(__HIP_DEVICE_COMPILE__)
+struct C64BnBwdLane {
+    float cmu, cinv, csc, cbt;
+    float ps[2][8];
+    u32x4 y[2];
+    __device__ __forceinline__ void load(const Y2BnBwd &bz, int c) {
+        cmu = bz.mean[c];
+        cinv = bn_inv_std(bz.var[c], bz.eps);
+        csc = cinv * bz.gamma[c];
+        cbt = bz.beta[c];
+#pragma unroll
+        for (int k = 0; k < 8; ++k) ps[0][k] = ps[1][k] = 0.f;
+    }
+    __device__ __forceinline__ void request(const __amdgpu_buffer_rsrc_t rsrcY, unsigned moff, int lane) {
+        const unsigned mo_even = (unsigned)__builtin_amdgcn_mov_dpp((int)moff, 0xA0, 0xF, 0xF, true);
+        const unsigned mo_odd = (unsigned)__builtin_amdgcn_mov_dpp((int)moff, 0xF5, 0xF, 0xF, true);
+        const unsigned lo16 = (lane & 1) ? 16u : 0u;
+        y[0] = __builtin_bit_cast(u32x4, __builtin_amdgcn_raw_buffer_load_b128(rsrcY, mo_even != 0xffffffffu ? mo_even + lo16 : Y2_OOB, 0, 0));
+        y[1] = __builtin_bit_cast(u32x4, __builtin_amdgcn_raw_buffer_load_b128(rsrcY, mo_odd != 0xffffffffu ? mo_odd + lo16 : Y2_OOB, 0, 0));
+    }
+    __device__ __forceinline__ void add(float alpha, int lane, const unsigned (&s0)[4], const unsigned (&s1)[4], bool live0, bool live1) {
+        const int src = (((lane >> 5) << 4) + ((lane & 1) << 3)) << 2;
+#pragma unroll
+        for (int k = 0; k < 8; ++k) {
+            const float mu = __builtin_bit_cast(float, __builtin_amdgcn_ds_bpermute(src + 4 * k, __builtin_bit_cast(int, cmu)));
+            const float inv = __builtin_bit_cast(float, __builtin_amdgcn_ds_bpermute(src + 4 * k, __builtin_bit_cast(int, cinv)));
+            const float sc = __builtin_bit_cast(float, __builtin_amdgcn_ds_bpermute(src + 4 * k, __builtin_bit_cast(int, csc)));
+            const float bt = __builtin_bit_cast(float, __builtin_amdgcn_ds_bpermute(src + 4 * k, __builtin_bit_cast(int, cbt)));
+#pragma unroll
+            for (int p = 0; p < 2; ++p) {
+                const unsigned dw = p ? s1[k >> 1] : s0[k >> 1], yw = y[p][k >> 1];
+                const float d = __builtin_bit_cast(float, (k & 1) ? (dw & 0xffff0000u) : (dw << 16));
+                const float yy = __builtin_bit_cast(float, (k & 1) ? (yw & 0xffff0000u) : (yw << 16));
+                const float xh = (yy - mu) * inv;
+                const float z = (yy - mu) * sc + bt;
+                float g = z >= 0.f ? d : alpha * d;
+                g = (p ? live1 : live0) ? g : 0.f;
+                ps[0][k] += g * xh;
+                ps[1][k] += g;
+            }
+        }
+    }
+    template <int NF> __device__ __forceinline__ void flush(unsigned char *smem, int tid, int wave, int lane, float *bn_part) {
+#pragma unroll
+        for (int pl = 0; pl < 2; ++pl)
+#pragma unroll
+            for (int k = 0; k < 8; ++k) {
+                float v = ps[pl][k];
+                v += __builtin_bit_cast(float, __builtin_amdgcn_mov_dpp(__builtin_bit_cast(int, v), 0x4E, 0xF, 0xF, true));
+                v += __builtin_bit_cast(float, __builtin_amdgcn_mov_dpp(__builtin_bit_cast(int, v), 0x124, 0xF, 0xF, true));
+                v += __builtin_bit_cast(float, __builtin_amdgcn_mov_dpp(__builtin_bit_cast(int, v), 0x128, 0xF, 0xF, true));
+                ps[pl][k] = y2_rows_pair_sum(v);
+            }
+        __syncthreads();
+        float *const red = reinterpret_cast<float *>(smem);
+        if ((lane & 31) < 2) {
+#pragma unroll
+            for (int pl = 0; pl < 2; ++pl)
+#pragma unroll
+                for (int k = 0; k < 8; ++k) red[(wave * 2 + pl) * 32 + ((lane >> 5) << 4) + ((lane & 1) << 3) + k] = ps[pl][k];
+        }
+        __syncthreads();
+        if (tid < 2 * NF) {
+            const int pl = tid / NF, ch = tid % NF;
+            float sum = 0.f;
+            if (NF == 32) {
+#pragma unroll
+                for (int w = 0; w < 8; ++w) sum += red[(w * 2 + pl) * 32 + ch];
+            } else {
+#pragma unroll
+                for (int j = 0; j < 4; ++j) sum += red[(((ch >> 5) + 2 * j) * 2 + pl) * 32 + (ch & 31)];
+            }
+            float *const dst = bn_part + (long)(pl * Y2_BN_PART_ROWS + (int)(blockIdx.x & (C64_STAT_ROWS - 1))) * NF + ch;
+            if (gridDim.x <= C64_STAT_ROWS) *dst = sum;
+            else unsafeAtomicAdd(dst, sum);
+        }
+    }
+};
+#endif
+
+template <int MODE, int NFG, bool BNB = false>
 __global__ __launch_bounds__(512) void conv_c64_fwd_kernel(
     const bf16 *__restrict__ X, unsigned x_bytes, const bf16 *__restrict__ F, bf16 *__restrict__ O, C64Geo g,
-    const float *__restrict__ vec, float *__restrict__ bn_part, float alpha) {
+    const float *__restrict__ vec, float *__restrict__ bn_part, float alpha, const Y2BnBwd bz) {
+    static_assert(!BNB || (MODE == 0 && NFG == 1), "the BN-backward epilogue belongs to the 32-filter data-gradient form");
     extern __shared__ __attribute__((aligned(1024))) unsigned char smem[];
     constexpr int NB = NFG == 4 ? 2 : 1;
     constexpr int NPASS = NFG == 4 ? 2 : 1;
@@ -110,6 +192,11 @@
     }
 
     const int T = (e0 - s0 + C64_TP - 1) / C64_TP;
+#if defined(__HIP_DEVICE_COMPILE__)
+    C64BnBwdLane bw;
+    const __amdgpu_buffer_rsrc_t rsrcY = __builtin_amdgcn_make_buffer_rsrc(const_cast<void *>(bz.Y), 0, BNB ? (unsigned)g.M * (unsigned)ROWB : 0u, 0x00020000);
+    if (BNB) bw.load(bz, l31);
+#endif
     int pslot = g.NP0;
     if (pslot >= NPR) pslot -= NPR;
     unsigned tro = 0;
@@ -127,6 +214,18 @@
         }
         pslot += 32;
         if (pslot >= NPR) pslot -= NPR;
+#if defined(__HIP_DEVICE_COMPILE__)
+        if (BNB) {
+            const unsigned q = (unsigned)(tb + pg * 32 + l31);
+            const unsigned R = c64_div(q, g.mP, g.sP);
+            const unsigned c = q - __umul24(R, P1);
+            const unsigned img = c64_div(R, g.mH, g.sH);
+            const unsigned r_ = R - __umul24(img, H1);
+            const bool live = (q < (unsigned)e0) & (c < (unsigned)W) & (r_ < (unsigned)H);
+            const unsigned m = __umul24(__umul24(img, (unsigned)H) + r_, (unsigned)W) + c;
+            bw.request(rsrcY, live ? m * (unsigned)ROWB + (unsigned)(half * 32) : 0xffffffffu, lane);
+        }
+#endif
 #pragma unroll 1
         for (int pa = 0; pa < NPASS; ++pa) {
             if (tb + pa * 128 >= e0) break;
@@ -218,6 +317,7 @@
                     *reinterpret_cast<u32x4 *>(reinterpret_cast<unsigned char *>(O) + mo_even + lo16) = u32x4{s0_[0], s0_[1], s0_[2], s0_[3]};
                 if (mo_odd != 0xffffffffu)
                     *reinterpret_cast<u32x4 *>(reinterpret_cast<unsigned char *>(O) + mo_odd + lo16) = u32x4{s1_[0], s1_[1], s1_[2], s1_[3]};
+                if (BNB) bw.add(bz.alpha, lane, s0_, s1_, mo_even != 0xffffffffu, mo_odd != 0xffffffffu);
             }
             __builtin_amdgcn_sched_barrier(0);
             if (MODE == 1 && bn_part) {
@@ -254,6 +354,9 @@
         tro += (unsigned)(C64_TP * 128);
         if (tro >= (unsigned)RRB) tro -= (unsigned)RRB;
     }
+#if defined(__HIP_DEVICE_COMPILE__)
+    if (BNB) bw.template flush<32>(smem, tid, wave, lane, bn_part);
+#endif
     if (MODE == 1 && bn_part) {
 #pragma unroll
         for (int o = 4; o <= 16; o <<= 1) {
@@ -274,7 +377,9 @@
 }
 
 #define C64W_TP 128
-__global__ __launch_bounds__(512) void conv_c64_wide_kernel(const bf16 *__restrict__ X, unsigned x_bytes, const bf16 *__restrict__ F, bf16 *__restrict__ O, C64Geo g) {
+template <bool BNB>
+__global__ __launch_bounds__(512) void conv_c64_wide_kernel(const bf16 *__restrict__ X, unsigned x_bytes, const bf16 *__restrict__ F, bf16 *__restrict__ O, C64Geo g,
+                                                            float *__restrict__ bn_part, const Y2BnBwd bz) {
     extern __shared__ __attribute__((aligned(1024))) unsigned char smem[];
     constexpr int TP = C64W_TP;
     const int H = g.H, W = g.W, Mp = g.Mp;
@@ -344,6 +449,11 @@
     }
 
     const int T = (e0 - s0 + TP - 1) / TP;
+#if defined(__HIP_DEVICE_COMPILE__)
+    C64BnBwdLane bw;
+    const __amdgpu_buffer_rsrc_t rsrcY = __builtin_amdgcn_make_buffer_rsrc(const_cast<void *>(bz.Y), 0, BNB ? (unsigned)g.M * 128u : 0u, 0x00020000);
+    if (BNB) bw.load(bz, 32 * fg + l31);
+#endif
     int pslot = g.NP0;
     if (pslot >= NPR) pslot -= NPR;
     unsigned tro = 0;
@@ -361,6 +471,18 @@
         }
         pslot += TP / 8;
         if (pslot >= NPR) pslot -= NPR;
+#if defined(__HIP_DEVICE_COMPILE__)
+        if (BNB) {
+            const unsigned q = (unsigned)(tb + pg * 64 + kh * 32 + l31);
+            const unsigned R = c64_div(q, g.mP, g.sP);
+            const unsigned c = q - __umul24(R, P1);
+            const unsigned img = c64_div(R, g.mH, g.sH);
+            const unsigned r_ = R - __umul24(img, H1);
+            const bool live = (q < (unsigned)e0) & (c < (unsigned)W) & (r_ < (unsigned)H);
+            const unsigned m = __umul24(__umul24(img, (unsigned)H) + r_, (unsigned)W) + c;
+            bw.request(rsrcY, live ? m * 128u + (unsigned)(fg * 64 + half * 32) : 0xffffffffu, lane);
+        }
+#endif
         f32x16 acc[2];
 #pragma unroll
         for (int i = 0; i < 2; ++i)
@@ -441,36 +563,51 @@
                 *reinterpret_cast<u32x4 *>(reinterpret_cast<unsigned char *>(O) + mo_even + lo16) = u32x4{s0_[0], s0_[1], s0_[2], s0_[3]};
             if (mo_odd != 0xffffffffu)
                 *reinterpret_cast<u32x4 *>(reinterpret_cast<unsigned char *>(O) + mo_odd + lo16) = u32x4{s1_[0], s1_[1], s1_[2], s1_[3]};
+            if (BNB) bw.add(bz.alpha, lane, s0_, s1_, mo_even != 0xffffffffu, mo_odd != 0xffffffffu);
         }
 #endif
         tro += (unsigned)(TP * 128);
         if (tro >= (unsigned)RRB) tro -= (unsigned)RRB;
     }
-}
-
-static int y2_c64_wide(const void *P, const void *F, void *O, int B, int H, int W, int cus, hipStream_t st) {
+#if defined(__HIP_DEVICE_COMPILE__)
+    if (BNB) bw.template flush<64>(smem, tid, wave, lane, bn_part);
+#endif
+}
+
+static bool y2_c64_wide_plan(int B, int H, int W, int cus, C64Geo &g, size_t &lds) {
     const long Mp = (long)B * (H + 1) * (W + 1);
-    if (Mp + 2 * C64W_TP >= (1L << 23) || H < 1 || W < 1 || cus < 1) return 1;
-    C64Geo g;
+    if (Mp + 2 * C64W_TP >= (1L << 23) || H < 1 || W < 1 || cus < 1) return false;
     g.H = H; g.W = W; g.M = B * H * W; g.Mp = (int)Mp;
     g.L = (int)(((Mp + cus - 1) / cus + C64W_TP - 1) / C64W_TP) * C64W_TP;
-    const int grid = (int)((Mp + g.L - 1) / g.L);
     g.HLa = (W + 2 + 7) & ~7;
     g.NP0 = (g.HLa + C64W_TP + W + 2 + 7) / 8;
     g.RR = (8 * g.NP0 + C64W_TP + 63) & ~63;
     g.shl_off = 0;
-    const size_t plane = (size_t)g.RR * 128, lds = 2 * plane + 8 * 4096;
-    if (lds > 160 * 1024 || (plane - (size_t)g.NP0 * 1024) + 8 * 4096 < 37 * 1024) return 1;
+    const size_t plane = (size_t)g.RR * 128;
+    lds = 2 * plane + 8 * 4096;
+    if (lds > 160 * 1024 || (plane - (size_t)g.NP0 * 1024) + 8 * 4096 < 37 * 1024) return false;
     y2_magic_u32((unsigned)(W + 1), &g.mP, &g.sP);
     y2_magic_u32((unsigned)(H + 1), &g.mH, &g.sH);
-    static std::atomic<size_t> lds_set[64];
+    return true;
+}
+static int y2_c64_wide(const void *P, const void *F, void *O, int B, int H, int W, int cus, float *bn_part, const Y2BnBwd *bz, int *rows, hipStream_t st) {
+    C64Geo g;
+    size_t lds = 0;
+    if (!y2_c64_wide_plan(B, H, W, cus, g, lds)) return 1;
+    const int grid = (int)(((long)g.Mp + g.L - 1) / g.L);
+    static std::atomic<size_t> lds_set[2][64];
     int dev = 0;
     if (hipGetDevice(&dev) != hipSuccess || dev < 0 || dev >= 64) dev = 0;
-    if (lds > lds_set[dev].load(std::memory_order_relaxed)) {
-        if (hipFuncSetAttribute((const void *)conv_c64_wide_kernel, hipFuncAttributeMaxDynamicSharedMemorySize, (int)lds) != hipSuccess) return 1;
-        lds_set[dev].store(lds, std::memory_order_relaxed);
-    }
-    conv_c64_wide_kernel<<<grid, 512, lds, st>>>((const bf16 *)P, (unsigned)((size_t)g.M * 128 * 2), (const bf16 *)F, (bf16 *)O, g);
+    const int slot = bz ? 1 : 0;
+    if (lds > lds_set[slot][dev].load(std::memory_order_relaxed)) {
+        const void *fn = bz ? (const void *)conv_c64_wide_kernel<true> : (const void *)conv_c64_wide_kernel<false>;
+        if (hipFuncSetAttribute(fn, hipFuncAttributeMaxDynamicSharedMemorySize, (int)lds) != hipSuccess) return 1;
+        lds_set[slot][dev].store(lds, std::memory_order_relaxed);
+    }
+    const unsigned x_bytes = (unsigned)((size_t)g.M * 128 * 2);
+    if (bz) conv_c64_wide_kernel<true><<<grid, 512, lds, st>>>((const bf16 *)P, x_bytes, (const bf16 *)F, (bf16 *)O, g, bn_part, *bz);
+    else conv_c64_wide_kernel<false><<<grid, 512, lds, st>>>((const bf16 *)P, x_bytes, (const bf16 *)F, (bf16 *)O, g, nullptr, Y2BnBwd{nullptr, nullptr, nullptr, nullptr, nullptr, 0.f, 0.f, 0});
+    if (rows) *rows = bz ? (grid < C64_STAT_ROWS ? grid : C64_STAT_ROWS) : 0;
     return 0;
 }
 
@@ -480,22 +617,12 @@
     return Cp == 64 && ldp == 64 && ((Nf == 128 && ldo == 128) || (Nf == 32 && ldo == 32));
 }
 
-int y2_c64_fwd(const void *P, const void *F, void *O, int B, int H, int W, int Nf, const float *bias, float alpha, const float *bn_shift, float *bn_part,
-               int cus, int *rows, hipStream_t st) {
-    if (Nf == 64) {
-        if (bn_part || bias || alpha != 1.0f) return 1;
-        if (rows) *rows = 0;
-        return y2_c64_wide(P, F, O, B, H, W, cus, st);
-    }
+static bool y2_c64_fwd_plan(int B, int H, int W, bool narrow, int cus, C64Geo &g, size_t &lds_out) {
     const long Mp = (long)B * (H + 1) * (W + 1);
-    if (Mp + 2 * C64_TP >= (1L << 23) || H < 1 || W < 1 || cus < 1) return 1;
-    const bool narrow = Nf == 32;
-    if (narrow && (bn_part || bias || alpha != 1.0f)) return 1;
-    C64Geo g;
+    if (Mp + 2 * C64_TP >= (1L << 23) || H < 1 || W < 1 || cus < 1) return false;
     g.H = H; g.W = W; g.M = B * H * W; g.Mp = (int)Mp;
     const int gran = narrow ? 256 : 128;
     g.L = (int)(((Mp + cus - 1) / cus + gran - 1) / gran) * gran;
-    const int grid = (int)((Mp + g.L - 1) / g.L);
     g.HLa = (W + 2 + 7) & ~7;
     g.NP0 = (g.HLa + C64_TP + W + 2 + 7) / 8;
     g.RR = (8 * g.NP0 + C64_TP + 63) & ~63;
@@ -504,25 +631,51 @@
     if (lds < (size_t)g.NP0 * 1024 + (fround + 1023) / 1024 * 1024) lds = (size_t)g.NP0 * 1024 + (fround + 1023) / 1024 * 1024;
     g.shl_off = (int)lds;
     lds += 512;
-    if (lds > 160 * 1024) return 1;
+    if (lds > 160 * 1024) return false;
     y2_magic_u32((unsigned)(W + 1), &g.mP, &g.sP);
     y2_magic_u32((unsigned)(H + 1), &g.mH, &g.sH);
+    lds_out = lds;
+    return true;
+}
+
+bool y2_c64_dgrad_bn_fits(int B, int H, int W, int Nf) {
+    C64Geo g;
+    size_t lds = 0;
+    if (Nf == 64) return y2_c64_wide_plan(B, H, W, 1, g, lds);
+    return Nf == 32 && y2_c64_fwd_plan(B, H, W, true, 1, g, lds);
+}
+
+int y2_c64_fwd(const void *P, const void *F, void *O, int B, int H, int W, int Nf, const float *bias, float alpha, const float *bn_shift, float *bn_part,
+               int cus, int *rows, hipStream_t st, const Y2BnBwd *bz) {
+    if (bz && (!bn_part || !bz->Y || ((uintptr_t)bz->Y & 15))) return 1;
+    if (Nf == 64) {
+        if ((bn_part && !bz) || bias || alpha != 1.0f) return 1;
+        return y2_c64_wide(P, F, O, B, H, W, cus, bn_part, bz, rows, st);
+    }
+    const bool narrow = Nf == 32;
+    if (narrow ? ((bn_part && !bz) || bias || alpha != 1.0f) : bz != nullptr) return 1;
+    C64Geo g;
+    size_t lds = 0;
+    if (!y2_c64_fwd_plan(B, H, W, narrow, cus, g, lds)) return 1;
+    const int grid = (int)(((long)g.Mp + g.L - 1) / g.L);
     const unsigned x_bytes = (unsigned)((size_t)g.M * 64 * 2);
-    static std::atomic<size_t> lds_set[4][64];
+    const Y2BnBwd nobz{nullptr, nullptr, nullptr, nullptr, nullptr, 0.f, 0.f, 0};
+    static std::atomic<size_t> lds_set[5][64];
     int dev = 0;
     if (hipGetDevice(&dev) != hipSuccess || dev < 0 || dev >= 64) dev = 0;
-#define C64_LAUNCH(SLOT, MODEv, NFGv, vecp)                                                                                                  \
+#define C64_LAUNCH(SLOT, MODEv, NFGv, BNBv, vecp, bzv)                                                                                       \
     do {                                                                                                                                     \
         if (lds > lds_set[SLOT][dev].load(std::memory_order_relaxed)) {                                                                      \
-            if (hipFuncSetAttribute((const void *)conv_c64_fwd_kernel<MODEv, NFGv>, hipFuncAttributeMaxDynamicSharedMemorySize, (int)lds) != hipSuccess) return 1; \
+            if (hipFuncSetAttribute((const void *)conv_c64_fwd_kernel<MODEv, NFGv, BNBv>, hipFuncAttributeMaxDynamicSharedMemorySize, (int)lds) != hipSuccess) return 1; \
             lds_set[SLOT][dev].store(lds, std::memory_order_relaxed);                                                                        \
         }                                                                                                                                    \
-        conv_c64_fwd_kernel<MODEv, NFGv><<<grid, 512, lds, st>>>((const bf16 *)P, x_bytes, (const bf16 *)F, (bf16 *)O, g, vecp, bn_part, alpha); \
+        conv_c64_fwd_kernel<MODEv, NFGv, BNBv><<<grid, 512, lds, st>>>((const bf16 *)P, x_bytes, (const bf16 *)F, (bf16 *)O, g, vecp, bn_part, alpha, bzv); \
     } while (0)
-    if (narrow) C64_LAUNCH(3, 0, 1, (const float *)nullptr);
-    else if (bn_part) C64_LAUNCH(1, 1, 4, bn_shift);
-    else if (bias || alpha != 1.0f) C64_LAUNCH(2, 2, 4, bias);
-    else C64_LAUNCH(0, 0, 4, (const float *)nullptr);
+    if (narrow && bz) C64_LAUNCH(4, 0, 1, true, (const float *)nullptr, *bz);
+    else if (narrow) C64_LAUNCH(3, 0, 1, false, (const float *)nullptr, nobz);
+    else if (bn_part) C64_LAUNCH(1, 1, 4, false, bn_shift, nobz);
+    else if (bias || alpha != 1.0f) C64_LAUNCH(2, 2, 4, false, bias, nobz);
+    else C64_LAUNCH(0, 0, 4, false, (const float *)nullptr, nobz);
 #undef C64_LAUNCH
     if (rows) *rows = grid < C64_STAT_ROWS ? grid : C64_STAT_ROWS;
     return 0;
diff --git a/yolo_tf_amd/csrc/conv_igemm.hip b/yolo_tf_amd/csrc/conv_igemm.hip
--- a/yolo_tf_amd/csrc/conv_igemm.hip
+++ b/yolo_tf_amd/csrc/conv_igemm.hip
@@ -769,6 +769,15 @@
 extern "C" int yolo2_conv2d_dgrad_bn_fuses(int B, int H, int W, int Nf, int ksize, int dtype) {
     return (B > 0 && H > 0 && W > 0 && Nf > 0 && (dtype == YOLO2_F32 || dtype == YOLO2_BF16) && y2_dgrad_bn_fuses(B, H, W, Nf, ksize, dtype)) ? 1 : 0;
 }
+static bool y2_c64_dgrad_bn_route(int B, int H, int W, int Cp, int ldp, int Nf, int ldo, int ksize, int dtype) {
+    static const bool on = y2_env_int("YOLO2_C64", 1) != 0 && y2_env_int("YOLO2_FUSE_BN_BWD", 1) != 0;
+    return on && (Nf == 32 || Nf == 64) && y2_c64_shape(Cp, ldp, Nf, ldo, ksize, dtype) && y2_env_int("YOLO2_C64_BN_BWD", 1) != 0 &&
+           y2_c64_dgrad_bn_fits(B, H, W, Nf);
+}
+extern "C" int yolo2_conv2d_dgrad_bn_fuses_at(int B, int H, int W, int Cp, int ldp, int Nf, int ldo, int ksize, int dtype) {
+    if (!(B > 0 && H > 0 && W > 0 && Cp > 0 && Nf > 0 && ldp >= Cp && ldo >= Nf) || !(dtype == YOLO2_F32 || dtype == YOLO2_BF16)) return 0;
+    return (y2_dgrad_bn_fuses(B, H, W, Nf, ksize, dtype) || y2_c64_dgrad_bn_route(B, H, W, Cp, ldp, Nf, ldo, ksize, dtype)) ? 1 : 0;
+}
 
 static int conv2d_impl(const void *P, const void *F, const float *bias, void *O, float *ws, size_t ws_bytes, int B, int H,
                        int W, int Cp, int ldp, int Nf, int ldo, int ksize, int dtype, void *stream, const char *fn,
@@ -823,6 +832,19 @@
     if (bwd) {
         static const bool d1_direct = y2_env_int("YOLO2_D1", 1) != 0;
         const bool can = y2_dgrad_bn_fuses(B, H, W, Nf, ksize, dtype);
+        if (bn_part && y2_c64_dgrad_bn_route(B, H, W, Cp, ldp, Nf, ldo, ksize, dtype) && ((uintptr_t)O & 15) == 0 && ((uintptr_t)F & 15) == 0 &&
+            ((uintptr_t)bwd->Y & 15) == 0) {
+            const Tune tu = tune_now();
+            int rows = 0;
+            if (y2_c64_fwd(P, F, O, B, H, W, Nf, nullptr, 1.0f, nullptr, bn_part, tu.cus, &rows, (hipStream_t)stream, bwd) == 0) {
+                const int plan_[8] = {Nf == 64 ? 128 : 256, Nf, 8, 8, 9, 0x100, rows, 1};
+                for (int i = 0; i < 8; ++i) g_last_plan[i] = plan_[i];
+                g_last_stat_rows = rows;
+                Y2_CHECK_LAUNCH();
+                if (pending) *pending = 1;
+                return pending ? YOLO2_OK : y2_bn_part_to_grads(bn_part, Nf, dgamma, dbeta, (hipStream_t)stream);
+            }
+        }
         if (can && d1_direct && bn_part && y2_d1_shape(Cp, ldp, Nf, ldo, ksize, dtype, (long)B * H * W) && ((uintptr_t)O & 15) == 0 && ((uintptr_t)bwd->Y & 15) == 0) {
             const Tune tu = tune_now();
             int rows = 0;
diff --git a/yolo_tf_amd/csrc/conv_shared.h b/yolo_tf_amd/csrc/conv_shared.h
--- a/yolo_tf_amd/csrc/conv_shared.h
+++ b/yolo_tf_amd/csrc/conv_shared.h
@@ -74,8 +74,9 @@
                int cus, int *rows, hipStream_t st);
 
 bool y2_c64_shape(int Cp, int ldp, int Nf, int ldo, int ksize, int dtype);
+bool y2_c64_dgrad_bn_fits(int B, int H, int W, int Nf);
 int y2_c64_fwd(const void *P, const void *F, void *O, int B, int H, int W, int Nf, const float *bias, float alpha, const float *bn_shift, float *bn_part,
-               int cus, int *rows, hipStream_t st);
+               int cus, int *rows, hipStream_t st, const Y2BnBwd *bz = nullptr);
 
 bool y2_d1_shape(int Cp, int ldp, int Nf, int ldo, int ksize, int dtype, long M);
 int y2_d1_dgrad_bn(const void *P, const void *F, void *O, long M, int Cp, int Nf, float *bn_part, const Y2BnBwd &bz, int cus, int *rows, hipStream_t st);
diff --git a/yolo_tf_amd/engine.py b/yolo_tf_amd/engine.py
--- a/yolo_tf_amd/engine.py
+++ b/yolo_tf_amd/engine.py
@@ -262,6 +262,8 @@
                         ):
                     fwd_pool[x] = op
         bn_bwd_fused = {}
+        c64_bn_bwd = os.environ.get('YOLO2_C64_BN_BWD', '1') != '0'
+        pooled_out = {pop['out']: px for px, pop in fused_pool.items()} if c64_bn_bwd else {}
         if self.training and os.environ.get('YOLO2_FUSE_BN_BWD', '1') != '0' and not self.deterministic:
             uses = {}
             for op in graph.ops:
@@ -270,10 +272,21 @@
             producers = {op['out']: op for op in graph.ops if op['kind'] == 'conv'}
             for op in graph.ops:
                 x = op.get('x')
-                if (op['kind'] == 'conv' and x in producers and producers[x]['bn'] and 'fold_bias' not in self.conv[producers[x]['name']]
-                        and uses.get(x, 0) == 1 and x not in fused_pool and x in gact and gact[x][1] == x.c and act[producers[x]['y']][1] == x.c
-                        and ops.conv2d_dgrad_bn_fuses(self.B, x.h, x.w, op['cin'], op['ksize'], self.dtype)):
+                if op['kind'] != 'conv' or uses.get(x, 0) != 1 or x not in gact or gact[x][1] != x.c:
+                    continue
+                ldy = pad8(op['cout'])
+                if c64_bn_bwd:
+                    fuses = ops.conv2d_dgrad_bn_fuses_at(self.B, x.h, x.w, ldy, ldy, op['cin'], x.c, op['ksize'], self.dtype)
+                else:
+                    fuses = ops.conv2d_dgrad_bn_fuses(self.B, x.h, x.w, op['cin'], op['ksize'], self.dtype)
+                if (x in producers and producers[x]['bn'] and 'fold_bias' not in self.conv[producers[x]['name']]
+                        and x not in fused_pool and act[producers[x]['y']][1] == x.c and fuses):
                     bn_bwd_fused[op['name']] = producers[x]
+                elif x in pooled_out and fuses:
+                    prod = producers[pooled_out[x]]
+                    pst = self.conv[prod['name']]
+                    if 'fold_bias' not in pst and 'pool_ymax' in pst:
+                        bn_bwd_fused[op['name']] = prod
         inp = next(iter(graph.inputs.values()))
         self._bindings[(inp.h, inp.w)] = {'graph': graph, 'act': act, 'gact': gact, 'fused_pool': fused_pool, 'zero_ranges': None, 'tmp_grad': {},
                                           'bn_bwd_fused': bn_bwd_fused, 'fwd_pool': fwd_pool}
@@ -630,7 +643,13 @@
                     pfin = None
                     limit = self._fin_limit(cout) if self.fold_finalize else 0
                     first = self._first_fused(op)
-                    if first:
+                    if op['name'] in reduced:
+                        if pool is not None:
+                            dpb, lddp = self.gact[pool['out']]
+                        pend = self._bz_pending.pop(op['name'], None)
+                        if pend is not None:
+                            pfin = (self.parts.bufs[pend[0]], pend[1], 256 * cout, pend[0])
+                    elif first:
                         dpb, lddp = self.gact[pool['out']]
                         part = self.parts.acquire(2 * 256 * 32)
                         ops.first_layer_pool_bwd_reduce(xb, st['Ffwd'], dpb, lddp, st['pool_idx'], st['mean'], st['var'], gamma, beta, self.parts.bufs[part],
@@ -650,10 +669,6 @@
                         else:
                             ops.bn_leaky_pool_bwd_reduce(dpb, lddp, st['pool_idx'], yb, st['mean'], st['var'], gamma, beta, dgam, dbet, self.ws,
                                                          B, out.h, out.w, cout, BN_EPS, LEAKY_ALPHA)
-                    elif op['name'] in reduced:
-                        pend = self._bz_pending.pop(op['name'], None)
-                        if pend is not None:
-                            pfin = (self.parts.bufs[pend[0]], pend[1], 256 * cout, pend[0])
                     elif limit >= 64:
                         rows = ops.bn_leaky_bwd_reduce_part(gob, ldgo, yb, st['mean'], st['var'], gamma, beta, self.ws, limit, M, cout, BN_EPS, LEAKY_ALPHA)
                         pfin = (self.ws, rows, rows * cout)
@@ -724,10 +739,16 @@
                 if x not in inputs:
                     prod = self.bn_bwd_fused.get(op['name'])
                     dst, ldd, fin = self._grad_sink(x, written)
+                    yprev = None
                     if prod is not None and fin is None:
                         pst = self.conv[prod['name']]
+                        if prod['out'] not in self.fused_pool:
+                            yprev = self.act[prod['y']][0]
+                        elif pst.get('ymax_valid') and not self._first_fused(prod):
+                            yprev = pst['pool_ymax']
+                    if yprev is not None:
                         pend = self._conv(dy, st['Fdgr'], None, dst, x.h, x.w, ldy, ldy, op['cin'], ldd, k, k * k * cout,
-                                          bn_bwd=(self.act[prod['y']][0], pst['mean'], pst['var'], self.var[prod['gamma'].name], self.var[prod['beta'].name],
+                                          bn_bwd=(yprev, pst['mean'], pst['var'], self.var[prod['gamma'].name], self.var[prod['beta'].name],
                                                   self.gvar[prod['gamma'].name], self.gvar[prod['beta'].name]))
                         reduced.add(prod['name'])
                         if pend is not None:
diff --git a/yolo_tf_amd/ops.py b/yolo_tf_amd/ops.py
--- a/yolo_tf_amd/ops.py
+++ b/yolo_tf_amd/ops.py
@@ -53,6 +53,13 @@
     if 'yolo2_conv2d_dgrad_bn_fuses' in _lib.MISSING:
         return True
     return bool(lib.yolo2_conv2d_dgrad_bn_fuses(B, H, W, Nf, ksize, dtype_code(dtype)))
+
+
+def conv2d_dgrad_bn_fuses_at(B, H, W, Cp, ldp, Nf, ldo, ksize, dtype):
+    lib = _lib.load()
+    if 'yolo2_conv2d_dgrad_bn_fuses_at' in _lib.MISSING:
+        return conv2d_dgrad_bn_fuses(B, H, W, Nf, ksize, dtype)
+    return bool(lib.yolo2_conv2d_dgrad_bn_fuses_at(B, H, W, Cp, ldp, Nf, ldo, ksize, dtype_code(dtype)))
 
 
 def filter_prep_blocks(ksize, ldcin, ldcout):
```

Result: no change. 4741 img/s (median of 6 runs) (+0.9%).
